# cherise215/Cooperative_Training_and_Latent_Space_Data_Augmentation

Hardware: AMD Instinct MI355X
Metric: cooperative-training slices/sec (256x256, bs16 per GPU) (higher is better)
Workload: dtype f32 (bf16x3 split)

## Files before the change

cooperative_training_and_latent_space_data_augmentation_amd/_ffi.py:

```python
from __future__ import annotations

import ctypes as C
import os

import numpy as np

_HERE = os.path.dirname(os.path.abspath(__file__))
LIB_PATH = os.path.join(_HERE, "csrc", "libctl_hip.so")
ABI_VERSION = 11
RED_BLOCKS = 512

IN_PLAIN, IN_UP2, IN_ZINS2, IN_C4 = 0, 1, 2, 3
ACT_NONE, ACT_LEAKY, ACT_SIGMOID = 0, 1, 2
EPI_BIAS, EPI_ACCUM, EPI_RES, EPI_STATS, EPI_BNBWD, EPI_TAILBWD = 1, 2, 4, 8, 16, 32
(OP_CONV, OP_WGRAD, OP_WGRAD_REDUCE, OP_PACK, OP_BN_FINALIZE, OP_BN_EVAL, OP_BN_ACT, OP_BWD_REDUCE, OP_BN_BWD_FINALIZE,
 OP_BWD_APPLY, OP_CHAN_SUM_FINALIZE, OP_SUMPOOL2, OP_SIGMOID_BWD, OP_ZERO, OP_COPY, OP_PACK_BATCH, OP_WGRAD_REDUCE_BATCH, OP_DROPOUT2D, OP_BN_REPLAY,
 OP_WGRAD_GROUP) = range(1, 21)
WGRAD_GROUP_MAX = 8
OP_MAX_T = 14

CONV_DTYPE = np.dtype([
    ("n", "<i4"), ("hin", "<i4"), ("win", "<i4"), ("cin", "<i4"), ("hout", "<i4"), ("wout", "<i4"), ("cout", "<i4"),
    ("ks", "<i4"), ("stride", "<i4"), ("pad", "<i4"), ("in_mode", "<i4"), ("pro_affine", "<i4"), ("pro_slope", "<f4"),
    ("epi_flags", "<i4"), ("epi_act", "<i4"), ("epi_slope", "<f4"), ("out_h", "<i4"), ("out_w", "<i4"),
    ("out_sy", "<i4"), ("out_sx", "<i4"), ("nsub", "<i4"), ("out_sub", "<i4"), ("groups", "<i4"), ("dt", "<i4")])
DT_BF16, DT_X16, DT_Y16, DT_RES16, DT_X3 = 1, 2, 4, 8, 16
PACK_X3 = 16
OP_DTYPE = np.dtype([("kind", "<i4"), ("i", "<i4", (27,)), ("f", "<f4", (4,)), ("slot", "<i4", (OP_MAX_T,)),
                     ("off", "<i8", (OP_MAX_T,)), ("l", "<i8", (4,))], align=True)


class CtlError(RuntimeError):
    pass


class _Lib:
    def __init__(self):
        self._lib = None

    def load(self):
        if self._lib is not None:
            return self._lib
        if not os.path.exists(LIB_PATH):
            raise CtlError(f"HIP extension not built: {LIB_PATH} is missing. Run `python -c 'import __graft_entry__ as g; "
                           "g.build()'` (or `make -C <package>/csrc`). There is no fallback path.")
        import torch
        lib = C.CDLL(LIB_PATH)
        lib.ctl_last_error.restype = C.c_char_p
        lib.ctl_version.restype = C.c_int
        lib.ctl_launch_count.restype = C.c_ulonglong
        for name in ("ctl_conv_wpack_floats", "ctl_conv_stats_floats", "ctl_wgrad_partial_floats",
                     "ctl_wgrad_bias_partial_floats", "ctl_latent_score_ws_floats", "ctl_latent_mask_apply_ws_floats",
                     "ctl_rescale_intensity_ws_floats", "ctl_sizeof_op", "ctl_sizeof_conv", "ctl_latent_mask_fused_ws_floats", "ctl_conv_wpack_floats_x3",
                     "ctl_surface_stats_ws_bytes", "ctl_surface_map_ws_bytes", "ctl_cc_ws_bytes", "ctl_aug_ws_bytes", "ctl_aug_warp_ws_bytes",
                     "ctl_aug_spline_ws_bytes", "ctl_aug_warp_cubic_ws_bytes", "ctl_aug_bias_ws_bytes"):
            getattr(lib, name).restype = C.c_size_t
        p, i32, i64, f32, u64 = C.c_void_p, C.c_int32, C.c_int64, C.c_float, C.c_uint64
        sig = {
            "ctl_conv_wpack_floats": [i32, i32, i32],
            "ctl_conv_stats_floats": [p], "ctl_conv_stats_blocks": [p],
            "ctl_wgrad_splits": [p], "ctl_wgrad_partial_floats": [p], "ctl_wgrad_bias_partial_floats": [p],
            "ctl_pack_weights": [p, p, i32, i32, i32, i64, i64, i64, i64, i32, p],
            "ctl_conv_forward": [p] * 12, "ctl_conv_forward_ex": [p] * 16, "ctl_conv_pool_ok": [p],
            "ctl_conv_wgrad": [p] * 8, "ctl_conv_wgrad_ex": [p] * 10,
            "ctl_wgrad_group_class": [p, i32], "ctl_wgrad_group_plan": [p, i32, p], "ctl_conv_wgrad_group": [i32] + [p] * 11,
            "ctl_wgrad_reduce": [p, p, p, p, i64, i64, i64, i64, p, i32, p],
            "ctl_confusion_hist": [p, p, i64, i32, p, p],
            "ctl_rescale_intensity": [p, p, p, i32, i64, f32, f32, f32, p],
            "ctl_noise_clamp": [p, p, u64, f32, f32, f32, p, i64, p],
            "ctl_rescale_intensity_ws_floats": [i32],
            "ctl_crop_or_pad": [p, p, i32, i32, i32, i32, i32, i32, p],
            "ctl_bn_finalize": [p, i32, i32, i64, p, p, f32, f32, i32, p, p, p, p, p, p, p, i32, p],
            "ctl_bn_finalize_ex": [p, i32, i32, i64, p, p, f32, f32, i32, p, p, p, p, p, p, p, p, i32, p],
            "ctl_bn_replay_running": [p, p, p, p, i32, f32, p],
            "ctl_bn_eval_coeffs": [i32, p, p, p, p, f32, p, p, i32, p],
            "ctl_bn_act": [p, p, p, f32, p, i64, i32, i32, p],
            "ctl_bwd_reduce": [i32, p, p, p, p, p, f32, i64, i32, p, i32, p], "ctl_red_blocks": [],
            "ctl_bn_bwd_finalize": [p, i32, i64, p, p, p, p, p, p, i32, i32, i32, p],
            "ctl_bn_bwd_finalize_ex": [p, i32, i64, p, p, p, p, p, p, i32, i32, i32, C.c_uint32, p],
            "ctl_bwd_apply": [i32, p, p, p, p, p, f32, p, i64, i32, p, p, i32, p],
            "ctl_chan_sum_finalize": [p, i32, p, i32, p],
            "ctl_sumpool2": [p, p, i32, i32, i32, i32, i32, p],
            "ctl_sigmoid_bwd": [p, p, p, i64, p],
            "ctl_softmax_t_fwd": [p, f32, p, i64, i32, p],
            "ctl_softmax_t_bwd": [p, p, f32, p, i64, i32, p],
            "ctl_onehot": [p, p, i64, i32, p],
            "ctl_ce2d_fwd": [p, p, i64, i32, p, p, p],
            "ctl_ce2d_bwd": [p, p, p, i64, i32, p, p],
            "ctl_mse_fwd": [p, p, i64, f32, p, p, p],
            "ctl_mse_bwd": [p, p, p, i64, f32, p, p],
            "ctl_argmax_c": [p, p, i64, i32, p],
            "ctl_latent_score_ws_floats": [i32, i32, i32, i32],
            "ctl_latent_score": [i32, p, p, p, i32, i32, i32, p],
            "ctl_latent_mask_apply": [i32, p, p, p, i32, p, p, p, p, i32, i32, i32, p],
            "ctl_latent_mask_apply_ws_floats": [i32, i32, i32, i32],
            "ctl_latent_mask_fused_ws_floats": [i32, i32, i32, i32],
            "ctl_latent_mask_fused": [i32, p, p, p, i32, p, p, p, p, p, i32, i32, i32, p],
            "ctl_dropout2d": [p, p, u64, f32, p, p, i32, i32, i32, p],
            "ctl_uniform": [p, i64, u64, p],
            "ctl_step_tick": [p, p],
            "ctl_spin": [i32, p],
            "ctl_dropout2d_ex": [p, p, u64, p, f32, p, p, p, i32, i32, i32, p],
            "ctl_dropout2d_dt": [p, p, u64, p, f32, p, p, i32, i32, i32, C.c_uint32, p],
            "ctl_uniform_dev": [p, i64, u64, p, p],
            "ctl_adam_dev": [p, p, p, p, i64, f32, f32, f32, f32, p, f32, p],
            "ctl_adam": [p, p, p, p, i64, f32, f32, f32, f32, i32, f32, p],
            "ctl_accumulate": [p, p, i32, i64, p],
            "ctl_plan_run": [p, i32, p, i32, p],
            "ctl_prof_start": [C.c_char_p], "ctl_prof_start_sampled": [C.c_char_p, i32], "ctl_prof_stop": [p, C.c_size_t],
            "ctl_pack_weights_batched": [p, p, p, i32, i64, p], "ctl_wgrad_reduce_batched": [p, p, p, i32, i64, p],
            "ctl_pack_weights_bf16_batched": [p, p, p, i32, i64, p],
            "ctl_pack_weights_x3_batched": [p, p, p, i32, i64, p], "ctl_conv_wpack_floats_x3": [i32, i32, i32],
            "ctl_bwd_reduce_rows": [i32, i64, i32],
            "ctl_bn_act_dt": [p, p, p, f32, p, i64, i32, i32, C.c_uint32, p],
            "ctl_bwd_reduce_dt": [i32, p, p, p, p, p, f32, i64, i32, p, i32, C.c_uint32, p, p],
            "ctl_bwd_apply_dt": [i32, p, p, p, p, p, f32, p, i64, i32, p, p, i32, C.c_uint32, p],
            "ctl_sumpool2_dt": [p, p, i32, i32, i32, i32, i32, C.c_uint32, p],
            "ctl_surface_stats_rows": [i32, i32, i32, i32], "ctl_surface_stats_ws_bytes": [i32] * 6,
            "ctl_surface_stats": [p, p, i32, i32, i32, i32, i32, i32, i32, p, p, p, C.c_size_t, p],
            "ctl_surface_map_ws_bytes": [i32] * 4,
            "ctl_surface_map": [p, i32, i32, i32, i32, i32, p, p, p, p, C.c_size_t, p],
            "ctl_cc_ws_bytes": [i32] * 5, "ctl_cc_label": [p, i32, i32, i32, i32, i32, i32, p, p],
            "ctl_cc_keep_largest": [p, i32, i32, i32, i32, i32, i32, p, p, p, C.c_size_t, p],
            "ctl_aug_ws_bytes": [i32] * 3, "ctl_aug_warp_ws_bytes": [i32] * 5, "ctl_aug_field": [p, p, p, p, i32, i32, i32, p, p, C.c_size_t, p],
            "ctl_aug_warp": [p, p, p, p, p, i32, i32, i32, i32, i32, p, p, p, C.c_size_t, p],
            "ctl_aug_spline_ws_bytes": [i32] * 4, "ctl_aug_warp_cubic_ws_bytes": [i32] * 6,
            "ctl_aug_spline_coeffs": [p, p, p, i32, i32, i32, i32, p, p, C.c_size_t, p],
            "ctl_aug_warp_cubic": [p, p, p, p, p, i32, i32, i32, i32, i32, i32, p, p, p, C.c_size_t, p],
            "ctl_aug_bias_ws_bytes": [i32] * 3, "ctl_aug_bias": [p, p, p, p, i32, i32, i32, p, p, C.c_size_t, p],
            "ctl_aug_coarse_field": [p, i32, i32, i32, p, p],
        }
        for name, args in sig.items():
            getattr(lib, name).argtypes = args
        if lib.ctl_version() != ABI_VERSION or lib.ctl_sizeof_op() != OP_DTYPE.itemsize or lib.ctl_sizeof_conv() != CONV_DTYPE.itemsize:
            raise CtlError(f"ABI mismatch: library version {lib.ctl_version()} vs binding {ABI_VERSION}, sizeof(ctl_op)={lib.ctl_sizeof_op()} "
                           f"vs {OP_DTYPE.itemsize}, sizeof(ctl_conv)={lib.ctl_sizeof_conv()} vs {CONV_DTYPE.itemsize}")
        if lib.ctl_red_blocks() != RED_BLOCKS:
            raise CtlError(f"ABI mismatch: the library was built with CTL_RED_BLOCKS={lib.ctl_red_blocks()}, this binding sizes scratch for {RED_BLOCKS}")
        self._lib = lib
        return lib

    def __getattr__(self, name):
        return getattr(self.load(), name)


lib = _Lib()

EXPORTED = ["ctl_version", "ctl_last_error", "ctl_conv_wpack_floats", "ctl_conv_stats_floats", "ctl_conv_stats_blocks",
            "ctl_pack_weights", "ctl_conv_forward", "ctl_conv_forward_ex", "ctl_conv_pool_ok", "ctl_wgrad_splits", "ctl_wgrad_partial_floats",
            "ctl_wgrad_bias_partial_floats", "ctl_conv_wgrad", "ctl_conv_wgrad_ex", "ctl_wgrad_reduce", "ctl_bn_finalize", "ctl_bn_finalize_ex", "ctl_bn_replay_running", "ctl_bn_eval_coeffs",
            "ctl_bn_act", "ctl_bwd_reduce", "ctl_bn_bwd_finalize", "ctl_bn_bwd_finalize_ex", "ctl_bwd_apply", "ctl_chan_sum_finalize", "ctl_sumpool2",
            "ctl_sigmoid_bwd", "ctl_softmax_t_fwd", "ctl_softmax_t_bwd", "ctl_onehot", "ctl_ce2d_fwd", "ctl_ce2d_bwd",
            "ctl_mse_fwd", "ctl_mse_bwd", "ctl_argmax_c", "ctl_latent_score_ws_floats", "ctl_latent_score",
            "ctl_latent_mask_apply", "ctl_latent_mask_apply_ws_floats", "ctl_dropout2d", "ctl_uniform", "ctl_adam", "ctl_plan_run", "ctl_sizeof_op",
            "ctl_sizeof_conv", "ctl_prof_start", "ctl_prof_start_sampled", "ctl_prof_stop", "ctl_pack_weights_batched",
            "ctl_wgrad_reduce_batched", "ctl_confusion_hist", "ctl_rescale_intensity_ws_floats", "ctl_rescale_intensity",
            "ctl_noise_clamp", "ctl_crop_or_pad", "ctl_step_tick", "ctl_spin", "ctl_dropout2d_ex", "ctl_dropout2d_dt", "ctl_uniform_dev", "ctl_adam_dev",
            "ctl_latent_mask_fused_ws_floats", "ctl_latent_mask_fused", "ctl_accumulate", "ctl_pack_weights_bf16_batched",
            "ctl_bn_act_dt", "ctl_bwd_reduce_dt", "ctl_bwd_apply_dt", "ctl_sumpool2_dt", "ctl_bwd_reduce_rows", "ctl_red_blocks",
            "ctl_launch_count", "ctl_conv_wpack_floats_x3", "ctl_pack_weights_x3_batched", "ctl_wgrad_group_class", "ctl_wgrad_group_plan",
            "ctl_conv_wgrad_group", "ctl_surface_stats_rows", "ctl_surface_stats_ws_bytes", "ctl_surface_stats", "ctl_surface_map_ws_bytes",
            "ctl_surface_map", "ctl_cc_ws_bytes", "ctl_cc_label", "ctl_cc_keep_largest", "ctl_aug_ws_bytes", "ctl_aug_warp_ws_bytes", "ctl_aug_field",
            "ctl_aug_warp", "ctl_aug_spline_ws_bytes", "ctl_aug_warp_cubic_ws_bytes", "ctl_aug_spline_coeffs", "ctl_aug_warp_cubic",
            "ctl_aug_bias_ws_bytes", "ctl_aug_bias", "ctl_aug_coarse_field"]


def prof_start(kernel_filter: str = "", every: int = 1) -> None:
    check(lib.ctl_prof_start_sampled(kernel_filter.encode(), int(every)), "ctl_prof_start_sampled")


def prof_stop() -> dict:
    buf = C.create_string_buffer(1 << 18)
    check(lib.ctl_prof_stop(buf, len(buf)), "ctl_prof_stop")
    out = {}
    for line in buf.value.decode().splitlines():
        parts = line.split()
        out[parts[0]] = {k: float(v) for k, v in (kv.split("=") for kv in parts[1:])}
    return out


def check(rc: int, what: str = "") -> None:
    if rc != 0:
        msg = lib.ctl_last_error()
        raise CtlError(f"{what} failed (rc={rc}): {msg.decode() if msg else ''}")


def conv_desc(**kw) -> np.ndarray:
    d = np.zeros((), dtype=CONV_DTYPE)
    d["pad"] = 1 if kw.get("ks", 3) in (3, 4) else 0
    d["stride"] = 1
    d["nsub"] = 1
    d["groups"] = 1
    d["out_sy"] = d["out_sx"] = 1
    for k, v in kw.items():
        d[k] = v
    if "out_h" not in kw:
        d["out_h"] = d["hout"]
    if "out_w" not in kw:
        d["out_w"] = d["wout"]
    return d


def desc_ptr(d: np.ndarray) -> int:
    return d.ctypes.data
```

cooperative_training_and_latent_space_data_augmentation_amd/csrc/ctl_common.h:

```cpp
#pragma once
#include <hip/hip_runtime.h>
#include <stdint.h>
#include <stdio.h>
#include "ctl_hip.h"

void ctl_set_error(const char* fmt, ...);

#define CTL_FAIL(code, ...)            \
    do {                               \
        ctl_set_error(__VA_ARGS__);    \
        return (code);                 \
    } while (0)

#define CTL_REQUIRE(cond, ...)                        \
    do {                                              \
        if (!(cond)) CTL_FAIL(CTL_EINVAL, __VA_ARGS__); \
    } while (0)

void ctl_count_launches(int n);
#define CTL_LAUNCH_CHECK(name)                                                         \
    do {                                                                               \
        ctl_count_launches(1);                                                         \
        hipError_t e__ = hipGetLastError();                                            \
        if (e__ != hipSuccess) CTL_FAIL(CTL_ELAUNCH, "%s: %s", name, hipGetErrorString(e__)); \
    } while (0)

__host__ __device__ static inline int ctl_cdiv(int a, int b) { return (a + b - 1) / b; }
__host__ __device__ static inline int64_t ctl_cdiv64(int64_t a, int64_t b) { return (a + b - 1) / b; }

typedef float f32x4 __attribute__((ext_vector_type(4)));

__device__ __forceinline__ float ctl_leaky(float v, float slope) { return v > 0.f ? v : v * slope; }
__device__ __forceinline__ float ctl_leaky_grad(float out, float slope) { return out > 0.f ? 1.f : slope; }

__device__ __forceinline__ void ctl_barrier_lds_reads_done() { asm volatile("s_barrier" ::: "memory"); }
__device__ __forceinline__ void ctl_barrier_lds_writes_done() { asm volatile("s_waitcnt lgkmcnt(0)\n\ts_barrier" ::: "memory"); }

#ifdef CTL_TUNING
#include <stdlib.h>
static inline int ctl_tune_int(const char* name, int dflt) { const char* e = getenv(name); return e ? atoi(e) : dflt; }
static inline const char* ctl_tune_str(const char* name) { return getenv(name); }
#else
static inline constexpr int ctl_tune_int(const char*, int dflt) { return dflt; }
static inline constexpr const char* ctl_tune_str(const char*) { return nullptr; }
#endif

typedef unsigned int u32x2e __attribute__((ext_vector_type(2)));
typedef __bf16 bf16x2e __attribute__((ext_vector_type(2)));
typedef float f32x2e __attribute__((ext_vector_type(2)));
__device__ __forceinline__ f32x4 ldq(const void* __restrict__ p, int64_t i, bool b16) {
    if (b16) {
        const u32x2e u = reinterpret_cast<const u32x2e*>(p)[i];
        return f32x4{__builtin_bit_cast(float, u.x << 16), __builtin_bit_cast(float, u.x & 0xffff0000u),
                     __builtin_bit_cast(float, u.y << 16), __builtin_bit_cast(float, u.y & 0xffff0000u)};
    }
    return reinterpret_cast<const f32x4*>(p)[i];
}
#ifndef CTL_ELEM_NT
#define CTL_ELEM_NT 0
#endif
__device__ __forceinline__ void stq(void* __restrict__ p, int64_t i, f32x4 v, bool b16) {
    if (b16) {
        const u32x2e pk = u32x2e{__builtin_bit_cast(unsigned, __builtin_convertvector(f32x2e{v.x, v.y}, bf16x2e)),
                                 __builtin_bit_cast(unsigned, __builtin_convertvector(f32x2e{v.z, v.w}, bf16x2e))};
        if (CTL_ELEM_NT) __builtin_nontemporal_store(pk, reinterpret_cast<u32x2e*>(p) + i); else reinterpret_cast<u32x2e*>(p)[i] = pk;
    } else {
        if (CTL_ELEM_NT) __builtin_nontemporal_store(v, reinterpret_cast<f32x4*>(p) + i); else reinterpret_cast<f32x4*>(p)[i] = v;
    }
}

__device__ __forceinline__ double wave_sum_double(double v) {
    for (int o = 32; o > 0; o >>= 1) v += __shfl_xor(v, o);
    return v;
}

struct ctl_bn_chan { float gamma, beta, rm, rv; };
__device__ __forceinline__ ctl_bn_chan ctl_bn_chan_load(int ch, const float* __restrict__ gamma, const float* __restrict__ beta,
                                                        int update_running, const float* __restrict__ running_mean,
                                                        const float* __restrict__ running_var) {
    ctl_bn_chan p;
    p.gamma = gamma[ch]; p.beta = beta[ch];
    p.rm = update_running ? running_mean[ch] : 0.f;
    p.rv = update_running ? running_var[ch] : 0.f;
    return p;
}
__device__ __forceinline__ void ctl_bn_coefs(double s1, double s2, double count, int c, int g, int ch, ctl_bn_chan& p, float eps,
                                             float momentum, int update_running, float* __restrict__ running_mean,
                                             float* __restrict__ running_var, float* __restrict__ scale, float* __restrict__ shift,
                                             float* __restrict__ save_mean, float* __restrict__ save_invstd,
                                             float* __restrict__ save_uvar = nullptr) {
    const double mean = s1 / count;
    double var = s2 / count - mean * mean;
    if (var < 0.0) var = 0.0;
    const float invstd = (float)(1.0 / sqrt(var + (double)eps));
    const float sc = p.gamma * invstd;
    scale[g * c + ch] = sc;
    shift[g * c + ch] = p.beta - (float)mean * sc;
    if (save_mean) save_mean[g * c + ch] = (float)mean;
    if (save_invstd) save_invstd[g * c + ch] = invstd;
    if (update_running) {
        const double unbiased = count > 1.0 ? var * count / (count - 1.0) : var;
        if (save_uvar) save_uvar[g * c + ch] = (float)unbiased;
        p.rm = (1.f - momentum) * p.rm + momentum * (float)mean;
        p.rv = (1.f - momentum) * p.rv + momentum * (float)unbiased;
        running_mean[ch] = p.rm;
        running_var[ch] = p.rv;
    }
}
struct ctl_conv_cfg {
    int mt, tw, nt;
    int th;
    int tiles_h, tiles_w;
    int g;
    int cot;
    int pc;
};
int ctl_conv_pick_cfg(const ctl_conv* d, ctl_conv_cfg* c, int for_wgrad);
int ctl_conv_grid_x(int ntiles, int other, int occ);
static inline int ctl_num_cus() { static const int n = ctl_tune_int("CTL_NUM_CUS", 256); return n; }

int ctl_conv_forward_bf16(const ctl_conv* d, const void* x, const void* x2, const void* wpack, const float* bias, const float* pro_scale,
                          const float* pro_shift, const void* res, const float* res_scale, const float* res_shift, const void* res2, void* y,
                          float* stats_partial, void* pool, void* xout, ctl_stream stream);
int ctl_conv_bf16_stats_blocks(const ctl_conv* d);
int ctl_wgrad_bf16_splits(const ctl_conv* d);
int ctl_conv_wgrad_bf16(const ctl_conv* d, const void* x, const float* pro_scale, const float* pro_shift, const void* dy, const void* dy2,
                        const float* dy_coef, float* w_partial, float* b_partial, ctl_stream stream);

int ctl_wgrad_bf16_group_class(const ctl_conv* d, int has_dy2);
int ctl_wgrad_bf16_group_plan(const ctl_conv* descs, int n, int32_t* splits);
int ctl_conv_wgrad_bf16_group(int n, const ctl_conv* descs, const int32_t* splits, const void* const* x, const float* const* pro_scale,
                              const float* const* pro_shift, const void* const* dy, const void* const* dy2, const float* const* dy_coef,
                              float* const* w_partial, float* const* b_partial, ctl_stream stream);

int ctl_conv_x3_ok(const ctl_conv* d);
int ctl_conv_x3_stats_blocks(const ctl_conv* d);
int ctl_conv_forward_x3(const ctl_conv* d, const float* x, const float* wpack, const float* bias, const float* pro_scale, const float* pro_shift,
                        const float* res, const float* res_scale, const float* res_shift, const float* res2, const float* x2, float* y,
                        float* stats_partial, float* pool, float* xout, ctl_stream stream);

int ctl_wgrad_x3_ok(const ctl_conv* d);
int ctl_wgrad_x3_splits(const ctl_conv* d);
int ctl_conv_wgrad_x3(const ctl_conv* d, const float* x, const float* pro_scale, const float* pro_shift, const float* dy, const float* dy2,
                      const float* dy_coef, float* w_partial, float* b_partial, ctl_stream stream);

int ctl_prof_begin(const char* kind, const ctl_conv* d, const ctl_conv_cfg* c, int nt, hipStream_t stream, bool dy2 = false);
void ctl_prof_end(int token, hipStream_t stream);
int ctl_prof_begin_raw(const char* id, double flops, double bytes, hipStream_t stream);
```

cooperative_training_and_latent_space_data_augmentation_amd/csrc/ctl_conv.hip:

```cpp
#include <stdlib.h>

#include <type_traits>

#include "ctl_common.h"

#include "ctl_conv_common.h"

#ifdef CTL_TIMING
#define CTL_TM_WAVES 65536
__device__ unsigned long long ctl_tm[CTL_TM_WAVES][10];
#define TM_DECL unsigned long long tm_prev = __builtin_amdgcn_s_memtime(), tm_acc[10] = {0, 0, 0, 0, 0, 0, 0, 0, 0, 0}; \
                const unsigned long long tm_t0 = tm_prev, tm_r0 = __builtin_amdgcn_s_memrealtime();
#define TM(i) { const unsigned long long tm_now = __builtin_amdgcn_s_memtime(); tm_acc[i] += tm_now - tm_prev; tm_prev = tm_now; }
#define TM_COUNT(i) { tm_acc[i] += 1; }
#define TM_FLUSH { const unsigned w_ = ((blockIdx.x + gridDim.x * (blockIdx.y + gridDim.y * blockIdx.z)) * 4 + (threadIdx.x >> 6)) % CTL_TM_WAVES; \
                   tm_acc[8] = __builtin_amdgcn_s_memtime() - tm_t0; tm_acc[9] = __builtin_amdgcn_s_memrealtime() - tm_r0; \
                   if ((threadIdx.x & 63) == 0) { _Pragma("unroll") for (int i_ = 0; i_ < 10; ++i_) ctl_tm[w_][i_] += tm_acc[i_]; } }
extern "C" int ctl_debug_timing(unsigned long long* out8) {
    static unsigned long long host[CTL_TM_WAVES][10];
    if (hipMemcpyFromSymbol(host, HIP_SYMBOL(ctl_tm), sizeof(host)) != hipSuccess) return -1;
    for (int i = 0; i < 12; ++i) out8[i] = 0;
    for (int w = 0; w < CTL_TM_WAVES; ++w) {
        for (int i = 0; i < 10; ++i) out8[i] += host[w][i];
        if (host[w][8] > out8[10]) out8[10] = host[w][8];
// ... 466 lines not shown
    constexpr int TPR = (LDS_FLOATS / TAP_FLOATS) < NACC ? (LDS_FLOATS / TAP_FLOATS) : NACC;
    const int64_t split_base = (int64_t)blockIdx.x * TAPS * cin_p * cout_p;
#pragma unroll
    for (int tap0 = 0; tap0 < NACC; tap0 += TPR) {
        if (tap0 > 0) ctl_barrier_lds_reads_done();
#pragma unroll
        for (int tp = 0; tp < TPR; ++tp) {
            const int tap = tap0 + tp;
            if (tap < NACC) {
#pragma unroll
                for (int t = 0; t < NTW; ++t) {
                    float* r0 = red + tp * TAP_FLOATS + ((wave * NTW + t) * 4) * 64 + lane;
                    r0[0] = acc[tap][t].x; r0[64] = acc[tap][t].y; r0[128] = acc[tap][t].z; r0[192] = acc[tap][t].w;
                }
            }
        }
        ctl_barrier_lds_writes_done();
#pragma unroll
        for (int tp = 0; tp < TPR; ++tp) {
            const int tap = tap0 + tp;
            if (tap < NACC) {
#pragma unroll
                for (int e0 = 0; e0 < NTW * 256; e0 += 256) {
                    const int e = e0 + tid;
                    const int t = e >> 8, r = (e >> 6) & 3, l = e & 63;
                    float v = 0.f;
#pragma unroll
                    for (int w = 0; w < 4; ++w) v += red[tp * TAP_FLOATS + ((w * NTW + t) * 4 + r) * 64 + l];
                    const int co = (cot0 + t) * 16 + (l & 15);
                    if (C4) {
                        const int wtap = 4 * tap + (l >> 4);
                        if (wtap < TAPS && co < cout_p) w_partial[split_base + ((int64_t)wtap * cin_p + r) * cout_p + co] = v;
                    } else {
                        const int ci = g * 16 + (l >> 4) * 4 + r;
                        if (co < cout_p) w_partial[split_base + ((int64_t)tap * cin_p + ci) * cout_p + co] = v;
                    }
                }
            }
        }
    }
    if (g == 0 && b_partial != nullptr) {
        ctl_barrier_lds_reads_done();
#pragma unroll
        for (int t = 0; t < NTW; ++t) {
            float v = bsum[t];
            v += __shfl_xor(v, 16);
            v += __shfl_xor(v, 32);
            if (q == 0) red[(wave * NTW + t) * 16 + p] = v;
        }
        ctl_barrier_lds_writes_done();
        if (tid < NTW * 16) {
            float v = 0.f;
#pragma unroll
            for (int w = 0; w < 4; ++w) v += red[w * NTW * 16 + tid];
            const int co = cot0 * 16 + tid;
            if (co < cout_p) b_partial[(int64_t)blockIdx.x * cout_p + co] = v;
        }
    }
#ifdef CTL_TIMING_WGRAD
    tm_acc[5] += __builtin_amdgcn_s_memtime() - tm_loop_end;
    TM_FLUSH
#endif
}

__global__ __launch_bounds__(256) void wgrad_reduce_kernel(const float* __restrict__ w_partial,
                                                            const float* __restrict__ b_partial, int splits, int taps,
                                                            int ks, int cin, int cout, int cin_p, int cout_p,
                                                            float* __restrict__ dw, int64_t s_co, int64_t s_ci,
                                                            int64_t s_kh, int64_t s_kw, float* __restrict__ dbias,
                                                            int accumulate) {
    __shared__ float sm[8][32];
    const int e = threadIdx.x & 31, sl = threadIdx.x >> 5;
    const int64_t total = (int64_t)taps * cin * cout;
    const int64_t idx = (int64_t)blockIdx.x * 32 + e;
    const bool is_w = idx < total;
    const bool is_b = !is_w && dbias != nullptr && idx < total + cout;
    float v = 0.f;
    int co = 0, ci = 0, tap = 0;
    if (is_w) {
        co = idx % cout;
        ci = (idx / cout) % cin;
        tap = idx / ((int64_t)cout * cin);
        const int64_t stride = (int64_t)taps * cin_p * cout_p;
        const float* src = w_partial + ((int64_t)tap * cin_p + ci) * cout_p + co;
        for (int s = sl; s < splits; s += 8) v += src[s * stride];
    } else if (is_b) {
        co = idx - total;
        for (int s = sl; s < splits; s += 8) v += b_partial[(int64_t)s * cout_p + co];
    }
    sm[sl][e] = v;
    __syncthreads();
    if (sl == 0 && (is_w || is_b)) {
        float t = 0.f;
#pragma unroll
        for (int k = 0; k < 8; ++k) t += sm[k][e];
        float* dst = is_w ? dw + co * s_co + ci * s_ci + (tap / ks) * s_kh + (tap % ks) * s_kw : dbias + co;
        *dst = accumulate ? (*dst + t) : t;
    }
}

__global__ void pack_weights_kernel(const float* __restrict__ src, float* __restrict__ dst, int cout, int cin, int ks,
                                    int g_chunks, int64_t total, int64_t s_co, int64_t s_ci, int64_t s_kh,
                                    int64_t s_kw, int flip) {
    const int64_t idx = (int64_t)blockIdx.x * blockDim.x + threadIdx.x;
    if (idx >= total) return;
    const int j = idx & 3, lane = (idx >> 2) & 63;
    int64_t rest = idx >> 8;
    const int g = rest % g_chunks;
    rest /= g_chunks;
    const int taps = ks * ks;
    const int tap = rest % taps;
    const int cot = rest / taps;
    const int co = cot * 16 + (lane & 15);
    const int ci = g * 16 + (lane >> 4) * 4 + j;
    int kh = tap / ks, kw = tap % ks;
    if (flip) { kh = ks - 1 - kh; kw = ks - 1 - kw; }
    float v = 0.f;
    if (co < cout && ci < cin) v = src[co * s_co + ci * s_ci + kh * s_kh + kw * s_kw];
    dst[idx] = v;
}

__global__ void pack_weights_batched_kernel(const float* __restrict__ params, float* __restrict__ wpack,
                                            const int64_t* __restrict__ table) {
    const int64_t* r = table + (int64_t)blockIdx.y * 12;
    const int64_t total = r[10];
    const int64_t idx = (int64_t)blockIdx.x * blockDim.x + threadIdx.x;
    if (idx >= total || (r[11] & CTL_PACK_X3)) return;
    const float* src = params + r[0];
    float* dst = wpack + r[1];
    const int cout = (int)r[2], cin = (int)r[3], ks = (int)r[4], flip = (int)r[5];
    const int g_chunks = (cin + 15) / 16;
    const int j = idx & 3, lane = (idx >> 2) & 63;
    int64_t rest = idx >> 8;
    const int g = rest % g_chunks;
    rest /= g_chunks;
    const int taps = ks * ks;
    const int tap = rest % taps;
    const int cot = rest / taps;
    const int co = cot * 16 + (lane & 15);
    const int ci = g * 16 + (lane >> 4) * 4 + j;
    int kh = tap / ks, kw = tap % ks;
    float v = 0.f;
    if (r[11] == 4) {
        const int c = j, quad = (int)((idx >> 8) % 3), cot4 = (int)((idx >> 8) / 3);
        const int co4 = cot4 * 16 + (lane & 15), tp = 4 * quad + (lane >> 4);
        if (co4 < cout && c < cin && tp < 9) v = src[co4 * r[6] + c * r[7] + (tp / 3) * r[8] + (tp % 3) * r[9]];
        dst[idx] = v;
        return;
    }
    if (r[11] == 1) {
        if (co < cout && ci < cin) {
            for (int a = 0; a < 2; ++a) {
                const int sh = a + 2 - kh;
                if (sh < 0 || sh > 2) continue;
                for (int b = 0; b < 2; ++b) {
                    const int sw = b + 2 - kw;
                    if (sw < 0 || sw > 2) continue;
                    v += src[co * r[6] + ci * r[7] + sh * r[8] + sw * r[9]];
                }
            }
        }
    } else if (r[11] == 2) {
        if (co < cout && ci < cin) {
            const int a = flip >> 1, b = flip & 1;
            const int h0 = (kh == 0) ? 0 : (a ? 2 : 1), h1 = (kh == 0) ? (a ? 1 : 0) : 2;
            const int w0 = (kw == 0) ? 0 : (b ? 2 : 1), w1 = (kw == 0) ? (b ? 1 : 0) : 2;
            for (int sh = h0; sh <= h1; ++sh)
                for (int sw = w0; sw <= w1; ++sw) v += src[co * r[6] + ci * r[7] + sh * r[8] + sw * r[9]];
        }
    } else if (r[11] == 3) {
        if (co < cout && ci < cin) {
            const int a = flip >> 1, b = flip & 1;
            const int sh = a ? (kh == 0 ? 2 : 0) : (kh == 0 ? 1 : -1);
            const int sw = b ? (kw == 0 ? 2 : 0) : (kw == 0 ? 1 : -1);
            if (sh >= 0 && sw >= 0) v = src[co * r[6] + ci * r[7] + sh * r[8] + sw * r[9]];
        }
    } else {
        if (flip) { kh = ks - 1 - kh; kw = ks - 1 - kw; }
        if (co < cout && ci < cin) v = src[co * r[6] + ci * r[7] + kh * r[8] + kw * r[9]];
    }
    dst[idx] = v;
}

__global__ __launch_bounds__(256) void wgrad_reduce_batched_kernel(const float* __restrict__ scratch, float* __restrict__ grad,
                                                                    const int64_t* __restrict__ table) {
    __shared__ float sm[32][65];
    const int64_t* r = table + (int64_t)blockIdx.y * 16;
    const int splits = (int)r[4], taps = (int)(r[5] & 0xff), ks = (int)(r[5] >> 8), cin = (int)r[6], cout = (int)r[7];
    const int cin_p = (int)r[8], cout_p = (int)r[9];
    const int64_t total = (int64_t)taps * cin * cout;
    const bool has_b = r[1] >= 0 && r[3] >= 0;
    const bool wide = splits <= 64;
    const int EW = wide ? 64 : 8, SLN = wide ? 4 : 32;
    if ((int64_t)blockIdx.x * EW >= total + (has_b ? cout : 0)) return;
    const int e = wide ? (threadIdx.x & 63) : (threadIdx.x & 7), sl = wide ? (threadIdx.x >> 6) : (threadIdx.x >> 3);
    const int64_t idx = (int64_t)blockIdx.x * EW + e;
    const bool is_w = idx < total, is_b = !is_w && has_b && idx < total + cout;
    float v = 0.f;
    int co = 0, ci = 0, tap = 0;
    if (is_w) {
        co = idx % cout;
        ci = (idx / cout) % cin;
        tap = idx / ((int64_t)cout * cin);
        const int64_t stride = (int64_t)taps * cin_p * cout_p;
        const float* src = scratch + r[0] + ((int64_t)tap * cin_p + ci) * cout_p + co;
        for (int s0 = sl; s0 < splits; s0 += 8 * SLN) {
            float t8[8];
#pragma unroll
            for (int u = 0; u < 8; ++u) { const int s = s0 + u * SLN; t8[u] = s < splits ? src[s * stride] : 0.f; }
#pragma unroll
            for (int u = 0; u < 8; ++u) v += t8[u];
        }
    } else if (is_b) {
        co = idx - total;
        const float* src = scratch + r[1] + co;
        for (int s = sl; s < splits; s += SLN) v += src[(int64_t)s * cout_p];
    }
    sm[sl][e] = v;
    __syncthreads();
    if (sl == 0 && (is_w || is_b)) {
        float t = 0.f;
        for (int k = 0; k < SLN; ++k) t += sm[k][e];
        float* dst = is_w ? grad + r[2] + co * r[10] + ci * r[11] + (tap / ks) * r[12] + (tap % ks) * r[13] : grad + r[3] + co;
        *dst = r[14] ? (*dst + t) : t;
    }
}

extern "C" int ctl_pack_weights_batched(const float* params, float* wpack, const int64_t* table, int32_t n_rec,
                                        int64_t max_total, ctl_stream stream) {
    CTL_REQUIRE(params && wpack && table && n_rec > 0 && max_total > 0, "pack_weights_batched: bad arguments");
    pack_weights_batched_kernel<<<dim3((unsigned)ctl_cdiv64(max_total, 256), (unsigned)n_rec), dim3(256), 0, (hipStream_t)stream>>>(
        params, wpack, table);
    CTL_LAUNCH_CHECK("pack_weights_batched");
    return CTL_OK;
}
extern "C" int ctl_wgrad_reduce_batched(const float* scratch, float* grad, const int64_t* table, int32_t n_rec,
                                        int64_t max_elems, ctl_stream stream) {
    CTL_REQUIRE(scratch && grad && table && n_rec > 0 && max_elems > 0, "wgrad_reduce_batched: bad arguments");
    wgrad_reduce_batched_kernel<<<dim3((unsigned)max_elems, (unsigned)n_rec), dim3(256), 0, (hipStream_t)stream>>>(
        scratch, grad, table);
    CTL_LAUNCH_CHECK("wgrad_reduce_batched");
    return CTL_OK;
}

extern "C" size_t ctl_conv_wpack_floats(int32_t cin, int32_t cout, int32_t ks) {
    return (size_t)ctl_cdiv(cout, 16) * ks * ks * ctl_cdiv(cin, 16) * 256;
}

static bool conv_combo_ok(const ctl_conv* d) {
    const int k = d->ks, s = d->stride, m = d->in_mode, pd = d->pad;
    if (k == 3 && s == 1 && pd == 1 && m != CTL_IN_C4) return true;
    if (k == 3 && s == 1 && pd == 1 && m == CTL_IN_C4 && d->cin <= 4 && d->nsub == 1) return true;
    if (k == 3 && s == 2 && pd == 1 && m == CTL_IN_PLAIN) return true;
    if (k == 1 && s == 1 && pd == 0 && m != CTL_IN_ZINS2) return true;
    if (k == 2 && s == 2 && pd == 0 && m == CTL_IN_PLAIN) return true;
    if (k == 4 && s == 2 && pd == 1 && m == CTL_IN_PLAIN) return true;
    if (k == 2 && s == 1 && (pd == 0 || pd == 2) && m == CTL_IN_PLAIN && d->nsub == 4) return true;
    return false;
}

int ctl_conv_pick_cfg(const ctl_conv* d, ctl_conv_cfg* c, int for_wgrad) {
    CTL_REQUIRE(conv_combo_ok(d), "conv: unsupported ks/stride/pad/in_mode %d/%d/%d/%d", d->ks, d->stride, d->pad,
                d->in_mode);
    CTL_REQUIRE(d->cin == 1 || d->cin % 4 == 0, "conv: cin must be 1 or a multiple of 4 (got %d)", d->cin);
    CTL_REQUIRE(d->cout == 1 || d->cout % 4 == 0, "conv: cout must be 1 or a multiple of 4 (got %d)", d->cout);
    CTL_REQUIRE(d->cin < 16 ? (d->cin == 1 || d->cin == 4 || d->cin == 8 || d->cin == 12) : d->cin % 16 == 0,
                "conv: cin >= 16 must be a multiple of 16 (got %d)", d->cin);
    CTL_REQUIRE(d->nsub == 1 || d->nsub == 4, "conv: nsub must be 1 or 4");
    c->cot = ctl_cdiv(d->cout, 16);
    c->g = ctl_cdiv(d->cin, 16);
    c->nt = (c->cot % 2 == 0) ? 2 : 1;
    auto blocks = [&](int mt, int tw) {
        const int th = 4 * mt * 16 / tw;
        return (int64_t)d->n * ctl_cdiv(d->hout, th) * ctl_cdiv(d->wout, tw) * (c->cot / c->nt) * d->nsub;
    };
    int mt, tw;
    if (for_wgrad) {
        if (d->hout >= 8) { mt = 2; tw = 16; }
        else { mt = 1; tw = 16; }
    } else if (d->stride == 2) {
        if (blocks(2, 16) >= 384) { mt = 2; tw = 16; } else { mt = 1; tw = 16; }
        if (d->ks == 4 && c->nt == 2) { mt = 1; tw = 16; }
    } else if (d->wout >= 32 && blocks(4, 32) >= 512 && !(c->nt == 2 && blocks(4, 32) > 768)) {
        mt = 4; tw = 32;
    } else if (blocks(2, 16) >= 384) {
        mt = 2; tw = 16;
    } else {
        mt = 1; tw = 16;
    }
    {
        static int fm = 0, ft = 0, fn = 0;
        static const bool forced = [] {
            const char* f = ctl_tune_str("CTL_FORCE_CFG");
            return f && sscanf(f, "%d,%d,%d", &fm, &ft, &fn) == 3;
        }();
        if (forced) {
            const bool tile_ok = (fm == 4 && ft == 32 && d->stride == 1 && !for_wgrad) || (fm == 2 && ft == 16) || (fm == 1 && ft == 16);
            if (tile_ok) { mt = fm; tw = ft; }
            if ((fn == 1 || fn == 2) && c->cot % fn == 0) c->nt = fn;
            if (d->ks == 4 && c->nt == 2) { mt = 1; tw = 16; }
        }
    }
    c->pc = 0;
    c->mt = mt; c->tw = tw; c->th = 4 * mt * 16 / tw;
    c->tiles_h = ctl_cdiv(d->hout, c->th);
    c->tiles_w = ctl_cdiv(d->wout, c->tw);
    return CTL_OK;
}

int ctl_conv_grid_x(int ntiles, int other, int occ) {
    static int per_cu = -1;
    if (per_cu < 0) {
        per_cu = ctl_tune_int("CTL_PERSIST", 4);
        if (per_cu < 1) per_cu = 1;
    }
    const int resident = occ < per_cu ? occ : per_cu;
    int cap = (ctl_num_cus() * resident) / other;
    if (other > 1 && cap >= 8) cap -= cap % 8;
    if (cap < 1) cap = 1;
    return ntiles < cap ? ntiles : cap;
}

extern "C" int ctl_pack_weights(const float* src, float* dst, int32_t cout, int32_t cin, int32_t ks, int64_t s_co,
                                int64_t s_ci, int64_t s_kh, int64_t s_kw, int32_t flip, ctl_stream stream) {
    CTL_REQUIRE(src && dst && cout > 0 && cin > 0 && ks >= 1 && ks <= 4, "pack_weights: bad arguments");
    const int64_t total = (int64_t)ctl_conv_wpack_floats(cin, cout, ks);
    pack_weights_kernel<<<dim3((unsigned)ctl_cdiv64(total, 256)), dim3(256), 0, (hipStream_t)stream>>>(
        src, dst, cout, cin, ks, ctl_cdiv(cin, 16), total, s_co, s_ci, s_kh, s_kw, flip);
    CTL_LAUNCH_CHECK("pack_weights");
    return CTL_OK;
}

struct conv_call {
    const ctl_conv* d; ctl_conv_cfg c;
    const float *x, *wpack, *bias, *pro_scale, *pro_shift, *res, *res_scale, *res_shift, *res2, *x2;
    float *y, *stats_partial, *pool, *xout;
    hipStream_t stream;
    bool query;
    int grid_x;
};

template <int KS, int S, int MODE, int MT, int TW, int NT, int EPI, bool X2 = false>
static void conv_go(conv_call& a) {
    if constexpr (!X2 && ((KS == 3 && S == 1 && MODE == CTL_IN_PLAIN) || (KS == 4 && S == 2)) && EPI != 2) {
        if (a.d->pro_affine == 2) { conv_go<KS, S, MODE, MT, TW, NT, EPI, true>(a); return; }
    }
    static int occ = 0;
    if (!occ) {
        int n = 0;
        if (hipOccupancyMaxActiveBlocksPerMultiprocessor(&n, conv_igemm_kernel<KS, S, MODE, MT, TW, NT, EPI, X2>, 256, 0) != hipSuccess || n < 1) {
            (void)hipGetLastError();
            n = 2;
        }
        occ = n;
    }
    const ctl_conv* d = a.d;
    const int ntiles = d->n * a.c.tiles_h * a.c.tiles_w;
    a.grid_x = ctl_conv_grid_x(ntiles, (a.c.cot / NT) * d->nsub, occ);
    if (a.query) return;
    const dim3 grid((unsigned)a.grid_x, (unsigned)(a.c.cot / NT), (unsigned)d->nsub);
    conv_igemm_kernel<KS, S, MODE, MT, TW, NT, EPI, X2><<<grid, dim3(256), 0, a.stream>>>(
        *d, a.x, a.wpack, a.bias, a.pro_scale, a.pro_shift, a.res, a.res_scale, a.res_shift, a.y, a.stats_partial, a.c.tiles_h,
        a.c.tiles_w, a.c.g, (int64_t)ctl_conv_wpack_floats(d->cin, d->cout, d->ks), ntiles, a.res2, a.x2, a.pool, a.xout);
}
template <int KS, int S, int MODE>
constexpr bool conv_tail_ok() { return (KS == 1 && MODE == CTL_IN_PLAIN) || KS == 2 || (KS == 3 && S == 1 && MODE == CTL_IN_ZINS2); }
template <int KS, int S, int MODE, int MT, int TW>
static void conv_go_nt(conv_call& a) {
    const bool epi = (a.d->epi_flags & (CTL_EPI_RES | CTL_EPI_ACCUM | CTL_EPI_BNBWD)) != 0;
    if constexpr (conv_tail_ok<KS, S, MODE>()) {
        if (a.d->epi_flags & CTL_EPI_TAILBWD) {
            if (a.c.nt == 2) conv_go<KS, S, MODE, MT, TW, 2, 2>(a); else conv_go<KS, S, MODE, MT, TW, 1, 2>(a);
            return;
        }
    }
    if constexpr (KS == 3 && S == 1 && MODE == CTL_IN_PLAIN) {
        if ((a.d->epi_flags & (CTL_EPI_RES | CTL_EPI_ACCUM | CTL_EPI_BNBWD)) == CTL_EPI_BNBWD && a.d->cout % 16 == 0 && a.d->epi_act == CTL_ACT_NONE) {
            if (a.c.nt == 2) conv_go<KS, S, MODE, MT, TW, 2, 3>(a); else conv_go<KS, S, MODE, MT, TW, 1, 3>(a);
            return;
        }
    }
    if (a.c.nt == 2) { if (epi) conv_go<KS, S, MODE, MT, TW, 2, 1>(a); else conv_go<KS, S, MODE, MT, TW, 2, 0>(a); }
    else { if (epi) conv_go<KS, S, MODE, MT, TW, 1, 1>(a); else conv_go<KS, S, MODE, MT, TW, 1, 0>(a); }
}
template <int KS, int S, int MODE>
static void conv_go_tile(conv_call& a) {
    if (S == 1 && a.c.mt == 4 && a.c.tw == 32) conv_go_nt<KS, S, MODE, (S == 1 ? 4 : 2), (S == 1 ? 32 : 16)>(a);
    else if (a.c.mt == 2) conv_go_nt<KS, S, MODE, 2, 16>(a);
    else conv_go_nt<KS, S, MODE, 1, 16>(a);
}
static int conv_dispatch(conv_call& a) {
    const int k = a.d->ks, s = a.d->stride, m = a.d->in_mode;
    if (k == 3 && s == 1 && m == CTL_IN_PLAIN) conv_go_tile<3, 1, CTL_IN_PLAIN>(a);
    else if (k == 3 && s == 1 && m == CTL_IN_UP2) conv_go_tile<3, 1, CTL_IN_UP2>(a);
    else if (k == 3 && s == 1 && m == CTL_IN_ZINS2) conv_go_tile<3, 1, CTL_IN_ZINS2>(a);
    else if (k == 3 && s == 1 && m == CTL_IN_C4) conv_go_tile<3, 1, CTL_IN_C4>(a);
    else if (k == 3 && s == 2) conv_go_tile<3, 2, CTL_IN_PLAIN>(a);
    else if (k == 1 && m == CTL_IN_PLAIN) conv_go_tile<1, 1, CTL_IN_PLAIN>(a);
    else if (k == 1 && m == CTL_IN_UP2) conv_go_tile<1, 1, CTL_IN_UP2>(a);
    else if (k == 2 && s == 2) conv_go_tile<2, 2, CTL_IN_PLAIN>(a);
    else if (k == 2 && s == 1) conv_go_tile<2, 1, CTL_IN_PLAIN>(a);
    else if (k == 4 && s == 2) {
        const bool epi = (a.d->epi_flags & (CTL_EPI_RES | CTL_EPI_ACCUM | CTL_EPI_BNBWD)) != 0;
        if (a.c.mt == 2 && a.c.nt == 1) { if (epi) conv_go<4, 2, CTL_IN_PLAIN, 2, 16, 1, 1>(a); else conv_go<4, 2, CTL_IN_PLAIN, 2, 16, 1, 0>(a); }
        else if (a.c.nt == 2) { if (epi) conv_go<4, 2, CTL_IN_PLAIN, 1, 16, 2, 1>(a); else conv_go<4, 2, CTL_IN_PLAIN, 1, 16, 2, 0>(a); }
        else { if (epi) conv_go<4, 2, CTL_IN_PLAIN, 1, 16, 1, 1>(a); else conv_go<4, 2, CTL_IN_PLAIN, 1, 16, 1, 0>(a); }
    }
    else CTL_FAIL(CTL_EUNSUPPORTED, "conv_forward: no kernel for this combination");
    return CTL_OK;
}

extern "C" int ctl_conv_stats_blocks(const ctl_conv* d) {
    if (d->dt & CTL_DT_BF16) return ctl_conv_bf16_stats_blocks(d);
    if (d->dt & CTL_DT_X3) return ctl_conv_x3_stats_blocks(d);
    conv_call a = {};
    a.d = d;
    if (ctl_conv_pick_cfg(d, &a.c, 0) != CTL_OK) return -1;
    a.query = true;
    if (conv_dispatch(a) != CTL_OK) return -1;
    return a.grid_x * d->nsub;
}
extern "C" size_t ctl_conv_stats_floats(const ctl_conv* d) {
    const int b = ctl_conv_stats_blocks(d);
    return b < 0 ? 0 : (size_t)(d->groups > 1 ? d->groups : 1) * b * 2 * d->cout;
}

extern "C" int ctl_conv_forward(const ctl_conv* d, const float* x, const float* wpack, const float* bias,
                                const float* pro_scale, const float* pro_shift, const float* res,
                                const float* res_scale, const float* res_shift, float* y, float* stats_partial,
                                ctl_stream stream) {
    return ctl_conv_forward_ex(d, x, wpack, bias, pro_scale, pro_shift, res, res_scale, res_shift, nullptr, nullptr, y, stats_partial, nullptr, nullptr, stream);
}
extern "C" int ctl_conv_pool_ok(const ctl_conv* d) {
    ctl_conv_cfg c;
    if (!d) return 0;
    if (!(d->epi_flags & CTL_EPI_TAILBWD) || d->ks != 1 || d->stride != 1 || d->in_mode != CTL_IN_PLAIN || d->nsub != 1 || (d->out_h & 1) || (d->out_w & 1) ||
        d->out_h != d->hout || d->out_w != d->wout || d->cout % 16 != 0)
        return 0;
    if (ctl_conv_pick_cfg(d, &c, 0) != CTL_OK) return 0;
    return (c.mt == 4 && c.tw == 32) || (c.mt == 2 && c.tw == 16);
}
extern "C" int ctl_conv_forward_ex(const ctl_conv* d, const float* x, const float* wpack, const float* bias,
                                   const float* pro_scale, const float* pro_shift, const float* res,
                                   const float* res_scale, const float* res_shift, const float* res2, const float* x2, float* y,
                                   float* stats_partial, float* pool, float* xout, ctl_stream stream) {
    CTL_REQUIRE(d && x && wpack && y, "conv_forward: null argument");
    CTL_REQUIRE(!xout || d->pro_affine == 2, "conv_forward: `xout` (the virtual input written out) goes with the BatchNorm-backward prologue (pro_affine 2)");
    CTL_REQUIRE(!pool || ctl_conv_pool_ok(d), "conv_forward: `pool` needs a CTL_EPI_TAILBWD 1x1 conv with even output sizes whose tile configuration gives every wave a row pair (ctl_conv_pool_ok)");
    CTL_REQUIRE((d->dt & CTL_DT_BF16) || !(d->dt & (CTL_DT_X16 | CTL_DT_Y16 | CTL_DT_RES16)), "conv_forward: bf16-stored tensors need CTL_DT_BF16");
    conv_call a = {};
    a.d = d;
    int rc = ctl_conv_pick_cfg(d, &a.c, 0);
    if (rc != CTL_OK) return rc;
    CTL_REQUIRE(!(d->epi_flags & CTL_EPI_BIAS) || bias, "conv_forward: CTL_EPI_BIAS without bias");
    CTL_REQUIRE(!(d->epi_flags & CTL_EPI_RES) || (res && res_scale && res_shift), "conv_forward: CTL_EPI_RES without res");
    CTL_REQUIRE(!(d->epi_flags & CTL_EPI_STATS) || stats_partial, "conv_forward: CTL_EPI_STATS without a partial buffer");
    CTL_REQUIRE(!(d->epi_flags & CTL_EPI_BNBWD) || ((d->epi_flags & CTL_EPI_STATS) && res && res_scale && res_shift &&
                                                    !(d->epi_flags & (CTL_EPI_RES | CTL_EPI_ACCUM | CTL_EPI_BIAS)) && d->epi_act == CTL_ACT_NONE),
                "conv_forward: CTL_EPI_BNBWD needs CTL_EPI_STATS + res (= u) + res_scale/res_shift (BatchNorm coefficients) and nothing else");
    if (d->epi_flags & CTL_EPI_TAILBWD) {
        const int k = d->ks, s = d->stride, m = d->in_mode;
        CTL_REQUIRE((d->epi_flags & CTL_EPI_STATS) && res && res2 && !(d->epi_flags & (CTL_EPI_RES | CTL_EPI_BNBWD | CTL_EPI_BIAS)) &&
                    d->epi_act == CTL_ACT_NONE && d->cout % 16 == 0,
                    "conv_forward: CTL_EPI_TAILBWD needs CTL_EPI_STATS + res (= the block output) + res2 (= the BatchNorm input), cout %% 16 == 0, nothing else but CTL_EPI_ACCUM");
        CTL_REQUIRE((k == 1 && m == CTL_IN_PLAIN) || k == 2 || (k == 3 && s == 1 && m == CTL_IN_ZINS2),
                    "conv_forward: CTL_EPI_TAILBWD is built for the launches that write a block's output gradient (1x1, 2x2, zero-insert 3x3)");
        CTL_REQUIRE(d->epi_slope >= 0.f && d->epi_slope <= 1.f, "conv_forward: LeakyReLU slope must be in [0, 1]");
    }
    CTL_REQUIRE(d->pro_affine >= 0 && d->pro_affine <= 2, "conv_forward: pro_affine must be 0, 1 or 2");
    CTL_REQUIRE(d->pro_affine != 1 || (pro_scale && pro_shift), "conv_forward: prologue without scale/shift");
    CTL_REQUIRE(d->pro_affine != 2 || (x2 && pro_scale && d->cin % 16 == 0 && d->in_mode == CTL_IN_PLAIN &&
                                       ((d->ks == 3 && d->stride == 1) || (d->ks == 4 && d->stride == 2)) && !(d->epi_flags & CTL_EPI_TAILBWD)),
                "conv_forward: the BatchNorm-backward prologue (pro_affine 2) needs x2 + coefficients, cin %% 16 == 0 and a plain 3x3 stride-1 or 4x4 stride-2 conv");
    CTL_REQUIRE(!d->pro_affine || (d->groups > 1 ? d->groups : 1) * d->cin <= CTL_PRO_MAX, "conv_forward: groups * cin = %d prologue coefficients exceed %d", (d->groups > 1 ? d->groups : 1) * d->cin, CTL_PRO_MAX);
    CTL_REQUIRE(d->pro_affine != 1 || (d->pro_slope >= 0.f && d->pro_slope <= 1.f), "conv_forward: prologue slope must be in [0, 1]");
    CTL_REQUIRE(d->epi_act != CTL_ACT_LEAKY || (d->epi_slope >= 0.f && d->epi_slope <= 1.f), "conv_forward: LeakyReLU slope must be in [0, 1]");
    CTL_REQUIRE(d->n > 0 && d->hout > 0 && d->wout > 0, "conv_forward: empty problem");
    CTL_REQUIRE(d->groups >= 0 && (d->groups <= 1 || d->n % d->groups == 0), "conv_forward: n=%d is not divisible into %d groups", d->n, d->groups);
    CTL_REQUIRE((int64_t)d->n * d->hin * d->win * d->cin * 4 < (1ll << 31) &&
                (int64_t)d->n * d->out_h * d->out_w * d->cout * 4 < (1ll << 31),
                "conv_forward: tensors must stay below 2 GiB (32-bit buffer offsets)");
    if (d->dt & CTL_DT_X3)
        return ctl_conv_forward_x3(d, x, wpack, bias, pro_scale, pro_shift, res, res_scale, res_shift, res2, x2, y, stats_partial, pool, xout, stream);
    if (d->dt & CTL_DT_BF16) {
        const int ptok16 = ctl_prof_begin("conv_igemm_bf16", d, &a.c, a.c.nt, (hipStream_t)stream);
        rc = ctl_conv_forward_bf16(d, x, x2, wpack, bias, pro_scale, pro_shift, res, res_scale, res_shift, res2, y, stats_partial, pool, xout, stream);
        ctl_prof_end(ptok16, (hipStream_t)stream);
        return rc;
    }
    a.x = x; a.wpack = wpack; a.bias = bias; a.pro_scale = pro_scale; a.pro_shift = pro_shift; a.res = res;
    a.res_scale = res_scale; a.res_shift = res_shift; a.res2 = res2; a.x2 = x2; a.y = y; a.stats_partial = stats_partial; a.pool = pool; a.xout = xout;
    a.stream = (hipStream_t)stream;
    const int ptok = ctl_prof_begin("conv_igemm", d, &a.c, a.c.nt, a.stream);
    rc = conv_dispatch(a);
    if (rc != CTL_OK) return rc;
    ctl_prof_end(ptok, a.stream);
    CTL_LAUNCH_CHECK("conv_forward");
    return CTL_OK;
}

#ifndef CTL_WGRAD_PIPE
#define CTL_WGRAD_PIPE 1
#endif
struct wgrad_cfg { ctl_conv_cfg c; int ntw, splits, ntiles, cin_p, cout_p; };

struct wgrad_call {
    const ctl_conv* d; wgrad_cfg* w;
    const float *x, *pro_scale, *pro_shift, *dy, *dy2, *dy_coef;
    float *w_partial, *b_partial;
    hipStream_t stream;
    bool query;
};

template <int KS, int S, int MODE, int MT, int TW, int NTW>
static void wgrad_go(wgrad_call& a) {
    static int occ = 0;
    if (!occ) {
        int n = 0;
        if (hipOccupancyMaxActiveBlocksPerMultiprocessor(&n, conv_wgrad_kernel<KS, S, MODE, MT, TW, NTW>, 256, 0) != hipSuccess || n < 1) {
            (void)hipGetLastError();
            n = 2;
        }
        occ = n;
    }
    wgrad_cfg& w = *a.w;
    static int per_cu = -1;
    if (per_cu < 0) {
        per_cu = ctl_tune_int("CTL_WGRAD_PERSIST", 1);
        if (per_cu < 1) per_cu = 1;
    }
    const int par = w.c.g * (w.c.cot / NTW);
    static const int slots = ctl_tune_int("CTL_WGRAD_SLOTS", 0);
    static const int narrow_cu = ctl_tune_int("CTL_WGRAD_NARROW_PERSIST", 2);
    const int cu_blocks = (KS == 1 || MODE == CTL_IN_C4) ? narrow_cu : per_cu;
    int splits = (slots > 0 ? slots : ctl_num_cus() * (occ < cu_blocks ? occ : cu_blocks)) / par;
    if (splits > 512) splits = 512;
    if (splits > w.ntiles) splits = w.ntiles;
    if (splits < 1) splits = 1;
    w.splits = splits;
    if (a.query) return;
    const dim3 grid((unsigned)splits, (unsigned)w.c.g, (unsigned)(w.c.cot / NTW));
    if constexpr (KS == 3 && S == 1 && MODE != CTL_IN_C4) {
        static const int pipe = ctl_tune_int("CTL_WGRAD_PIPE", CTL_WGRAD_PIPE);
        const bool pipe_on = pipe >= 2 || (pipe == 1 && a.dy2 && w.ntiles >= 8 * splits);
        if (pipe_on && a.d->cin % 4 == 0 && a.d->cout % 4 == 0 && a.d->cin <= CTL_PRO_MAX) {
            if (a.dy2)
                conv_wgrad_kernel<KS, S, MODE, MT, TW, NTW, true, true><<<grid, dim3(256), 0, a.stream>>>(
                    *a.d, a.x, a.pro_scale, a.pro_shift, a.dy, a.w_partial, a.b_partial, w.c.tiles_h, w.c.tiles_w, w.ntiles, w.cin_p, w.cout_p, a.dy2, a.dy_coef);
            else
                conv_wgrad_kernel<KS, S, MODE, MT, TW, NTW, false, true><<<grid, dim3(256), 0, a.stream>>>(
                    *a.d, a.x, a.pro_scale, a.pro_shift, a.dy, a.w_partial, a.b_partial, w.c.tiles_h, w.c.tiles_w, w.ntiles, w.cin_p, w.cout_p, nullptr, nullptr);
            return;
        }
    }
    if constexpr (KS == 3 && S == 1) {
        if (a.dy2) {
            conv_wgrad_kernel<KS, S, MODE, MT, TW, NTW, true><<<grid, dim3(256), 0, a.stream>>>(
                *a.d, a.x, a.pro_scale, a.pro_shift, a.dy, a.w_partial, a.b_partial, w.c.tiles_h, w.c.tiles_w, w.ntiles, w.cin_p, w.cout_p, a.dy2, a.dy_coef);
            return;
        }
    }
    conv_wgrad_kernel<KS, S, MODE, MT, TW, NTW><<<grid, dim3(256), 0, a.stream>>>(
        *a.d, a.x, a.pro_scale, a.pro_shift, a.dy, a.w_partial, a.b_partial, w.c.tiles_h, w.c.tiles_w, w.ntiles, w.cin_p, w.cout_p, nullptr, nullptr);
}
template <int KS, int S, int MODE>
static void wgrad_go_tile(wgrad_call& a) {
    const wgrad_cfg& w = *a.w;
    if (w.c.mt == 2) { if (w.ntw == 2) wgrad_go<KS, S, MODE, 2, 16, 2>(a); else wgrad_go<KS, S, MODE, 2, 16, 1>(a); }
    else { if (w.ntw == 2) wgrad_go<KS, S, MODE, 1, 16, 2>(a); else wgrad_go<KS, S, MODE, 1, 16, 1>(a); }
}
static int wgrad_dispatch(wgrad_call& a) {
    const int k = a.d->ks, s = a.d->stride, m = a.d->in_mode;
    if (k == 3 && s == 1 && m == CTL_IN_PLAIN) wgrad_go_tile<3, 1, CTL_IN_PLAIN>(a);
    else if (k == 3 && s == 1 && m == CTL_IN_UP2) wgrad_go_tile<3, 1, CTL_IN_UP2>(a);
    else if (k == 3 && s == 1 && m == CTL_IN_C4) wgrad_go_tile<3, 1, CTL_IN_C4>(a);
    else if (k == 3 && s == 2) wgrad_go_tile<3, 2, CTL_IN_PLAIN>(a);
    else if (k == 1 && m == CTL_IN_PLAIN) wgrad_go_tile<1, 1, CTL_IN_PLAIN>(a);
    else if (k == 1 && m == CTL_IN_UP2) wgrad_go_tile<1, 1, CTL_IN_UP2>(a);
    else if (k == 2 && s == 2) wgrad_go_tile<2, 2, CTL_IN_PLAIN>(a);
    else CTL_FAIL(CTL_EUNSUPPORTED, "conv_wgrad: no kernel for this combination");
    return CTL_OK;
}

static int wgrad_pick(const ctl_conv* d, wgrad_cfg* w) {
    CTL_REQUIRE(d->nsub == 1, "wgrad: nsub must be 1");
    CTL_REQUIRE(d->in_mode != CTL_IN_ZINS2, "wgrad: zero-insert input is not a forward mode");
    int rc = ctl_conv_pick_cfg(d, &w->c, 1);
    if (rc != CTL_OK) return rc;
    w->ntw = (w->c.cot >= 2 && w->c.cot % 2 == 0) ? 2 : 1;
    w->ntiles = d->n * w->c.tiles_h * w->c.tiles_w;
    w->cin_p = w->c.g * 16;
    w->cout_p = w->c.cot * 16;
    if (d->dt & CTL_DT_BF16) {
        w->splits = ctl_wgrad_bf16_splits(d);
        return w->splits > 0 ? CTL_OK : CTL_EUNSUPPORTED;
    }
    if (d->dt & CTL_DT_X3) {
        w->splits = ctl_wgrad_x3_splits(d);
        return w->splits > 0 ? CTL_OK : CTL_EUNSUPPORTED;
    }
    wgrad_call a = {};
    a.d = d; a.w = w; a.query = true;
    return wgrad_dispatch(a);
}

extern "C" int ctl_wgrad_splits(const ctl_conv* d) {
// ... 70 lines not shown
```

cooperative_training_and_latent_space_data_augmentation_amd/csrc/ctl_conv_igemm.h:

```cpp
#pragma once
#include <stdlib.h>

#include <type_traits>

#include "ctl_common.h"

#include "ctl_conv_common.h"
#include "ctl_conv_x3_stage.h"

#ifndef TM_DECL
#define TM_DECL
#define TM(i)
#define TM_COUNT(i)
#define TM_FLUSH
#endif

#define CTL_MODE_IS_PLAIN(M) ((M) == CTL_IN_PLAIN || (M) == CTL_IN_C4)

template <int KS, int S, int MODE, int MT, int TW, bool X2 = false>
struct XStage {
    using G = Geom<KS, S, MT, TW>;
    static constexpr bool C4M = (MODE == CTL_IN_C4);
    static constexpr int UNITS = G::IH * G::IW * (C4M ? 1 : 4);
    static constexpr int NU = (UNITS + 255) / 256;
    static constexpr int PADH = (G::PAD + 1) >> 1;
    int rel[NU];
    int rc[NU];
    int lds[NU];
    f32x4 v[NU];
    f32x4 v2[X2 ? NU : 1];
    unsigned vmask;
    int pad_h, pad_w;
    bool all_in;
    int tb_last;

    __device__ __forceinline__ void init(const ctl_conv& d) {
        const int tid = threadIdx.x, cq = C4M ? 0 : (tid & 3);
#pragma unroll
        for (int i = 0; i < NU; ++i) {
            const int u = tid + i * 256;
            const int pix = C4M ? u : (u >> 2);
            const int r = pix / G::IW;
            const int c = pix - r * G::IW;
            const bool in = u < UNITS;
            const int rr = CTL_MODE_IS_PLAIN(MODE) ? r : (((r - G::PAD) >> 1) + PADH);
            const int cc = CTL_MODE_IS_PLAIN(MODE) ? c : (((c - G::PAD) >> 1) + PADH);
            rel[i] = in ? ((rr * d.win + cc) * d.cin + cq * 4) * 4 : CTL_OOB;
            rc[i] = in ? (r | (c << 16)) : 0x7fff7fff;
            lds[i] = in ? (C4M ? (r * G::IWP + c) * 4 : ((r * G::IWP + G::ldscol(c)) * 16 + cq * 4)) : G::XT_IMAGE;
        }
        vmask = 0;
        all_in = false;
        pad_h = pad_w = G::PAD;
    }

    __device__ __forceinline__ void load(__amdgpu_buffer_rsrc_t rx, const ctl_conv& d, int n, int ho0, int wo0, int g) { load(rx, rx, d, n, ho0, wo0, g); }
    __device__ __forceinline__ void load(__amdgpu_buffer_rsrc_t rx, __amdgpu_buffer_rsrc_t rx2, const ctl_conv& d, int n, int ho0, int wo0, int g) {
        const int vh0 = ho0 * S - pad_h, vw0 = wo0 * S - pad_w;
        const unsigned hv = CTL_MODE_IS_PLAIN(MODE) ? d.hin : 2 * d.hin;
        const unsigned wv = CTL_MODE_IS_PLAIN(MODE) ? d.win : 2 * d.win;
        const int oh = CTL_MODE_IS_PLAIN(MODE) ? vh0 : ((ho0 >> 1) - PADH);
        const int ow = CTL_MODE_IS_PLAIN(MODE) ? vw0 : ((wo0 >> 1) - PADH);
        const int tb = (((n * d.hin + oh) * d.win + ow) * d.cin + g * 16) * 4;
        tb_last = tb;
#ifdef CTL_NO_INTERIOR
        all_in = false;
#else
        all_in = MODE != CTL_IN_ZINS2 && vh0 >= 0 && vw0 >= 0 && vh0 + G::IH <= (int)hv && vw0 + G::IW <= (int)wv &&
                 g * 16 + 16 <= d.cin;
#endif
        if (all_in) {
#pragma unroll
            for (int i = 0; i < NU; ++i) v[i] = ctl_bload4s(rx, rel[i], tb);
            if constexpr (X2) {
#pragma unroll
                for (int i = 0; i < NU; ++i) v2[i] = ctl_bload4s(rx2, rel[i], tb);
            }
            return;
        }
        const bool chan_ok = C4M || g * 16 + (threadIdx.x & 3) * 4 < d.cin;
        unsigned m = 0;
        int vo[NU];
#pragma unroll
        for (int i = 0; i < NU; ++i) {
            const int vh = vh0 + (rc[i] & 0xffff), vw = vw0 + (rc[i] >> 16);
            bool ok = chan_ok && (unsigned)vh < hv && (unsigned)vw < wv;
            if (MODE == CTL_IN_ZINS2) ok = ok && (((vh | vw) & 1) == 0);
            vo[i] = ok ? (tb + rel[i]) : CTL_OOB;
            m |= ok ? (1u << i) : 0u;
        }
        vmask = m;
        if constexpr (X2) {
#pragma unroll
            for (int i = 0; i < NU; ++i) { v[i] = ctl_bload4(rx, vo[i]); v2[i] = ctl_bload4(rx2, vo[i]); }
        } else if (d.cin >= 4) {
#pragma unroll
            for (int i = 0; i < NU; ++i) v[i] = ctl_bload4(rx, vo[i]);
        } else {
#pragma unroll
            for (int i = 0; i < NU; ++i) v[i] = f32x4{ctl_bload1(rx, vo[i]), 0.f, 0.f, 0.f};
        }
    }

    __device__ __forceinline__ void store(float* __restrict__ xt, const ctl_conv& d, int g,
                                          const float* pro_scale, const float* pro_shift, int goff, const float* pro_c = nullptr) {
        store(xt, d, g, pro_scale, pro_shift, goff, pro_c, ctl_rsrc((const void*)nullptr, 0), false);
    }
    __device__ __forceinline__ void store(float* __restrict__ xt, const ctl_conv& d, int g,
                                          const float* pro_scale, const float* pro_shift, int goff, const float* pro_c,
                                          __amdgpu_buffer_rsrc_t rxout, bool xout_on) {
        if constexpr (X2) {
            const int cb = g * 16 + (threadIdx.x & 3) * 4;
            const f32x4 ca = *reinterpret_cast<const f32x4*>(pro_scale + goff + cb), cbb = *reinterpret_cast<const f32x4*>(pro_shift + goff + cb);
            const f32x4 cc = *reinterpret_cast<const f32x4*>(pro_c + goff + cb);
            const f32x4 zero = {0.f, 0.f, 0.f, 0.f};
#pragma unroll
            for (int i = 0; i < NU; ++i) {
                const bool in = all_in || ((vmask >> i) & 1u);
                const f32x4 r = in ? (ca * v[i] + cbb * v2[i] + cc) : zero;
                *reinterpret_cast<f32x4*>(xt + lds[i]) = r;
                if (xout_on) {
                    const unsigned tr = (unsigned)((rc[i] & 0xffff) - pad_h), tc = (unsigned)((rc[i] >> 16) - pad_w);
                    const bool own = in && tr < (unsigned)(G::TH * S) && tc < (unsigned)(TW * S);
                    ctl_bstore4(rxout, own ? (tb_last + rel[i]) : CTL_OOB, r);
                }
            }
            return;
        }
        if (!d.pro_affine) {
#pragma unroll
            for (int i = 0; i < NU; ++i) *reinterpret_cast<f32x4*>(xt + lds[i]) = v[i];
            return;
        }
        const int cb = C4M ? 0 : g * 16 + (threadIdx.x & 3) * 4;
        f32x4 sc = {1.f, 1.f, 1.f, 1.f}, sh = {0.f, 0.f, 0.f, 0.f};
        if (cb < d.cin) {
            if (d.cin >= 4) {
                sc = *reinterpret_cast<const f32x4*>(pro_scale + goff + cb);
                sh = *reinterpret_cast<const f32x4*>(pro_shift + goff + cb);
            } else {
                sc.x = pro_scale[goff];
                sh.x = pro_shift[goff];
            }
        }
        const float slope = d.pro_slope;
        if (all_in) {
#pragma unroll
            for (int i = 0; i < NU; ++i) *reinterpret_cast<f32x4*>(xt + lds[i]) = ctl_leaky01(v[i] * sc + sh, slope);
            return;
        }
        const f32x4 zero = {0.f, 0.f, 0.f, 0.f};
#pragma unroll
        for (int i = 0; i < NU; ++i) {
            const f32x4 t = ctl_leaky01(v[i] * sc + sh, slope);
            *reinterpret_cast<f32x4*>(xt + lds[i]) = ((vmask >> i) & 1u) ? t : zero;
        }
    }
};


#ifndef CTL_LB_MID
#define CTL_LB_MID 3
#endif
#ifndef CTL_LB_SMALL
#define CTL_LB_SMALL 3
#endif
#ifndef CTL_PC_SETS
#define CTL_PC_SETS 3
#endif
#ifndef CTL_PC_SETS_X2
#define CTL_PC_SETS_X2 2
#endif
template <int KS, int S, int MODE, int MT, int TW, int NT, int EPI, bool X2 = false, bool X3 = false, bool PC = false>
#ifndef CTL_LB_X2EPI
#define CTL_LB_X2EPI 2
#endif
#ifndef CTL_LB_X2
#define CTL_LB_X2 2
#endif
#ifndef CTL_LB_SMALL_X2EPI
#define CTL_LB_SMALL_X2EPI CTL_LB_SMALL
#endif
#ifndef CTL_LB_X3
#define CTL_LB_X3(MT, NT, X2) (((NT) == 1 && (MT) >= 2 && !(X2)) ? 3 : 2)
#endif
__global__ __launch_bounds__(PC ? 512 : 256, PC ? 2 : X3 ? CTL_LB_X3(MT, NT, X2) : (MT * NT >= 8 || KS == 4) ? 2 : ((MT * NT >= 4) ? (X2 ? (EPI ? CTL_LB_X2EPI : CTL_LB_X2) : CTL_LB_MID)
                                                                                    : ((X2 && EPI) ? CTL_LB_SMALL_X2EPI : CTL_LB_SMALL))) void conv_igemm_kernel(const ctl_conv d, const float* __restrict__ x,
                                                          const float* __restrict__ wpack,
                                                          const float* __restrict__ bias,
                                                          const float* __restrict__ pro_scale,
                                                          const float* __restrict__ pro_shift,
                                                          const float* __restrict__ res,
                                                          const float* __restrict__ res_scale,
                                                          const float* __restrict__ res_shift, float* __restrict__ y,
                                                          float* __restrict__ stats_partial, int tiles_h, int tiles_w,
                                                          int G_chunks, int64_t wpack_sub_stride, int ntiles,
                                                          const float* __restrict__ res2, const float* __restrict__ x2,
                                                          float* __restrict__ pool, float* __restrict__ xout) {
    using G = Geom<KS, S, MT, TW>;
    constexpr int TAPS = KS * KS;
    constexpr bool C4 = (MODE == CTL_IN_C4);
    static_assert(!C4 || (KS == 3 && S == 1), "K-packed taps: 3x3 stride-1 only");
    static_assert(!X3 || !C4, "X3: whole 16-channel chunks");
    static_assert(!PC || X3, "the producer / consumer form exists for the X3 launches");
    constexpr int NIMG = PC ? 2 : 1;
    using XS3 = XStage3<KS, S, C4 ? CTL_IN_PLAIN : MODE, MT, TW, X2>;
    constexpr int NFRAG = X3 ? (TAPS + 1) / 2 : (C4 ? 3 : TAPS);
    constexpr int WSPL = X3 ? 3 : 1;
    constexpr int RED_FLOATS = 4 * NT * 16 * 2;
    constexpr int WT_FLOATS = NFRAG * NT * WSPL * 256;
    constexpr int XT_ALLOC = X3 ? XS3::XT_BYTES / 4 : G::XT_FLOATS;
    static_assert((NIMG * (XT_ALLOC + WT_FLOATS) + RED_FLOATS + (X2 ? 3 : 2) * CTL_PRO_MAX) * 4 <= 160 * 1024, "LDS budget of one CU");
    __shared__ __attribute__((aligned(16))) float xt[NIMG * (XT_ALLOC + WT_FLOATS) + RED_FLOATS + (X2 ? 3 : 2) * CTL_PRO_MAX];
    float* wt = xt + NIMG * XT_ALLOC;
    float* sred = wt + NIMG * WT_FLOATS;
    float* cf_scale = sred + RED_FLOATS;
    float* cf_shift = cf_scale + CTL_PRO_MAX;
    float* cf_c = cf_shift + (X2 ? CTL_PRO_MAX : 0);
    constexpr int WU = NFRAG * NT * WSPL * 64, NW = (WU + 255) / 256;

    const int tid = threadIdx.x;
    const int lane = tid & 63;
    const int wave_all = __builtin_amdgcn_readfirstlane(tid >> 6);
    const int wave = PC ? (wave_all & 3) : wave_all;
    const bool consumer = PC && wave_all >= 4;
    const int p = lane & 15, q = lane >> 4;
    const int P = gridDim.x < 8 ? (int)gridDim.x : 8;
    const int xcd = blockIdx.x % P, jblk = blockIdx.x / P;
    const int nb = ((int)gridDim.x - xcd + P - 1) / P;
    const int t_lo = (int)(((int64_t)ntiles * xcd) / P), t_hi = (int)(((int64_t)ntiles * (xcd + 1)) / P);
    const int bid0 = t_lo + jblk;
    const int z = blockIdx.z;
    const int cot0 = blockIdx.y * NT;
    const float* wp = wpack + (int64_t)z * wpack_sub_stride;
    const int my_tiles = (bid0 < t_hi) ? (t_hi - bid0 + nb - 1) / nb : 0;
    const int total_it = my_tiles * G_chunks;
    const int flags = d.epi_flags;
    const int ngroups = d.groups > 1 ? d.groups : 1;
    const int group_n = d.n / ngroups;
    const int oy0 = (z >> 1) * d.out_sub, ox0 = (z & 1) * d.out_sub;
    const __amdgpu_buffer_rsrc_t rx = ctl_rsrc(x, (int64_t)d.n * d.hin * d.win * d.cin * 4);
    const __amdgpu_buffer_rsrc_t rx2 = X2 ? ctl_rsrc(x2, (int64_t)d.n * d.hin * d.win * d.cin * 4) : rx;
    const bool xout_on = X2 && xout != nullptr && blockIdx.y == 0 && blockIdx.z == 0;
    const __amdgpu_buffer_rsrc_t rxout = xout_on ? ctl_rsrc(xout, (int64_t)d.n * d.hin * d.win * d.cin * 4) : rx;
    const int64_t ybytes = (int64_t)d.n * d.out_h * d.out_w * d.cout * 4;
    const __amdgpu_buffer_rsrc_t ry = ctl_rsrc(y, ybytes);
    const __amdgpu_buffer_rsrc_t rres = ctl_rsrc(EPI ? (const void*)res : (const void*)y, ybytes);
    constexpr bool TAIL = (EPI == 2);
    const __amdgpu_buffer_rsrc_t rres2 = ctl_rsrc(TAIL ? (const void*)res2 : (const void*)y, ybytes);
    constexpr bool CAN_POOL = TAIL && KS == 1 && S == 1 && MODE == CTL_IN_PLAIN && (MT / (TW / 16)) == 2;
    const __amdgpu_buffer_rsrc_t rpool = ctl_rsrc(CAN_POOL && pool ? (const void*)pool : (const void*)y, CAN_POOL && pool ? ybytes / 4 : ybytes);

    f32x4 ssum[NT], ssq[NT];
#pragma unroll
    for (int t = 0; t < NT; ++t) ssum[t] = ssq[t] = f32x4{0.f, 0.f, 0.f, 0.f};

    constexpr int TWT = TW / 16;
    static_assert(MT % TWT == 0, "a wave's M-tiles must cover whole tile rows");
    const int wrow = wave * (MT / TWT);
    int yrel[MT];
#pragma unroll
    for (int m = 0; m < MT; ++m)
        yrel[m] = (((wrow + m / TWT) * d.out_sy * d.out_w + ((m % TWT) * 16 + p) * d.out_sx) * d.cout + q * 4) * 4;
    const float* xrd = xt + ((wrow * S) * G::IWP + p) * 16 + q * 4;
    const float* wrd = wt + lane * 4;
    const float* xrd4[3];
#pragma unroll
    for (int j = 0; j < 3; ++j) {
        const int tp = (4 * j + q < 9) ? 4 * j + q : 8;
        xrd4[j] = xt + ((wrow + tp / 3) * G::IWP + p + tp % 3) * 4;
    }
    int xoff3[X3 ? NFRAG : 1];
    if constexpr (X3) {
#pragma unroll
        for (int f = 0; f < NFRAG; ++f) {
            int tap = 2 * f + (q >> 1);
            tap = tap < TAPS ? tap : TAPS - 1;
            const int kh = tap / KS, kw = tap % KS;
            const int kcol = (S == 2) ? ((kw & 1) * G::IWH + (kw >> 1)) : kw;
            xoff3[f] = (((wrow * S + kh) * G::IWP + p + kcol) * 16) + (q & 1) * XS3::PLANE;
        }
    }
    const unsigned char* xt8 = reinterpret_cast<const unsigned char*>(xt);
    const unsigned char* wrd8 = reinterpret_cast<const unsigned char*>(wt) + lane * 16;

    std::conditional_t<X3, XS3, XStage<KS, S, MODE, MT, TW, X2>> xs;
    xs.init(d);
    if (KS == 2 && S == 1) {
        xs.pad_h = d.pad == 2 ? 1 - (z >> 1) : 0;
        xs.pad_w = d.pad == 2 ? 1 - (z & 1) : 0;
    }
    const __amdgpu_buffer_rsrc_t rw = ctl_rsrc(wp, (int64_t)ctl_cdiv(d.cout, 16) * NFRAG * G_chunks * WSPL * 1024);
    f32x4 wv[NW];
    int wrel[NW];
#pragma unroll
    for (int i = 0; i < NW; ++i) {
        const int u = tid + i * 256;
        const int tt = u >> 6, l = u & 63;
        const int sp = X3 ? tt % WSPL : 0, tq = tt / WSPL;
        const int tap = tq / NT, t = tq - tap * NT;
        wrel[i] = (u < WU) ? (((((cot0 + t) * NFRAG + tap) * G_chunks) * WSPL + sp) * 64 + l) * 16 : CTL_OOB;
    }
    auto wload = [&](int g) {
#pragma unroll
        for (int i = 0; i < NW; ++i) wv[i] = ctl_bload4s(rw, wrel[i], g * WSPL * 1024);
    };
    auto wstore = [&](int img = 0) {
#pragma unroll
        for (int i = 0; i < NW; ++i) {
            const int u = tid + i * 256;
            if (u < WU) *reinterpret_cast<f32x4*>(wt + img * WT_FLOATS + u * 4) = wv[i];
        }
    };

    TileWalk cur, nxt;
    cur.init(bid0, nb, tiles_h, tiles_w);
    nxt = cur;
    TM_DECL
    if (!PC && total_it > 0) {
        xs.load(rx, rx2, d, cur.n, cur.th * G::TH, cur.tw * TW, 0);
        wload(0);
    }
    f32x4 bias4[NT];
    float bv[NT][4];
    {
        const bool has_bias = (flags & CTL_EPI_BIAS) != 0;
        const float* bp = has_bias ? bias : wpack;
#pragma unroll
        for (int t = 0; t < NT; ++t) {
            const int co0 = (cot0 + t) * 16 + q * 4;
#pragma unroll
            for (int k = 0; k < 4; ++k) bv[t][k] = bp[has_bias ? (co0 + k < d.cout ? co0 + k : d.cout - 1) : k];
        }
    }
    {
        const int ncf = ngroups * d.cin;
        const bool pro_on = X2 || d.pro_affine != 0;
        const bool con = pro_on && tid < ncf;
        const int ci = con ? tid : 0;
        float c0, c1, c2 = 0.f;
        if constexpr (X2) {
            const int gi = ci / d.cin, ch = ci - gi * d.cin;
            c0 = pro_scale[(gi * 3 + 0) * d.cin + ch]; c1 = pro_scale[(gi * 3 + 1) * d.cin + ch]; c2 = pro_scale[(gi * 3 + 2) * d.cin + ch];
        } else {
            const float* ps = pro_on ? pro_scale : wpack;
            const float* ph = pro_on ? pro_shift : wpack;
            c0 = ps[ci]; c1 = ph[ci];
        }
        static_assert(NT == 1 || NT == 2, "bias hand-over written for one or two cout tiles per block");
        if constexpr (NT == 1)
            asm volatile("" : "+v"(c0), "+v"(c1), "+v"(c2), "+v"(bv[0][0]), "+v"(bv[0][1]), "+v"(bv[0][2]), "+v"(bv[0][3]));
        else
            asm volatile("" : "+v"(c0), "+v"(c1), "+v"(c2), "+v"(bv[0][0]), "+v"(bv[0][1]), "+v"(bv[0][2]), "+v"(bv[0][3]),
                              "+v"(bv[NT - 1][0]), "+v"(bv[NT - 1][1]), "+v"(bv[NT - 1][2]), "+v"(bv[NT - 1][3]));
        const bool hb = (flags & CTL_EPI_BIAS) != 0;
#pragma unroll
        for (int t = 0; t < NT; ++t) {
            const int co0 = (cot0 + t) * 16 + q * 4;
            bias4[t] = f32x4{(hb && co0 + 0 < d.cout) ? bv[t][0] : 0.f, (hb && co0 + 1 < d.cout) ? bv[t][1] : 0.f,
                             (hb && co0 + 2 < d.cout) ? bv[t][2] : 0.f, (hb && co0 + 3 < d.cout) ? bv[t][3] : 0.f};
            asm volatile("" ::"v"(bias4[t]));
        }
        if (pro_on) {
            if (con) {
                cf_scale[tid] = c0; cf_shift[tid] = c1;
                if constexpr (X2) cf_c[tid] = c2;
            }
            __syncthreads();
        }
    }
    if constexpr (!PC) {
        if (total_it > 0) {
            xs.store(xt, d, 0, cf_scale, cf_shift, (cur.n / group_n) * d.cin, cf_c, rxout, xout_on);
            wstore();
        }
        __syncthreads();
    }

    constexpr bool WREG3 = X3 && !PC && MT == 1 && (NFRAG * NT * 3 <= 15);
    const bool wreg_on = WREG3 && G_chunks == 1;
    x3_bf16x8 wreg[WREG3 ? NFRAG : 1][WREG3 ? 3 : 1][WREG3 ? NT : 1];
    if constexpr (WREG3) {
        if (wreg_on) {
#pragma unroll
            for (int f = 0; f < NFRAG; ++f)
#pragma unroll
                for (int sp = 0; sp < 3; ++sp)
#pragma unroll
                    for (int t = 0; t < NT; ++t) wreg[f][sp][t] = *reinterpret_cast<const x3_bf16x8*>(wrd8 + ((f * NT + t) * 3 + sp) * 1024);
        }
    }

    const int srows = gridDim.x * gridDim.z * (PC ? 4 : 1), srow = (z * gridDim.x + blockIdx.x) * (PC ? 4 : 1) + (PC ? wave : 0);
    auto flush_stats = [&](int grp) {
#pragma unroll
        for (int t = 0; t < NT; ++t) {
            float a[8] = {ssum[t].x, ssum[t].y, ssum[t].z, ssum[t].w, ssq[t].x, ssq[t].y, ssq[t].z, ssq[t].w};
#pragma unroll
            for (int i = 0; i < 8; ++i) {
                float v = a[i];
                v += __shfl_xor(v, 1); v += __shfl_xor(v, 2); v += __shfl_xor(v, 4); v += __shfl_xor(v, 8);
                a[i] = v;
            }
            if constexpr (PC) {
                if (p == 0) {
#pragma unroll
                    for (int r = 0; r < 4; ++r) {
                        const int co = (cot0 + t) * 16 + q * 4 + r;
                        if (co < d.cout) {
                            stats_partial[(((int64_t)grp * srows + srow) * 2 + 0) * d.cout + co] = a[r];
                            stats_partial[(((int64_t)grp * srows + srow) * 2 + 1) * d.cout + co] = a[4 + r];
                        }
                    }
                }
                ssum[t] = ssq[t] = f32x4{0.f, 0.f, 0.f, 0.f};
                continue;
            }
            if (p == 0) {
#pragma unroll
                for (int r = 0; r < 4; ++r) {
                    sred[((wave * NT + t) * 16 + q * 4 + r) * 2 + 0] = a[r];
                    sred[((wave * NT + t) * 16 + q * 4 + r) * 2 + 1] = a[4 + r];
                }
            }
            ssum[t] = ssq[t] = f32x4{0.f, 0.f, 0.f, 0.f};
        }
        if constexpr (PC) return;
        __syncthreads();
        if (tid < NT * 16 * 2) {
            const int stat = tid / (NT * 16), cl = tid % (NT * 16);
            float v = 0.f;
#pragma unroll
            for (int w = 0; w < 4; ++w) v += sred[((w * NT * 16) + cl) * 2 + stat];
            const int co = cot0 * 16 + cl;
            if (co < d.cout) stats_partial[(((int64_t)grp * srows + srow) * 2 + stat) * d.cout + co] = v;
        }
        __syncthreads();
    };
    int cur_grp = (my_tiles > 0) ? cur.n / group_n : 0;
    if constexpr (PC) {
        if ((flags & CTL_EPI_STATS) && ngroups > 1 && consumer && p == 0) {
            for (int gi = 0; gi < ngroups; ++gi)
#pragma unroll
                for (int t = 0; t < NT; ++t)
#pragma unroll
                    for (int r = 0; r < 4; ++r) {
                        const int co = (cot0 + t) * 16 + q * 4 + r;
                        if (co < d.cout) {
                            stats_partial[(((int64_t)gi * srows + srow) * 2 + 0) * d.cout + co] = 0.f;
                            stats_partial[(((int64_t)gi * srows + srow) * 2 + 1) * d.cout + co] = 0.f;
                        }
                    }
        }
    } else if ((flags & CTL_EPI_STATS) && ngroups > 1 && tid < NT * 16 * 2) {
        const int stat = tid / (NT * 16), co = cot0 * 16 + tid % (NT * 16);
        if (co < d.cout)
            for (int gi = 0; gi < ngroups; ++gi) stats_partial[(((int64_t)gi * srows + srow) * 2 + stat) * d.cout + co] = 0.f;
    }

    TM(7)
    f32x4 acc[MT][NT];
#ifndef CTL_X3_ABLATE
#define CTL_X3_ABLATE 0
#endif

    auto mfma_phase3 = [&](auto wreg_tag, const unsigned char* xb, const unsigned char* wb) {
        constexpr bool WR = decltype(wreg_tag)::value;
#ifndef CTL_X3_MS
#define CTL_X3_MS(MT, NT, X2) ((CTL_LB_X3(MT, NT, X2) == 3 || (MT) < 2) ? 1 : 2)
#endif
        constexpr int MS = PC ? (MT >= 2 ? 2 : 1) : CTL_X3_MS(MT, NT, X2);
        constexpr int NSTEP = NFRAG * (MT / MS);
        x3_bf16x8 xf[2][MS][3], wf[2][WR ? 1 : 3][WR ? 1 : NT];
        auto xread = [&](int st, int b) {
            const int f = st / (MT / MS), m0 = (st % (MT / MS)) * MS;
#pragma unroll
            for (int mi = 0; mi < MS; ++mi)
#pragma unroll
                for (int sp = 0; sp < 3; ++sp)
                    xf[b][mi][sp] = *reinterpret_cast<const x3_bf16x8*>(xb + xoff3[f] + ((((m0 + mi) / TWT) * S) * G::IWP + ((m0 + mi) % TWT) * 16) * 16 + 2 * sp * XS3::PLANE);
        };
        auto wread = [&](int f, int b) {
            if constexpr (!WR) {
#pragma unroll
                for (int sp = 0; sp < 3; ++sp)
#pragma unroll
                    for (int t = 0; t < NT; ++t) wf[b][sp][t] = *reinterpret_cast<const x3_bf16x8*>(wb + ((f * NT + t) * 3 + sp) * 1024);
            }
        };
        xread(0, 0);
        wread(0, 0);
#pragma unroll
        for (int st = 0; st < NSTEP; ++st) {
            const int f = st / (MT / MS), m0 = (st % (MT / MS)) * MS, b = st & 1;
            if (st + 1 < NSTEP) {
                xread(st + 1, b ^ 1);
                if ((st + 1) % (MT / MS) == 0) wread(f + 1, (f + 1) & 1);
            }
#pragma unroll
            for (int mi = 0; mi < MS; ++mi) asm volatile("" : "+v"(xf[b][mi][0]), "+v"(xf[b][mi][1]), "+v"(xf[b][mi][2]) : : "memory");
#pragma unroll
            for (int t = 0; t < NT; ++t) {
                x3_bf16x8 ah, am, al;
                if constexpr (WR) { ah = wreg[WREG3 ? f : 0][0][WREG3 ? t : 0]; am = wreg[WREG3 ? f : 0][WREG3 ? 1 : 0][WREG3 ? t : 0]; al = wreg[WREG3 ? f : 0][WREG3 ? 2 : 0][WREG3 ? t : 0]; }
                else { ah = wf[f & 1][0][t]; am = wf[f & 1][WR ? 0 : 1][t]; al = wf[f & 1][WR ? 0 : 2][t]; }
#define CTL_X3_MFMA(A, SP) _Pragma("unroll") for (int mi = 0; mi < MS; ++mi) \
                    acc[m0 + mi][t] = __builtin_amdgcn_mfma_f32_16x16x32_bf16(A, xf[b][mi][SP], acc[m0 + mi][t], 0, 0, 0);
                CTL_X3_MFMA(al, 0)
                CTL_X3_MFMA(ah, 2)
                CTL_X3_MFMA(am, 1)
                CTL_X3_MFMA(am, 0)
                CTL_X3_MFMA(ah, 1)
                CTL_X3_MFMA(ah, 0)
#undef CTL_X3_MFMA
            }
        }
    };

    constexpr bool BNB = (EPI == 3), HAS_OV = (EPI == 1 || EPI == 2);
    f32x4 rv[EPI ? MT : 1][EPI ? NT : 1], ov[HAS_OV ? MT : 1][HAS_OV ? NT : 1], r2[TAIL ? MT : 1][TAIL ? NT : 1];
    f32x4 e_rs[EPI ? NT : 1] = {}, e_rh[EPI ? NT : 1] = {};
    auto tile_full = [&](int ho0, int wo0) {
#ifdef CTL_NO_FULL_EPI
        return false;
#else
        return ho0 + G::TH <= d.hout && wo0 + TW <= d.wout && (cot0 + NT) * 16 <= d.cout;
#endif
    };
    auto tile_ybase = [&](int n, int ho0, int wo0) {
        return (((n * d.out_h + ho0 * d.out_sy + oy0) * d.out_w + wo0 * d.out_sx + ox0) * d.cout + cot0 * 16) * 4;
    };
    auto epi_load = [&](auto full_tag, int n, int ho0, int wo0) {
        constexpr bool FULL = decltype(full_tag)::value;
        if constexpr (EPI != 0) {
            const int grp = n / group_n;
            const int ybase = tile_ybase(n, ho0, wo0);
#pragma unroll
            for (int t = 0; t < NT; ++t) {
                const bool cok = FULL || (cot0 + t) * 16 + q * 4 < d.cout;
#pragma unroll
                for (int m = 0; m < MT; ++m) {
                    const bool pvm = FULL || ((ho0 + wrow + m / TWT < d.hout) && (wo0 + (m % TWT) * 16 + p < d.wout));
                    const int vo = FULL ? (yrel[m] + t * 64) : ((pvm && cok) ? (ybase + yrel[m] + t * 64) : CTL_OOB);
                    const int so = FULL ? ybase : 0;
                    rv[m][t] = f32x4{0.f, 0.f, 0.f, 0.f};
                    if constexpr (HAS_OV) ov[m][t] = f32x4{0.f, 0.f, 0.f, 0.f};
                    if constexpr (BNB) {
                        rv[m][t] = ctl_bload4s(rres, vo, so);
                    } else if constexpr (TAIL) {
                        rv[m][t] = ctl_bload4s(rres, vo, so);
                        r2[m][t] = ctl_bload4s(rres2, vo, so);
                        if (flags & CTL_EPI_ACCUM) ov[m][t] = ctl_bload4s(ry, vo, so);
                    } else if (d.cout >= 4) {
                        if (flags & (CTL_EPI_RES | CTL_EPI_BNBWD)) rv[m][t] = ctl_bload4s(rres, vo, so);
                        if (flags & CTL_EPI_ACCUM) ov[m][t] = ctl_bload4s(ry, vo, so);
                    } else {
                        if (flags & (CTL_EPI_RES | CTL_EPI_BNBWD)) rv[m][t].x = ctl_bload1(rres, vo);
                        if (flags & CTL_EPI_ACCUM) ov[m][t].x = ctl_bload1(ry, vo);
                    }
                }
                const int co0 = (cot0 + t) * 16 + q * 4;
                const int cc = cok ? co0 : 0;
                f32x4 rs = {0.f, 0.f, 0.f, 0.f}, rh = {0.f, 0.f, 0.f, 0.f};
                if (!TAIL && (BNB || (flags & (CTL_EPI_RES | CTL_EPI_BNBWD)))) {
                    if (d.cout >= 4) {
                        rs = *reinterpret_cast<const f32x4*>(res_scale + grp * d.cout + cc);
                        rh = *reinterpret_cast<const f32x4*>(res_shift + grp * d.cout + cc);
                    } else { rs.x = res_scale[grp]; rh.x = res_shift[grp]; }
                }
                e_rs[t] = rs; e_rh[t] = rh;
            }
        }
    };
    auto epi_finish = [&](auto full_tag, int n, int ho0, int wo0) {
        constexpr bool FULL = decltype(full_tag)::value;
        const int ybase = tile_ybase(n, ho0, wo0);
#ifndef CTL_NO_FAST_EPI
        if constexpr (!EPI && FULL) {
            if (d.epi_act == CTL_ACT_NONE) {
                if (flags & CTL_EPI_STATS) {
                    asm volatile("" ::: "memory");
#pragma unroll
                    for (int t = 0; t < NT; ++t)
#pragma unroll
                        for (int m = 0; m < MT; ++m) { ssum[t] += acc[m][t]; ssq[t] += acc[m][t] * acc[m][t]; }
                }
#pragma unroll
                for (int t = 0; t < NT; ++t)
#pragma unroll
                    for (int m = 0; m < MT; ++m) ctl_bstore4(ry, ybase + yrel[m] + t * 64, acc[m][t]);
                return;
            }
        }
#endif
        bool pv[MT];
#pragma unroll
        for (int m = 0; m < MT; ++m)
            pv[m] = FULL || ((ho0 + wrow + m / TWT < d.hout) && (wo0 + (m % TWT) * 16 + p < d.wout));
#pragma unroll
        for (int t = 0; t < NT; ++t) {
            const int co0 = (cot0 + t) * 16 + q * 4;
            const bool cok = FULL || co0 < d.cout;
            const f32x4 rs = e_rs[EPI ? t : 0], rh = e_rh[EPI ? t : 0];
#pragma unroll
            for (int m = 0; m < MT; ++m) {
                f32x4 v = acc[m][t];
                if constexpr (TAIL) {
                    v += ov[m][t];
                    const f32x4 o = rv[m][t];
                    const float sl = d.epi_slope;
                    v.x *= o.x > 0.f ? 1.f : sl; v.y *= o.y > 0.f ? 1.f : sl;
                    v.z *= o.z > 0.f ? 1.f : sl; v.w *= o.w > 0.f ? 1.f : sl;
                    if (FULL || pv[m]) { ssum[t] += v; ssq[t] += v * r2[m][t]; }
                    if (FULL) ctl_bstore4(ry, ybase + yrel[m] + t * 64, v);
                    else ctl_bstore4(ry, (pv[m] && cok) ? (ybase + yrel[m] + t * 64) : CTL_OOB, v);
                    if constexpr (CAN_POOL) {
                        if (pool) {
                            f32x4 hs;
                            hs.x = v.x + __shfl_xor(v.x, 1); hs.y = v.y + __shfl_xor(v.y, 1);
                            hs.z = v.z + __shfl_xor(v.z, 1); hs.w = v.w + __shfl_xor(v.w, 1);
                            if (m < TWT) ov[m][t] = hs;
                            else {
                                const f32x4 top = ov[m - TWT][t];
                                const f32x4 pl = {top.x + hs.x, top.y + hs.y, top.z + hs.z, top.w + hs.w};
                                const int lo = ((((n * (d.out_h >> 1) + ((ho0 + wrow) >> 1)) * (d.out_w >> 1) + ((wo0 + (m % TWT) * 16 + p) >> 1)) * d.cout) + co0) * 4;
                                ctl_bstore4(rpool, ((p & 1) == 0 && (FULL || (pv[m] && cok))) ? lo : CTL_OOB, pl);
                            }
                        }
                    }
                    continue;
                }
                if (BNB || (EPI == 1 && (flags & CTL_EPI_BNBWD))) {
                    const f32x4 u = rv[m][t], sa = u * rs + rh;
                    const float sl = d.epi_slope;
                    v.x *= sa.x > 0.f ? 1.f : sl; v.y *= sa.y > 0.f ? 1.f : sl;
                    v.z *= sa.z > 0.f ? 1.f : sl; v.w *= sa.w > 0.f ? 1.f : sl;
                    if (FULL || pv[m]) { ssum[t] += v; ssq[t] += v * u; }
                } else {
                    if (EPI) v += rv[m][t] * rs + rh;
                    if (flags & CTL_EPI_STATS) {
                        if (FULL) { ssum[t] += v; ssq[t] += v * v; }
                        else if (pv[m]) { ssum[t] += v; ssq[t] += v * v; }
                    }
                }
                if (d.epi_act == CTL_ACT_LEAKY) {
                    v = ctl_leaky01(v, d.epi_slope);
                } else if (d.epi_act == CTL_ACT_SIGMOID) {
                    v.x = 1.f / (1.f + expf(-v.x)); v.y = 1.f / (1.f + expf(-v.y));
                    v.z = 1.f / (1.f + expf(-v.z)); v.w = 1.f / (1.f + expf(-v.w));
                }
                if constexpr (HAS_OV) v += ov[m][t];
                if (FULL) {
                    ctl_bstore4(ry, ybase + yrel[m] + t * 64, v);
                } else {
                    const int vo = (pv[m] && cok) ? (ybase + yrel[m] + t * 64) : CTL_OOB;
                    if (d.cout >= 4) ctl_bstore4(ry, vo, v);
                    else ctl_bstore1(ry, vo, v.x);
                }
            }
        }
    };

    if constexpr (PC) {
        const bool wdouble = G_chunks > 1;
        if (!consumer) {
            constexpr int R = X2 ? CTL_PC_SETS_X2 : CTL_PC_SETS;
            typename XS3::Pay P[R];
            int s_n[R], s_g[R];
            TileWalk lw = cur;
            int lg = 0, lit = 0;
            auto load_step = [&](typename XS3::Pay& pay, int& sn, int& sg) {
                xs.template load<true>(pay, rx, rx2, d, lw.n, lw.th * G::TH, lw.tw * TW, lg, lit < total_it);
                sn = lw.n; sg = lg;
                ++lit;
                if (++lg == G_chunks) { lg = 0; lw.next(); }
            };
#pragma unroll
            for (int r = 0; r < R - 1; ++r) load_step(P[r], s_n[r], s_g[r]);
            wload(0);
            load_step(P[R - 1], s_n[R - 1], s_g[R - 1]);
            auto run = [&](auto wd_tag) {
                constexpr bool WD = decltype(wd_tag)::value;
                int wg = 0;
                auto step = [&](int it, typename XS3::Pay& pay, int& sn, int& sg, bool more) {
                    const int img = it & 1;
#ifdef CTL_TIMING_X3_VMCNT
                    asm volatile("s_waitcnt vmcnt(%0)" :: "n"((R - 1) * XS3::NU * (X2 ? 4 : 2)) : "memory");
                    TM(9)
#endif
                    xs.template store<true>(pay, xt + img * XT_ALLOC, d, sg, cf_scale, cf_shift, (sn / group_n) * d.cin, cf_c, rxout, xout_on);
                    if constexpr (WD) wstore(img);
                    else if (it == 0) wstore(0);
                    TM(3)
                    if (more) {
                        if constexpr (WD) { wg = (wg + 1 == G_chunks) ? 0 : wg + 1; wload(wg); }
                        load_step(pay, sn, sg);
                    }
                    TM(0)
                    ctl_barrier_lds_writes_done();
                    TM(4)
                };
                const int full = (total_it / R) * R;
                for (int it0 = 0; it0 < full; it0 += R) {
#pragma unroll
                    for (int r = 0; r < R; ++r) step(it0 + r, P[r], s_n[r], s_g[r], true);
                }
#pragma unroll
                for (int r = 0; r < R - 1; ++r)
                    if (full + r < total_it) {
                        step(full + r, P[r], s_n[r], s_g[r], false);
                        if constexpr (WD) { if (full + r + 1 < total_it) { wg = (wg + 1 == G_chunks) ? 0 : wg + 1; wload(wg); } }
                    }
            };
            if (wdouble) run(std::true_type{}); else run(std::false_type{});
            TM_FLUSH
            return;
        }
#ifndef CTL_PC_PRIO
#define CTL_PC_PRIO 2
#endif
        __builtin_amdgcn_s_setprio(CTL_PC_PRIO);
        TileWalk cw = cur;
        int g = 0;
        for (int it = 0; it < total_it; ++it) {
            const int n = cw.n, ho0 = cw.th * G::TH, wo0 = cw.tw * TW;
            const bool last = (g == G_chunks - 1);
            const bool full = tile_full(ho0, wo0);
            if (last) {
                const int grp = n / group_n;
                if ((flags & CTL_EPI_STATS) && grp != cur_grp) { flush_stats(cur_grp); cur_grp = grp; }
                if (full) epi_load(std::true_type{}, n, ho0, wo0); else epi_load(std::false_type{}, n, ho0, wo0);
            }
            TM(7)
            ctl_barrier_lds_reads_done();
            TM(2)
            TM_COUNT(6)
            if (g == 0) {
#pragma unroll
                for (int m = 0; m < MT; ++m)
#pragma unroll
                    for (int t = 0; t < NT; ++t) acc[m][t] = bias4[t];
            }
            const int img = it & 1;
            mfma_phase3(std::false_type{}, xt8 + img * (XT_ALLOC * 4), wrd8 + (wdouble ? img : 0) * (WT_FLOATS * 4));
            TM(1)
            if (last) {
                if (full) epi_finish(std::true_type{}, n, ho0, wo0); else epi_finish(std::false_type{}, n, ho0, wo0);
            }
            TM(5)
            if (++g == G_chunks) { g = 0; cw.next(); }
        }
        if (flags & CTL_EPI_STATS) flush_stats(cur_grp);
        TM_FLUSH
        return;
    } else {
    for (int it = 0, g = 0; it < total_it; ++it) {
        TM_COUNT(6)
        const int n = cur.n, ho0 = cur.th * G::TH, wo0 = cur.tw * TW;
        const bool has_next = it + 1 < total_it;
        const int g2 = (g + 1 == G_chunks) ? 0 : g + 1;
        const bool new_w = has_next && G_chunks > 1;
        if (g2 == 0) nxt.next();
        if (has_next && !(X3 && (CTL_X3_ABLATE & 2))) {
            xs.load(rx, rx2, d, nxt.n, nxt.th * G::TH, nxt.tw * TW, g2);
            if (new_w) wload(g2);
        }
        TM(0)
        if (g == 0) {
#pragma unroll
            for (int m = 0; m < MT; ++m)
#pragma unroll
                for (int t = 0; t < NT; ++t) acc[m][t] = bias4[t];
        }
        if constexpr (X3 && (CTL_X3_ABLATE & 4)) {
        } else if constexpr (X3) {
            if constexpr (WREG3) {
                if (wreg_on) mfma_phase3(std::true_type{}, xt8, wrd8);
                else mfma_phase3(std::false_type{}, xt8, wrd8);
            } else {
                mfma_phase3(std::false_type{}, xt8, wrd8);
            }
        } else
        {
            f32x4 wf[2][NT], xf[2][MT];
            auto lds_operands = [&](int tap, int b) {
                const int kh = tap / KS, kw = tap % KS;
                const int kcol = (S == 2) ? ((kw & 1) * G::IWH + (kw >> 1)) : kw;
#pragma unroll
                for (int t = 0; t < NT; ++t) wf[b][t] = *reinterpret_cast<const f32x4*>(wrd + (tap * NT + t) * 256);
#pragma unroll
                for (int m = 0; m < MT; ++m) {
                    if (C4) xf[b][m] = *reinterpret_cast<const f32x4*>(xrd4[tap] + ((m / TWT) * G::IWP + (m % TWT) * 16) * 4);
                    else xf[b][m] = *reinterpret_cast<const f32x4*>(xrd + (((m / TWT) * S + kh) * G::IWP + (m % TWT) * 16 + kcol) * 16);
                }
            };
            lds_operands(0, 0);
#pragma unroll
            for (int tap = 0; tap < NFRAG; ++tap) {
                const int b = tap & 1;
                if (tap + 1 < NFRAG) lds_operands(tap + 1, b ^ 1);
#ifdef CTL_PIN_READ_AHEAD
                __builtin_amdgcn_sched_barrier(0);
#endif
#pragma unroll
                for (int m = 0; m < MT; ++m) {
#pragma unroll
                    for (int t = 0; t < NT; ++t) {
                        acc[m][t] = __builtin_amdgcn_mfma_f32_16x16x4f32(wf[b][t].x, xf[b][m].x, acc[m][t], 0, 0, 0);
                        acc[m][t] = __builtin_amdgcn_mfma_f32_16x16x4f32(wf[b][t].y, xf[b][m].y, acc[m][t], 0, 0, 0);
                        acc[m][t] = __builtin_amdgcn_mfma_f32_16x16x4f32(wf[b][t].z, xf[b][m].z, acc[m][t], 0, 0, 0);
                        acc[m][t] = __builtin_amdgcn_mfma_f32_16x16x4f32(wf[b][t].w, xf[b][m].w, acc[m][t], 0, 0, 0);
                    }
                }
#ifdef CTL_PIN_READ_AHEAD
                __builtin_amdgcn_sched_barrier(0);
#endif
            }
        }

        TM(1)
        ctl_barrier_lds_reads_done();
        TM(2)
#ifdef CTL_TIMING_X3_VMCNT
        asm volatile("s_waitcnt vmcnt(0)" ::: "memory");
        TM(9)
#endif
        if (has_next) {
            xs.store(xt, d, g2, cf_scale, cf_shift, (nxt.n / group_n) * d.cin, cf_c, rxout, xout_on);
            if (new_w) wstore();
        }
        TM(3)
        ctl_barrier_lds_writes_done();
        TM(4)

        if (g == G_chunks - 1 && !(X3 && (CTL_X3_ABLATE & 8))) {
            const int grp = n / group_n;
            if ((flags & CTL_EPI_STATS) && grp != cur_grp) {
                flush_stats(cur_grp);
                cur_grp = grp;
            }
            if (tile_full(ho0, wo0)) { epi_load(std::true_type{}, n, ho0, wo0); epi_finish(std::true_type{}, n, ho0, wo0); }
            else { epi_load(std::false_type{}, n, ho0, wo0); epi_finish(std::false_type{}, n, ho0, wo0); }
        }
        TM(5)
        if (g2 == 0) cur = nxt;
        g = g2;
    }
    }
#ifndef CTL_TIMING_WGRAD
#ifdef CTL_TIMING_DOMINANT_ONLY
    if (KS == 3 && S == 1 && MODE == 0 && MT == 4 && TW == 32 && NT == 1 && EPI == 0)
#endif
    TM_FLUSH
#endif

    if (flags & CTL_EPI_STATS) flush_stats(cur_grp);
}
```

cooperative_training_and_latent_space_data_augmentation_amd/csrc/ctl_conv_x3.hip:

```cpp
#include "ctl_common.h"
#ifdef CTL_TIMING_X3
#define CTL_TM_WAVES 65536
__device__ unsigned long long ctl_tm3[CTL_TM_WAVES][10];
#define TM_DECL unsigned long long tm_prev = __builtin_amdgcn_s_memtime(), tm_acc[10] = {0, 0, 0, 0, 0, 0, 0, 0, 0, 0}; \
                const unsigned long long tm_t0 = tm_prev, tm_r0 = __builtin_amdgcn_s_memrealtime();
#define TM(i) { const unsigned long long tm_now = __builtin_amdgcn_s_memtime(); tm_acc[i] += tm_now - tm_prev; tm_prev = tm_now; }
#define TM_COUNT(i) { tm_acc[i] += 1; }
#ifdef CTL_TIMING_X3_VMCNT
#define CTL_TM3_REAL
#else
#define CTL_TM3_REAL tm_acc[9] = __builtin_amdgcn_s_memrealtime() - tm_r0;
#endif
#define TM_FLUSH { const unsigned w_ = ((blockIdx.x + gridDim.x * (blockIdx.y + gridDim.y * blockIdx.z)) * 8 + (threadIdx.x >> 6)) % CTL_TM_WAVES; \
                   tm_acc[8] = __builtin_amdgcn_s_memtime() - tm_t0; CTL_TM3_REAL \
                   if ((threadIdx.x & 63) == 0) { _Pragma("unroll") for (int i_ = 0; i_ < 10; ++i_) ctl_tm3[w_][i_] += tm_acc[i_]; } }
extern "C" int ctl_debug_timing_x3(unsigned long long* out12) {
    static unsigned long long host[CTL_TM_WAVES][10];
    if (hipMemcpyFromSymbol(host, HIP_SYMBOL(ctl_tm3), sizeof(host)) != hipSuccess) return -1;
    for (int i = 0; i < 12; ++i) out12[i] = 0;
    for (int w = 0; w < CTL_TM_WAVES; ++w) {
        for (int i = 0; i < 10; ++i) out12[i] += host[w][i];
        if (host[w][8] > out12[10]) out12[10] = host[w][8];
        if (host[w][8]) out12[11] += 1;
    }
    for (int w = 0; w < CTL_TM_WAVES; ++w) for (int i = 0; i < 10; ++i) host[w][i] = 0;
    return hipMemcpyToSymbol(HIP_SYMBOL(ctl_tm3), host, sizeof(host)) == hipSuccess ? 0 : -1;
}
#endif
#include "ctl_conv_igemm.h"

__device__ static float x3_pack_value(const float* __restrict__ src, const int64_t* __restrict__ r, int mode, int co, int ci, int kh, int kw) {
    const int cout = (int)r[2], cin = (int)r[3], ks = (int)r[4], flip = (int)r[5];
    if (co >= cout || ci >= cin) return 0.f;
    float v = 0.f;
    if (mode == 1) {
        for (int a = 0; a < 2; ++a) {
            const int sh = a + 2 - kh;
            if (sh < 0 || sh > 2) continue;
            for (int b = 0; b < 2; ++b) {
                const int sw = b + 2 - kw;
                if (sw < 0 || sw > 2) continue;
                v += src[co * r[6] + ci * r[7] + sh * r[8] + sw * r[9]];
            }
        }
    } else if (mode == 2) {
        const int a = flip >> 1, b = flip & 1;
        const int h0 = (kh == 0) ? 0 : (a ? 2 : 1), h1 = (kh == 0) ? (a ? 1 : 0) : 2;
        const int w0 = (kw == 0) ? 0 : (b ? 2 : 1), w1 = (kw == 0) ? (b ? 1 : 0) : 2;
        for (int sh = h0; sh <= h1; ++sh)
            for (int sw = w0; sw <= w1; ++sw) v += src[co * r[6] + ci * r[7] + sh * r[8] + sw * r[9]];
    } else if (mode == 3) {
        const int a = flip >> 1, b = flip & 1;
        const int sh = a ? (kh == 0 ? 2 : 0) : (kh == 0 ? 1 : -1);
        const int sw = b ? (kw == 0 ? 2 : 0) : (kw == 0 ? 1 : -1);
        if (sh >= 0 && sw >= 0) v = src[co * r[6] + ci * r[7] + sh * r[8] + sw * r[9]];
    } else {
        if (flip) { kh = ks - 1 - kh; kw = ks - 1 - kw; }
        v = src[co * r[6] + ci * r[7] + kh * r[8] + kw * r[9]];
    }
    return v;
}
__global__ void pack_weights_x3_batched_kernel(const float* __restrict__ params, float* __restrict__ wpack, const int64_t* __restrict__ table) {
    const int64_t* r = table + (int64_t)blockIdx.y * 12;
    if (!(r[11] & CTL_PACK_X3)) return;
    const int mode = (int)(r[11] & ~(int64_t)CTL_PACK_X3);
    const int cout = (int)r[2], cin = (int)r[3], ks = (int)r[4];
    const int g_chunks = (cin + 15) / 16, taps = ks * ks, nfrag = (taps + 1) / 2;
    const int64_t total = (int64_t)((cout + 15) / 16) * nfrag * g_chunks * 64 * 4;
    const int64_t idx = (int64_t)blockIdx.x * blockDim.x + threadIdx.x;
    if (idx >= total) return;
    const float* src = params + r[0];
    unsigned* dst = reinterpret_cast<unsigned*>(wpack + r[1]);
    const int jp = idx & 3, lane = (idx >> 2) & 63;
    int64_t rest = idx >> 8;
    const int g = rest % g_chunks;
    rest /= g_chunks;
    const int f = rest % nfrag;
    const int cot = rest / nfrag;
    const int co = cot * 16 + (lane & 15), q = lane >> 4;
    const int tap = 2 * f + (q >> 1);
    float a = 0.f, b = 0.f;
    if (tap < taps) {
        const int ci = g * 16 + (q & 1) * 8 + jp * 2;
        a = x3_pack_value(src, r, mode, co, ci, tap / ks, tap % ks);
        b = x3_pack_value(src, r, mode, co, ci + 1, tap / ks, tap % ks);
    }
    const int64_t base = ((((int64_t)cot * nfrag + f) * g_chunks + g) * 3) * 256 + lane * 4 + jp;
#pragma unroll
    for (int sp = 0; sp < 3; ++sp) dst[base + sp * 256] = x3_pack2(x3_part(a, sp), x3_part(b, sp));
}
extern "C" size_t ctl_conv_wpack_floats_x3(int32_t cin, int32_t cout, int32_t ks) {
    return (size_t)ctl_cdiv(cout, 16) * ((ks * ks + 1) / 2) * ctl_cdiv(cin, 16) * 3 * 256;
}
extern "C" int ctl_pack_weights_x3_batched(const float* params, float* wpack, const int64_t* table, int32_t n_rec, int64_t max_total, ctl_stream stream) {
    CTL_REQUIRE(params && wpack && table && n_rec > 0 && max_total > 0, "pack_weights_x3_batched: bad arguments");
    pack_weights_x3_batched_kernel<<<dim3((unsigned)ctl_cdiv64(max_total, 3 * 256) + 1, (unsigned)n_rec), dim3(256), 0, (hipStream_t)stream>>>(params, wpack, table);
    CTL_LAUNCH_CHECK("pack_weights_x3_batched");
    return CTL_OK;
}

struct conv3_call {
    const ctl_conv* d; ctl_conv_cfg c;
    const float *x, *wpack, *bias, *pro_scale, *pro_shift, *res, *res_scale, *res_shift, *res2, *x2;
    float *y, *stats_partial, *pool, *xout;
    hipStream_t stream;
    bool query;
    int grid_x;
    int stat_rows_per_block;
};

#ifndef CTL_X3_PC_DEFAULT
#define CTL_X3_PC_DEFAULT 1
#endif
#ifndef CTL_X3_PC_MIN_STEPS
#define CTL_X3_PC_MIN_STEPS 4
#endif
static bool conv3_pc_shape_ok(const ctl_conv* d) {
    const int f = d->epi_flags & (CTL_EPI_RES | CTL_EPI_ACCUM | CTL_EPI_BNBWD | CTL_EPI_TAILBWD);
    const bool epi_ok = f == 0 || (f == CTL_EPI_BNBWD && d->cout % 16 == 0 && d->epi_act == CTL_ACT_NONE);
    return d->ks == 3 && d->stride == 1 && d->in_mode == CTL_IN_PLAIN && d->nsub == 1 && epi_ok;
}
template <int KS, int S, int MODE, int MT, int TW, int NT, int EPI, bool X2>
constexpr bool conv3_pc_ok() { return S == 1 && KS == 3 && MODE == CTL_IN_PLAIN && (EPI == 0 || EPI == 3); }
template <int KS, int S, int MODE, int MT, int TW, int NT, int EPI, bool X2>
static bool conv3_go_pc(conv3_call& a) {
    if constexpr (conv3_pc_ok<KS, S, MODE, MT, TW, NT, EPI, X2>()) {
        if (!a.c.pc) return false;
        const ctl_conv* d = a.d;
        const int ntiles = d->n * a.c.tiles_h * a.c.tiles_w;
        const int grid_x = ctl_conv_grid_x(ntiles, (a.c.cot / NT) * d->nsub, 1);
        a.grid_x = grid_x;
        a.stat_rows_per_block = 4;
        if (a.query) return true;
        const dim3 grid((unsigned)grid_x, (unsigned)(a.c.cot / NT), (unsigned)d->nsub);
        conv_igemm_kernel<KS, S, MODE, MT, TW, NT, EPI, X2, true, true><<<grid, dim3(512), 0, a.stream>>>(
            *d, a.x, a.wpack, a.bias, a.pro_scale, a.pro_shift, a.res, a.res_scale, a.res_shift, a.y, a.stats_partial, a.c.tiles_h,
            a.c.tiles_w, a.c.g, (int64_t)ctl_conv_wpack_floats_x3(d->cin, d->cout, d->ks), ntiles, a.res2, a.x2, a.pool, a.xout);
        return true;
    }
    return false;
}
template <int KS, int S, int MODE, int MT, int TW, int NT, int EPI, bool X2 = false>
static void conv3_go(conv3_call& a) {
    if constexpr (!X2 && ((KS == 3 && S == 1 && MODE == CTL_IN_PLAIN) || (KS == 4 && S == 2)) && EPI != 2) {
        if (a.d->pro_affine == 2) { conv3_go<KS, S, MODE, MT, TW, NT, EPI, true>(a); return; }
    }
    a.stat_rows_per_block = 1;
    if (conv3_go_pc<KS, S, MODE, MT, TW, NT, EPI, X2>(a)) return;
    static int occ = 0;
    if (!occ) {
        int n = 0;
        if (hipOccupancyMaxActiveBlocksPerMultiprocessor(&n, conv_igemm_kernel<KS, S, MODE, MT, TW, NT, EPI, X2, true>, 256, 0) != hipSuccess || n < 1) {
            (void)hipGetLastError();
            n = 2;
        }
        occ = n;
    }
    const ctl_conv* d = a.d;
    const int ntiles = d->n * a.c.tiles_h * a.c.tiles_w;
    a.grid_x = ctl_conv_grid_x(ntiles, (a.c.cot / NT) * d->nsub, occ);
    if (a.query) return;
    const dim3 grid((unsigned)a.grid_x, (unsigned)(a.c.cot / NT), (unsigned)d->nsub);
    conv_igemm_kernel<KS, S, MODE, MT, TW, NT, EPI, X2, true><<<grid, dim3(256), 0, a.stream>>>(
        *d, a.x, a.wpack, a.bias, a.pro_scale, a.pro_shift, a.res, a.res_scale, a.res_shift, a.y, a.stats_partial, a.c.tiles_h,
        a.c.tiles_w, a.c.g, (int64_t)ctl_conv_wpack_floats_x3(d->cin, d->cout, d->ks), ntiles, a.res2, a.x2, a.pool, a.xout);
}
template <int KS, int S, int MODE>
constexpr bool conv3_tail_ok() { return KS == 2 || (KS == 3 && S == 1 && MODE == CTL_IN_ZINS2); }
template <int KS, int S, int MODE, int MT, int TW>
static void conv3_go_nt(conv3_call& a) {
    constexpr bool NT2 = !(S == 2 && KS >= 3);
    const bool epi = (a.d->epi_flags & (CTL_EPI_RES | CTL_EPI_ACCUM | CTL_EPI_BNBWD)) != 0;
    const bool two = NT2 && a.c.nt == 2;
    auto go = [&](auto E) {
        constexpr int EPI = decltype(E)::value;
        if constexpr (NT2) { if (two) { conv3_go<KS, S, MODE, MT, TW, 2, EPI>(a); return; } }
        conv3_go<KS, S, MODE, MT, TW, 1, EPI>(a);
    };
    if constexpr (conv3_tail_ok<KS, S, MODE>()) {
        if (a.d->epi_flags & CTL_EPI_TAILBWD) { go(std::integral_constant<int, 2>{}); return; }
    }
    if constexpr (KS == 3 && S == 1 && MODE == CTL_IN_PLAIN) {
        if ((a.d->epi_flags & (CTL_EPI_RES | CTL_EPI_ACCUM | CTL_EPI_BNBWD)) == CTL_EPI_BNBWD && a.d->cout % 16 == 0 && a.d->epi_act == CTL_ACT_NONE) {
            go(std::integral_constant<int, 3>{});
            return;
        }
    }
    if (epi) go(std::integral_constant<int, 1>{}); else go(std::integral_constant<int, 0>{});
}
template <int KS, int S, int MODE>
static void conv3_go_tile(conv3_call& a) {
    if (S == 1 && a.c.mt == 4 && a.c.tw == 32) conv3_go_nt<KS, S, MODE, (S == 1 ? 4 : 2), (S == 1 ? 32 : 16)>(a);
    else if (a.c.mt == 2) conv3_go_nt<KS, S, MODE, 2, 16>(a);
    else conv3_go_nt<KS, S, MODE, 1, 16>(a);
}
static int conv3_dispatch(conv3_call& a) {
    const int k = a.d->ks, s = a.d->stride, m = a.d->in_mode;
    if (k == 3 && s == 1 && m == CTL_IN_PLAIN) conv3_go_tile<3, 1, CTL_IN_PLAIN>(a);
    else if (k == 3 && s == 1 && m == CTL_IN_UP2) conv3_go_tile<3, 1, CTL_IN_UP2>(a);
    else if (k == 3 && s == 1 && m == CTL_IN_ZINS2) conv3_go_tile<3, 1, CTL_IN_ZINS2>(a);
    else if (k == 3 && s == 2) conv3_go_tile<3, 2, CTL_IN_PLAIN>(a);
    else if (k == 2 && s == 2) conv3_go_tile<2, 2, CTL_IN_PLAIN>(a);
    else if (k == 2 && s == 1) conv3_go_tile<2, 1, CTL_IN_PLAIN>(a);
    else if (k == 4 && s == 2) conv3_go_nt<4, 2, CTL_IN_PLAIN, 1, 16>(a);
    else CTL_FAIL(CTL_EUNSUPPORTED, "conv_forward(x3): no kernel for ks/stride/in_mode %d/%d/%d", k, s, m);
    return CTL_OK;
}

static int conv3_pick_cfg(const ctl_conv* d, ctl_conv_cfg* c) {
    const int rc = ctl_conv_pick_cfg(d, c, 0);
    if (rc != CTL_OK) return rc;
    static const int pc_on = ctl_tune_int("CTL_X3_PC", CTL_X3_PC_DEFAULT), min_steps = ctl_tune_int("CTL_X3_PC_MIN_STEPS", CTL_X3_PC_MIN_STEPS);
    static const int pc_min_g = ctl_tune_int("CTL_X3_PC_MIN_G", 4);
    if (pc_on && conv3_pc_shape_ok(d) && c->g >= pc_min_g && c->nt == 2) {
        static const int tiles[3][2] = {{4, 32}, {2, 16}, {1, 16}};
        const int other = (c->cot / c->nt) * d->nsub;
        for (int i = 0; i < 3; ++i) {
            const int mt = tiles[i][0], tw = tiles[i][1], th = 4 * mt * 16 / tw;
            if (tw == 32 && d->wout < 32) continue;
            const int64_t ntiles = (int64_t)d->n * ctl_cdiv(d->hout, th) * ctl_cdiv(d->wout, tw);
            if (ntiles * other < ctl_num_cus() && i < 2) continue;
            const int grid_x = ctl_conv_grid_x((int)ntiles, other, 1);
            static const int gate = ctl_tune_int("CTL_X3_PC_GATE", 1);
            const bool shares_ok = !gate || ntiles <= grid_x || ntiles % grid_x == 0;
            if (shares_ok && ntiles * c->g >= (int64_t)min_steps * grid_x) {
                c->pc = 1; c->mt = mt; c->tw = tw; c->th = th;
                c->tiles_h = ctl_cdiv(d->hout, th); c->tiles_w = ctl_cdiv(d->wout, tw);
            }
            break;
        }
    }
    if (d->stride == 2 && d->ks >= 3) {
        c->nt = 1;
        if (d->ks == 4 && c->mt != 1) {
            c->mt = 1; c->tw = 16; c->th = 4;
            c->tiles_h = ctl_cdiv(d->hout, c->th);
            c->tiles_w = ctl_cdiv(d->wout, c->tw);
        }
    }
    return CTL_OK;
}

int ctl_conv_x3_ok(const ctl_conv* d) {
    return d->cin % 16 == 0 && (d->cout % 16 == 0 || (d->cout < 16 && d->cout % 4 == 0)) && d->ks >= 2 && d->in_mode != CTL_IN_C4 && !(d->dt & (CTL_DT_BF16 | CTL_DT_X16 | CTL_DT_Y16 | CTL_DT_RES16));
}
int ctl_conv_x3_stats_blocks(const ctl_conv* d) {
    conv3_call a = {};
    a.d = d;
    if (!ctl_conv_x3_ok(d) || conv3_pick_cfg(d, &a.c) != CTL_OK) return -1;
    a.query = true;
    if (conv3_dispatch(a) != CTL_OK) return -1;
    return a.grid_x * d->nsub * a.stat_rows_per_block;
}
int ctl_conv_forward_x3(const ctl_conv* d, const float* x, const float* wpack, const float* bias, const float* pro_scale, const float* pro_shift,
                        const float* res, const float* res_scale, const float* res_shift, const float* res2, const float* x2, float* y,
                        float* stats_partial, float* pool, float* xout, ctl_stream stream) {
    CTL_REQUIRE(ctl_conv_x3_ok(d), "conv_forward(x3): CTL_DT_X3 needs fp32-stored tensors, cin %% 16 == 0, cout %% 16 == 0 (or 4 / 8 / 12) and a 2x2 / 3x3 / 4x4 kernel "
                                   "(got cin %d, cout %d, ks %d, in_mode %d, dt %d)", d->cin, d->cout, d->ks, d->in_mode, d->dt);
    CTL_REQUIRE(!pool, "conv_forward(x3): `pool` belongs to the 1x1 hosts, which stay on the fp32 pipe");
    conv3_call a = {};
    a.d = d;
    int rc = conv3_pick_cfg(d, &a.c);
    if (rc != CTL_OK) return rc;
    a.x = x; a.wpack = wpack; a.bias = bias; a.pro_scale = pro_scale; a.pro_shift = pro_shift; a.res = res; a.res_scale = res_scale;
    a.res_shift = res_shift; a.res2 = res2; a.x2 = x2; a.y = y; a.stats_partial = stats_partial; a.pool = pool; a.xout = xout;
    a.stream = (hipStream_t)stream;
    a.query = true;
    rc = conv3_dispatch(a);
    if (rc != CTL_OK) return rc;
    a.query = false;
    const int ptok = ctl_prof_begin(a.stat_rows_per_block == 4 ? "conv_igemm_x3pc" : "conv_igemm_x3", d, &a.c, a.c.nt, a.stream);
    rc = conv3_dispatch(a);
    if (ptok >= 0) ctl_prof_end(ptok, a.stream);
    if (rc != CTL_OK) return rc;
    CTL_LAUNCH_CHECK("conv_forward(x3)");
    return CTL_OK;
}
```

cooperative_training_and_latent_space_data_augmentation_amd/csrc/ctl_plan.cpp:

```cpp
#include <stdarg.h>
#include <stdlib.h>
#include <string.h>

#include "ctl_common.h"

static thread_local char g_err[512] = "";

void ctl_set_error(const char* fmt, ...) {
    va_list ap;
    va_start(ap, fmt);
    vsnprintf(g_err, sizeof(g_err), fmt, ap);
    va_end(ap);
}

#include <atomic>
#include <map>
#include <string>
#include <vector>
namespace {
struct ProfRec { std::string id; hipEvent_t a, b; double flops, bytes; void* stream; };
bool g_prof_on = false;
std::string g_prof_filter;
std::vector<ProfRec> g_prof;
std::vector<hipEvent_t> g_prof_pool;
int g_prof_every = 1;
long g_prof_seen = 0;
hipEvent_t prof_event() {
    if (!g_prof_pool.empty()) { hipEvent_t e = g_prof_pool.back(); g_prof_pool.pop_back(); return e; }
    hipEvent_t e = nullptr;
    return hipEventCreate(&e) == hipSuccess ? e : nullptr;
}
}

int ctl_prof_begin(const char* kind, const ctl_conv* d, const ctl_conv_cfg* c, int nt, hipStream_t stream, bool dy2) {
    if (!g_prof_on) return -1;
    char id[160], sfx[40];
    const int f = d->epi_flags;
    const bool bnb_only = (f & (CTL_EPI_RES | CTL_EPI_ACCUM | CTL_EPI_BNBWD)) == CTL_EPI_BNBWD && d->ks == 3 && d->stride == 1 && d->in_mode == CTL_IN_PLAIN && d->cout % 16 == 0;
    const int e32 = (f & CTL_EPI_TAILBWD) ? 2 : (bnb_only ? 3 : ((f & (CTL_EPI_RES | CTL_EPI_ACCUM | CTL_EPI_BNBWD)) ? 1 : 0));
    const int e16 = (f & CTL_EPI_TAILBWD) ? 5 : ((f & CTL_EPI_BNBWD) ? 4 : ((f & CTL_EPI_RES) ? 2 : ((f & CTL_EPI_ACCUM) ? 3 : 0)));
    const int e = (d->dt & CTL_DT_BF16) ? e16 : e32;
    const bool two = d->pro_affine == 2 || dy2;
    char nar[12] = "";
    if (d->cout < 16) snprintf(nar, sizeof(nar), ",co%d", d->cout);
    if (e) snprintf(sfx, sizeof(sfx), ",e%d%s%s", e, two ? ",x2" : "", nar);
    else snprintf(sfx, sizeof(sfx), "%s%s", two ? ",x2" : "", nar);
    static const bool shapes = ctl_tune_str("CTL_PROF_SHAPES") != nullptr;
    if (shapes)
        snprintf(id, sizeof(id), "%s<ks%d,s%d,in%d,mt%d,tw%d,nt%d%s>[n%d,h%d,ci%d,co%d,e%d]", kind, d->ks, d->stride, d->in_mode, c->mt, c->tw, nt, sfx, d->n,
                 d->hout, d->cin, d->cout, d->epi_flags);
    else
        snprintf(id, sizeof(id), "%s<ks%d,s%d,in%d,mt%d,tw%d,nt%d%s>", kind, d->ks, d->stride, d->in_mode, c->mt, c->tw, nt, sfx);
    if (!g_prof_filter.empty() && std::string(id).find(g_prof_filter) == std::string::npos) return -1;
    if (g_prof_every > 1 && (g_prof_seen++ % g_prof_every) != 0) return -1;
    ProfRec r;
    r.id = id;
    r.stream = (void*)stream;
    r.a = prof_event();
    r.b = prof_event();
    if (!r.a || !r.b) return -1;
    const double pix = (double)d->n * d->hout * d->wout * d->nsub;
    r.flops = 2.0 * pix * d->cout * d->cin * d->ks * d->ks;
    const double in_b = ((d->dt & CTL_DT_X16) ? 2.0 : 4.0) * d->n * d->hin * d->win * d->cin, out_b = ((d->dt & CTL_DT_Y16) ? 2.0 : 4.0) * pix * d->cout;
    r.bytes = in_b + out_b;
    if (d->pro_affine == 2) r.bytes += in_b;
    if (dy2) r.bytes += out_b;
    if (d->epi_flags & (CTL_EPI_RES | CTL_EPI_BNBWD)) r.bytes += ((d->dt & CTL_DT_RES16) ? 2.0 : 4.0) * pix * d->cout;
    if (d->epi_flags & CTL_EPI_TAILBWD) r.bytes += 2.0 * 4.0 * pix * d->cout;
    if (d->epi_flags & CTL_EPI_ACCUM) r.bytes += out_b;
    (void)hipEventRecord(r.a, stream);
    g_prof.push_back(r);
    return (int)g_prof.size() - 1;
}
int ctl_prof_begin_raw(const char* id, double flops, double bytes, hipStream_t stream) {
    if (!g_prof_on) return -1;
    if (!g_prof_filter.empty() && std::string(id).find(g_prof_filter) == std::string::npos) return -1;
    if (g_prof_every > 1 && (g_prof_seen++ % g_prof_every) != 0) return -1;
    ProfRec r;
    r.id = id;
    r.stream = (void*)stream;
    r.a = prof_event();
    r.b = prof_event();
    if (!r.a || !r.b) return -1;
    r.flops = flops; r.bytes = bytes;
    (void)hipEventRecord(r.a, stream);
    g_prof.push_back(r);
    return (int)g_prof.size() - 1;
}
static int prof_begin_op(const ctl_op& op, hipStream_t stream) {
    if (!g_prof_on) return -1;
    static const bool timeline = ctl_tune_str("CTL_PROF_TIMELINE") != nullptr;
    char id[96];
    double bytes = 0.0;
    const unsigned m = (unsigned)op.i[25];
    auto w = [&](int bit) { return (m >> bit) & 1u ? 2.0 : 4.0; };
    switch (op.kind) {
        case CTL_OP_BWD_REDUCE: {
            const double e = (double)op.l[0] * op.i[1];
            snprintf(id, sizeof(id), "bwd_reduce<%d>", op.i[0]);
            bytes = e * w(0) + (op.i[0] == 0 ? e * w(1) : 0.0) + (op.i[0] != 2 ? e * w(2) : 0.0) + (op.slot[6] >= 0 ? e * w(3) : 0.0);
            break;
        }
        case CTL_OP_BWD_APPLY: {
            const double e = (double)op.l[0] * op.i[1];
            snprintf(id, sizeof(id), "bwd_apply<%d>", op.i[0]);
            bytes = e * w(0) + (op.i[0] == 0 ? e * w(1) : 0.0) + e * w(2) + (op.slot[6] >= 0 ? e * w(3) : 0.0) + e * w(4);
            break;
        }
        case CTL_OP_BN_ACT: {
            const double e = (double)op.l[0] * op.i[0];
            snprintf(id, sizeof(id), "bn_act");
            bytes = e * w(0) + e * w(1);
            break;
        }
        case CTL_OP_SUMPOOL2: {
            const double e = (double)op.i[0] * op.i[1] * op.i[2] * op.i[3];
            snprintf(id, sizeof(id), "sumpool2");
            bytes = 4.0 * e * w(0) + e * w(1) * (op.i[4] ? 2.0 : 1.0);
            break;
        }
        default:
            if (!timeline) return -1;
            snprintf(id, sizeof(id), "op%d", op.kind);
    }
    if (!g_prof_filter.empty() && std::string(id).find(g_prof_filter) == std::string::npos) return -1;
    if (g_prof_every > 1 && (g_prof_seen++ % g_prof_every) != 0) return -1;
    ProfRec r;
    r.id = id;
    r.stream = (void*)stream;
    r.flops = 0.0;
    r.bytes = bytes;
    r.a = prof_event();
    r.b = prof_event();
    if (!r.a || !r.b) return -1;
    (void)hipEventRecord(r.a, stream);
    g_prof.push_back(r);
    return (int)g_prof.size() - 1;
}
void ctl_prof_end(int token, hipStream_t stream) {
    if (token >= 0 && token < (int)g_prof.size()) (void)hipEventRecord(g_prof[token].b, stream);
}
extern "C" int ctl_prof_start_sampled(const char* filter, int32_t every) {
    for (auto& r : g_prof) { g_prof_pool.push_back(r.a); g_prof_pool.push_back(r.b); }
    g_prof.clear();
    g_prof_filter = filter ? filter : "";
    g_prof_every = every > 1 ? every : 1;
    g_prof_seen = 0;
    g_prof_on = true;
    return CTL_OK;
}
extern "C" int ctl_prof_start(const char* filter) { return ctl_prof_start_sampled(filter, 1); }
extern "C" int ctl_prof_stop(char* out, size_t cap) {
    g_prof_on = false;
    struct Agg { long n = 0; double ms = 0, flops = 0, bytes = 0; };
    std::map<std::string, Agg> agg;
    FILE* tl = nullptr;
    if (const char* path = ctl_tune_str("CTL_PROF_TIMELINE")) tl = fopen(path, "w");
    for (auto& r : g_prof) {
        if (tl && !g_prof.empty() && hipEventSynchronize(r.b) == hipSuccess) {
            float t0 = 0.f, t1 = 0.f;
            if (hipEventElapsedTime(&t0, g_prof[0].a, r.a) == hipSuccess && hipEventElapsedTime(&t1, g_prof[0].a, r.b) == hipSuccess)
                fprintf(tl, "%s %p %.6f %.6f\n", r.id.c_str(), r.stream, t0, t1);
        }
        float ms = 0.f;
        if (hipEventSynchronize(r.b) == hipSuccess && hipEventElapsedTime(&ms, r.a, r.b) == hipSuccess) {
            Agg& a = agg[r.id];
            a.n++; a.ms += ms; a.flops += r.flops; a.bytes += r.bytes;
        }
    }
    for (auto& r : g_prof) { g_prof_pool.push_back(r.a); g_prof_pool.push_back(r.b); }
    g_prof.clear();
    if (tl) fclose(tl);
    std::string text;
    for (auto& kv : agg) {
        char line[320];
        snprintf(line, sizeof(line), "%s launches=%ld ms=%.6f flops=%.6e bytes=%.6e\n", kv.first.c_str(), kv.second.n,
                 kv.second.ms, kv.second.flops, kv.second.bytes);
        text += line;
    }
    if (out && cap) {
        CTL_REQUIRE(text.size() + 1 <= cap, "prof_stop: output buffer too small (%zu needed)", text.size() + 1);
        memcpy(out, text.c_str(), text.size() + 1);
    }
    return CTL_OK;
}

static std::atomic<unsigned long long> g_launches{0};
void ctl_count_launches(int n) { g_launches.fetch_add((unsigned long long)n, std::memory_order_relaxed); }
extern "C" unsigned long long ctl_launch_count(void) { return g_launches.load(std::memory_order_relaxed); }
extern "C" int ctl_version(void) { return CTL_ABI_VERSION; }
extern "C" const char* ctl_last_error(void) { return g_err; }
extern "C" size_t ctl_sizeof_op(void) { return sizeof(ctl_op); }
extern "C" size_t ctl_sizeof_conv(void) { return sizeof(ctl_conv); }

static_assert(sizeof(ctl_conv) == 24 * 4, "ctl_conv must be 24 32-bit words (it is embedded in ctl_op.i[0..23]; i[24] and i[25] are taken)");

extern "C" int ctl_plan_run(const ctl_op* ops, int32_t n_ops, void* const* bases, int32_t n_bases, ctl_stream stream_) {
    CTL_REQUIRE(ops && bases && n_ops >= 0, "plan_run: null arguments");
    const ctl_stream stream = stream_;
#ifdef CTL_TUNING
    static const int skip_mask = ctl_tune_int("CTL_SKIP_OPS", 0);
#endif
    for (int32_t k = 0; k < n_ops; ++k) {
        const ctl_op& op = ops[k];
#ifdef CTL_TUNING
        if (((skip_mask & 1) && op.kind == CTL_OP_BN_FINALIZE) || ((skip_mask & 2) && op.kind == CTL_OP_BN_BWD_FINALIZE) ||
            ((skip_mask & 4) && op.kind == CTL_OP_BWD_REDUCE && op.i[0] == 0) || ((skip_mask & 8) && op.kind == CTL_OP_BWD_REDUCE && op.i[0] == 1) ||
            ((skip_mask & 16) && op.kind == CTL_OP_BWD_APPLY))
            continue;
#endif
        void* t[CTL_OP_MAX_T];
        for (int a = 0; a < CTL_OP_MAX_T; ++a) {
            const int s = op.slot[a];
            if (s < 0) { t[a] = nullptr; continue; }
            CTL_REQUIRE(s < n_bases && bases[s], "plan_run: op %d arg %d uses empty slot %d", k, a, s);
            t[a] = (char*)bases[s] + op.off[a];
        }
#define F(a) ((float*)t[a])
#define NG(v) ((v) > 0 ? (v) : 1)
#define CF(a) ((const float*)t[a])
        int rc = CTL_OK;
        ctl_conv d;
        const int ptok = (op.kind == CTL_OP_CONV || op.kind == CTL_OP_WGRAD) ? -1 : prof_begin_op(op, (hipStream_t)stream);
        switch (op.kind) {
            case CTL_OP_CONV:
                memcpy(&d, op.i, sizeof(d));
                rc = ctl_conv_forward_ex(&d, CF(0), CF(1), CF(2), CF(3), CF(4), CF(5), CF(6), CF(7), CF(10), CF(11), F(8), F(9), F(12), F(13), stream);
                break;
            case CTL_OP_WGRAD:
                CTL_REQUIRE(op.i[24] == 0, "plan_run: op %d is a member record of a WGRAD_GROUP (i[24] = %d splits) without its GROUP record", k, op.i[24]);
                memcpy(&d, op.i, sizeof(d));
                rc = ctl_conv_wgrad_ex(&d, CF(0), CF(1), CF(2), CF(3), CF(6), CF(7), F(4), F(5), stream);
                break;
            case CTL_OP_WGRAD_GROUP: {
                const int nm = op.i[0];
                CTL_REQUIRE(nm >= 1 && nm <= 8 && k + nm < n_ops, "plan_run: op %d WGRAD_GROUP with %d members", k, nm);
                ctl_conv ds[8];
                int32_t sp[8];
                const float *mx[8], *mps[8], *mpb[8], *mdy[8], *mdy2[8], *mco[8];
                float *mw[8], *mb[8];
                for (int j = 0; j < nm; ++j) {
                    const ctl_op& mo = ops[k + 1 + j];
                    CTL_REQUIRE(mo.kind == CTL_OP_WGRAD, "plan_run: op %d: member %d of a WGRAD_GROUP is not a WGRAD record", k, j);
                    void* mt[8];
                    for (int a = 0; a < 8; ++a) {
                        const int s = mo.slot[a];
                        if (s < 0) { mt[a] = nullptr; continue; }
                        CTL_REQUIRE(s < n_bases && bases[s], "plan_run: op %d member %d arg %d uses empty slot %d", k, j, a, s);
                        mt[a] = (char*)bases[s] + mo.off[a];
                    }
                    memcpy(&ds[j], mo.i, sizeof(ctl_conv));
                    sp[j] = mo.i[24];
                    mx[j] = (const float*)mt[0]; mps[j] = (const float*)mt[1]; mpb[j] = (const float*)mt[2]; mdy[j] = (const float*)mt[3];
                    mw[j] = (float*)mt[4]; mb[j] = (float*)mt[5]; mdy2[j] = (const float*)mt[6]; mco[j] = (const float*)mt[7];
                }
                rc = ctl_conv_wgrad_group(nm, ds, sp, mx, mps, mpb, mdy, mdy2, mco, mw, mb, stream);
                k += nm;
                break;
            }
            case CTL_OP_WGRAD_REDUCE:
                memcpy(&d, op.i, sizeof(d));
                rc = ctl_wgrad_reduce(&d, CF(0), CF(1), F(2), op.l[0], op.l[1], op.l[2], op.l[3], F(3), op.i[24], stream);
                break;
            case CTL_OP_PACK:
                rc = ctl_pack_weights(CF(0), F(1), op.i[0], op.i[1], op.i[2], op.l[0], op.l[1], op.l[2], op.l[3], op.i[3], stream);
                break;
            case CTL_OP_BN_FINALIZE:
                rc = ctl_bn_finalize_ex(CF(0), op.i[0], op.i[1], op.l[0], CF(1), CF(2), op.f[0], op.f[1], op.i[2], F(3), F(4),
                                        (int64_t*)t[5], F(6), F(7), F(8), F(9), F(10), NG(op.i[3]), stream);
                break;
            case CTL_OP_BN_REPLAY:
                rc = ctl_bn_replay_running(t[0], F(1), (int64_t*)t[2], (const int64_t*)t[3], op.i[0], op.f[0], stream);
                break;
            case CTL_OP_BN_EVAL:
                rc = ctl_bn_eval_coeffs(op.i[0], CF(0), CF(1), CF(2), CF(3), op.f[0], F(4), F(5), NG(op.i[1]), stream);
                break;
            case CTL_OP_BN_ACT:
                rc = ctl_bn_act_dt(CF(0), CF(1), CF(2), op.f[0], F(3), op.l[0], op.i[0], NG(op.i[1]), (uint32_t)op.i[25], stream);
                break;
            case CTL_OP_BWD_REDUCE:
                rc = ctl_bwd_reduce_dt(op.i[0], CF(0), CF(1), CF(2), CF(3), CF(4), op.f[0], op.l[0], op.i[1], F(5), NG(op.i[2]), (uint32_t)op.i[25], F(6), stream);
                break;
            case CTL_OP_BN_BWD_FINALIZE:
                rc = ctl_bn_bwd_finalize_ex(CF(0), op.i[0], op.l[0], CF(1), CF(2), CF(3), F(4), F(5), F(6), op.i[1], NG(op.i[2]), op.i[3], (uint32_t)op.i[4], stream);
                break;
            case CTL_OP_BWD_APPLY:
                rc = ctl_bwd_apply_dt(op.i[0], CF(0), CF(1), CF(2), CF(3), CF(4), op.f[0], CF(5), op.l[0], op.i[1], F(6), F(7), NG(op.i[2]), (uint32_t)op.i[25], stream);
                break;
            case CTL_OP_CHAN_SUM_FINALIZE:
                rc = ctl_chan_sum_finalize(CF(0), op.i[0], F(1), op.i[1], stream);
                break;
            case CTL_OP_SUMPOOL2:
                rc = ctl_sumpool2_dt(CF(0), F(1), op.i[0], op.i[1], op.i[2], op.i[3], op.i[4], (uint32_t)op.i[25], stream);
                break;
            case CTL_OP_SIGMOID_BWD:
                rc = ctl_sigmoid_bwd(CF(0), CF(1), F(2), op.l[0], stream);
                break;
            case CTL_OP_ZERO: {
                CTL_REQUIRE(t[0] && op.l[0] > 0, "plan_run: op %d ZERO needs a pointer and a size", k);
                ctl_count_launches(1);
                hipError_t e = hipMemsetAsync(t[0], 0, (size_t)op.l[0], (hipStream_t)stream);
                if (e != hipSuccess) CTL_FAIL(CTL_ELAUNCH, "plan_run: memset: %s", hipGetErrorString(e));
                break;
            }
            case CTL_OP_PACK_BATCH:
                rc = (op.i[1] & 1) ? ctl_pack_weights_bf16_batched(CF(0), F(1), (const int64_t*)t[2], op.i[0], op.l[0], stream)
                                   : ctl_pack_weights_batched(CF(0), F(1), (const int64_t*)t[2], op.i[0], op.l[0], stream);
                if (rc == CTL_OK && (op.i[1] & 2)) rc = ctl_pack_weights_x3_batched(CF(0), F(1), (const int64_t*)t[2], op.i[0], op.l[0], stream);
                break;
            case CTL_OP_WGRAD_REDUCE_BATCH:
                rc = ctl_wgrad_reduce_batched(CF(0), F(1), (const int64_t*)t[2], op.i[0], op.l[0], stream);
                break;
            case CTL_OP_DROPOUT2D:
                rc = ctl_dropout2d_dt(t[0], CF(1), (uint64_t)op.l[0], (const int64_t*)t[2], op.f[0], t[3], F(4), op.i[0], op.i[1], op.i[2], (uint32_t)op.i[25], stream);
                break;
            case CTL_OP_COPY: {
                CTL_REQUIRE(t[0] && t[1] && op.l[0] > 0, "plan_run: op %d COPY needs two pointers and a size", k);
                ctl_count_launches(1);
                hipError_t e = hipMemcpyAsync(t[1], t[0], (size_t)op.l[0], hipMemcpyDeviceToDevice, (hipStream_t)stream);
                if (e != hipSuccess) CTL_FAIL(CTL_ELAUNCH, "plan_run: memcpy: %s", hipGetErrorString(e));
                break;
            }
            default:
                CTL_FAIL(CTL_EINVAL, "plan_run: op %d has unknown kind %d", k, op.kind);
        }
#undef F
#undef CF
#undef NG
        if (ptok >= 0) ctl_prof_end(ptok, (hipStream_t)stream);
        if (rc != CTL_OK) {
            char msg[400];
            snprintf(msg, sizeof(msg), "%s", g_err);
            ctl_set_error("plan_run: op %d (kind %d) failed: %s", k, op.kind, msg);
            return rc;
        }
    }
    return CTL_OK;
}
```

cooperative_training_and_latent_space_data_augmentation_amd/nets.py:

```python
from __future__ import annotations

import ctypes
from collections import namedtuple
from typing import Dict, List, Optional, Tuple

import numpy as np
import torch
import torch.nn as nn

from . import _ffi, init as _init
from ._ffi import lib, check, OP_DTYPE

(S_X, S_P, S_B, S_NBT, S_WP, S_ACT, S_SCR, S_OUT0, S_OUT1, S_DOUT0, S_DOUT1, S_GRAD, S_DX, S_BSCR, S_TAB, S_STATE, S_KEEP) = range(17)
N_SLOTS = 17
SLOPE = 0.2
EPS = 1e-5
MOMENTUM = 0.1
SMALL_CIN = True
PHASE_CONVS = True
FUSE_BNBWD = True
FUSE_BNAPPLY = True
FUSE_BNBWD16 = True
FUSE_XOUT16 = True
FUSE_XOUT = False
FUSE_POOL = True
FUSE_PAIR = True
FUSE_PAIR16 = True
FUSE_TAIL16 = True
FUSE_BNAPPLY16 = True
X3 = True
X3_WGRAD = True
GROUP_WGRAD = True
GROUP_WGRAD_BF16 = True
FUSE_TAIL = True
CONV_WORDS = _ffi.CONV_DTYPE.itemsize // 4
ALIGN_F = 64

T = namedtuple("T", "ref n h w c b16", defaults=(False,))


def _rup(x: int, a: int) -> int:
    return (x + a - 1) // a * a


class _Holder(nn.Module):
    """Plain container (stands in for nn.Sequential / the block classes; it owns no compute)."""


class _ConvP(nn.Module):
    def __init__(self, cin, cout, ks, transposed=False):
        super().__init__()
        self.cin, self.cout, self.ks, self.transposed = cin, cout, ks, transposed
        shape = (cin, cout, ks, ks) if transposed else (cout, cin, ks, ks)
        self.weight = nn.Parameter(torch.zeros(shape))
        self.bias = nn.Parameter(torch.zeros(cout))


class _BNP(nn.Module):
    def __init__(self, c):
        super().__init__()
        self.c = c
        self.weight = nn.Parameter(torch.ones(c))
        self.bias = nn.Parameter(torch.zeros(c))
        self.register_buffer("running_mean", torch.zeros(c))
        self.register_buffer("running_var", torch.ones(c))
        self.register_buffer("num_batches_tracked", torch.tensor(0, dtype=torch.long))


class ConvInfo:
    __slots__ = ("key", "cin", "cout", "ks", "transposed", "w_off", "b_off", "wp_fwd", "wp_dgrad", "wp_sub", "wp_up", "wp_upf", "wp_s2d", "wp_ph", "wp_c4")


class BNInfo:
    __slots__ = ("key", "c", "g_off", "b_off", "rm_off", "rv_off", "nbt_idx")


class Arena:

    def __init__(self, slot, b16=False, pp=(0, 1)):
        self.slot, self.size, self.b16, self.pp = slot, 0, b16, pp

    def alloc(self, nbytes: int):
        off = self.size
        self.size += _rup(max(int(nbytes), 4), 256)
        return (self.slot, off)

    def tensor(self, n, h, w, c, *_, b16=None) -> T:
        b16 = self.b16 if b16 is None else b16
        p, P = self.pp
        one = (2 if b16 else 4) * n * h * w * c
        slot, off = self.alloc(P * one)
        return T((slot, off + p * one), n, h, w, c, b16)

    def rows(self, floats: int, groups: int):
        p, P = self.pp
        one = 4 * floats * groups
        slot, off = self.alloc(P * one)
        return (slot, off + p * one)


class _ArenaLease:
    __slots__ = ("free", "t")

    def __init__(self, free, t):
        self.free, self.t = free, t

    def __del__(self):
        if self.free is not None:
            self.free.append(self.t)


class ArenaPool:

    def __init__(self):
        self._free: Dict[tuple, list] = {}

    def acquire(self, nbytes: int, device) -> "_ArenaLease":
        nbytes = max(int(nbytes), 256)
        if torch.cuda.is_current_stream_capturing():
            return _ArenaLease(None, torch.empty(nbytes, dtype=torch.uint8, device=device))
        free = self._free.setdefault((torch.cuda.current_stream().cuda_stream, nbytes), [])
        t = free.pop() if free else torch.empty(nbytes, dtype=torch.uint8, device=device)
        return _ArenaLease(free, t)

    def clear(self):
        for lst in self._free.values():
            lst.clear()


class Plan:
    __slots__ = ("ops", "n_ops", "act_bytes", "scr_bytes", "bscr_bytes", "rec", "out_shapes", "table_np", "table_dev", "groups", "bn_log",
                 "replay", "main_ops", "tail_ops")


_TAIL_KINDS = (_ffi.OP_WGRAD, _ffi.OP_WGRAD_GROUP, _ffi.OP_WGRAD_REDUCE, _ffi.OP_WGRAD_REDUCE_BATCH, _ffi.OP_CHAN_SUM_FINALIZE)


def _stack_rec(obj, P: int):
    if isinstance(obj, T):
        return obj._replace(n=obj.n * P)
    if isinstance(obj, dict):
        return {k: _stack_rec(v, P) for k, v in obj.items()}
    if isinstance(obj, (list, tuple)):
        return type(obj)(_stack_rec(v, P) for v in obj)
    return obj


class _StackedForward:
    __slots__ = ("rec", "groups")

    def __init__(self, rec, groups):
        self.rec, self.groups = rec, groups


class PassStack:

    def __init__(self, net: "CtlNet", P: int = 2):
        self.net, self.P = net, P
        self.lease = None
        self.outs = None
        self.shape = None
        self.plans, self.modes, self.xs, self.roots, self.need_dx, self.seqs = [], [], [], [], [], []
        self.douts = []
        self.keep = []
        self.events = []
        self.done = False

    @property
    def filled(self) -> int:
        return len(self.plans)

    def accepts(self, n, h, w, groups) -> bool:
        return (not self.done and self.filled < self.P and self.net.drop_p is None and
                (self.shape is None or self.shape == (n, h, w, groups)))

    def receive(self, p: int, douts):
        cur = self.douts[p]
        for k, d in enumerate(douts):
            if d is None:
                continue
            d = d.float().contiguous(memory_format=torch.channels_last)
            cur[k] = d if cur[k] is None else cur[k] + d
        ev = torch.cuda.Event()
        ev.record()
        self.events[p].append(ev)


class PlanBuilder:
    def __init__(self, net: "CtlNet"):
        self.net = net
        self.groups = int(getattr(net, "_cur_groups", 1))
        self.ops: List[np.ndarray] = []
        self.b16 = bool(getattr(net, "bf16", False))
        self.pp = tuple(getattr(net, "_cur_pp", (0, 1)))
        self.affine_mask = int(getattr(net, "_cur_affine_mask", 0))
        self.split_tail = bool(getattr(net, "_cur_split", False))
        self.act = Arena(S_ACT, self.b16, self.pp)
        self.bscr = Arena(S_BSCR, self.b16)
        self.scr_bytes = 0
        self.reduce_recs: List[list] = []
        self.pending_wgrads: List[dict] = []
        self.table: Optional[np.ndarray] = None
        self.bn_log: List[tuple] = []

    def op(self, kind: int) -> np.ndarray:
        r = np.zeros((), dtype=OP_DTYPE)
        r["kind"] = kind
        r["slot"][:] = -1
        self.ops.append(r)
        return r

    @staticmethod
    def set_t(op, idx, ref):
        if ref is not None:
            op["slot"][idx] = ref[0]
            op["off"][idx] = ref[1]

    def scr(self, *nbytes):
        refs, off = [], 0
        for nb in nbytes:
            refs.append((S_SCR, off))
            off += _rup(int(nb), 256)
        self.scr_bytes = max(self.scr_bytes, off)
        return refs

    @staticmethod
    def P(off_floats):
        return (S_P, 4 * off_floats)

    @staticmethod
    def G(off_floats):
        return (S_GRAD, 4 * off_floats)

    def _conv_desc(self, x: T, cout, ks, stride, in_mode, hout, wout, pro, flags, act, slope, nsub=1, pad=None, dt=0):
        d = _ffi.conv_desc(n=x.n, hin=x.h, win=x.w, cin=x.c, hout=hout, wout=wout, cout=cout, ks=ks, stride=stride,
                           pad=(1 if ks in (3, 4) else 0) if pad is None else pad, in_mode=in_mode, pro_affine=1 if pro else 0,
                           pro_slope=pro[2] if pro else 0.0, epi_flags=flags, epi_act=act, epi_slope=slope, dt=dt)
        if nsub == 4:
            d["out_h"], d["out_w"], d["out_sy"], d["out_sx"], d["nsub"], d["out_sub"] = 2 * hout, 2 * wout, 2, 2, 4, 1
        d["groups"] = self.groups
        return d

    def conv(self, x: T, wp_ref, cout, ks, *, stride=1, in_mode=0, pro=None, bias_ref=None, stats=False, act=0,
             slope=0.0, res=None, accum=False, out: Optional[T] = None, arena: Optional[Arena] = None, nsub=1,
             hout=None, wout=None, bnbwd=None, pad=None, tail=None, x2=None, keep_stats=False, xout: Optional[T] = None):
        res2, want_pool, pool_t = None, False, None
        if tail is not None:
            assert res is None and bnbwd is None and bias_ref is None and act == 0
            stats, res2, slope = True, tail[1], tail[2]
            want_pool = len(tail) > 3 and bool(tail[3])
        if bnbwd is not None:
            assert res is None and not accum and bias_ref is None and act == 0
            stats, res, slope = True, (bnbwd[0], bnbwd[1], bnbwd[2]), bnbwd[3]
        if hout is None:
            if in_mode == _ffi.IN_UP2:
                hout, wout = 2 * x.h, 2 * x.w
            elif stride == 2:
                hout, wout = ((x.h + 1) // 2, (x.w + 1) // 2) if ks == 3 else (x.h // 2, x.w // 2)
            else:
                hout, wout = x.h, x.w
        flags = (_ffi.EPI_BIAS if bias_ref is not None else 0) | (_ffi.EPI_STATS if stats else 0) | \
                ((_ffi.EPI_BNBWD if bnbwd is not None else _ffi.EPI_RES) if res is not None else 0) | (_ffi.EPI_ACCUM if accum else 0) | \
                (_ffi.EPI_TAILBWD if tail is not None else 0)
        oh, ow = (2 * hout, 2 * wout) if nsub == 4 else (hout, wout)
        if out is None:
            out = (arena or self.act).tensor(x.n, oh, ow, cout)
        assert (out.n, out.h, out.w, out.c) == (x.n, oh, ow, cout), (out, x.n, oh, ow, cout)
        dt = _ffi.DT_X3 if (wp_ref[0] == S_WP and wp_ref[1] // 4 in self.net._x3_packs) else 0
        if self.b16:
            assert bnbwd is None or (x.b16 and out.b16 and bnbwd[0].b16), "CTL_EPI_BNBWD (bf16): x, y and u must be bf16-stored"
            assert tail is None or (out.b16 and tail[0].b16 and tail[1].b16), "CTL_EPI_TAILBWD (bf16): y, out and v must be bf16-stored"
            dt = _ffi.DT_BF16 | (_ffi.DT_X16 if x.b16 else 0) | (_ffi.DT_Y16 if out.b16 else 0) | \
                (_ffi.DT_RES16 if (res is not None and res[0].b16) or tail is not None else 0)
        d = self._conv_desc(x, cout, ks, stride, in_mode, hout, wout, pro, flags, act, slope, nsub, pad, dt)
        if x2 is not None:
            assert pro is None and x.b16 == x2[0].b16 == self.b16 and (x2[0].n, x2[0].h, x2[0].w, x2[0].c) == (x.n, x.h, x.w, x.c)
            d["pro_affine"] = 2
            pro = (x2[1], None)
        op = self.op(_ffi.OP_CONV)
        op["i"][:CONV_WORDS] = np.frombuffer(d.tobytes(), dtype="<i4")
        if want_pool and FUSE_POOL and lib.ctl_conv_pool_ok(_ffi.desc_ptr(d)):
            pool_t = self.bscr.tensor(out.n, out.h // 2, out.w // 2, out.c)
        self.last_pool = pool_t
        stats_ref, blocks = None, 0
        if stats:
            blocks = lib.ctl_conv_stats_blocks(_ffi.desc_ptr(d))
            if blocks <= 0:
                raise _ffi.CtlError("conv plan: " + lib.ctl_last_error().decode())
            if tail is not None or keep_stats:
                stats_ref = self.bscr.alloc(4 * self.groups * blocks * 2 * cout)
            else:
                stats_ref, = self.scr(4 * self.groups * blocks * 2 * cout)
        for idx, ref in enumerate([x.ref, wp_ref, bias_ref, pro[0] if pro else None, pro[1] if pro else None,
                                   (tail[0].ref if tail is not None else (res[0].ref if res else None)), res[1] if res else None, res[2] if res else None,
                                   out.ref, stats_ref, res2.ref if res2 is not None else None, x2[0].ref if x2 is not None else None,
                                   pool_t.ref if pool_t is not None else None, xout.ref if xout is not None else None]):
            self.set_t(op, idx, ref)
        assert xout is None or (x2 is not None and (xout.n, xout.h, xout.w, xout.c, xout.b16) == (x.n, x.h, x.w, x.c, x.b16))
        return out, stats_ref, blocks

    def wgrad(self, x: T, dy: T, ks, *, stride=1, in_mode=0, pro=None, dw_ref, strides, dbias_ref=None, accumulate=False, dy2=None):
        assert dy2 is None or (dy.b16 == dy2[0].b16 == self.b16 and ks == 3 and stride == 1)
        dt = (_ffi.DT_BF16 | (_ffi.DT_X16 if x.b16 else 0) | (_ffi.DT_Y16 if dy.b16 else 0)) if self.b16 else 0
        if (X3 and X3_WGRAD and not self.b16 and x.c % 16 == 0 and dy.c % 16 == 0 and
                ((ks == 3 and in_mode in (_ffi.IN_PLAIN, _ffi.IN_UP2) and (stride == 1 or in_mode == _ffi.IN_PLAIN)) or (ks == 2 and stride == 2 and in_mode == _ffi.IN_PLAIN))):
            dt = _ffi.DT_X3
        d = self._conv_desc(x, dy.c, ks, stride, in_mode, dy.h, dy.w, pro, 0, 0, 0.0, dt=dt)
        dp = _ffi.desc_ptr(d)
        assert dw_ref[0] == S_GRAD and (dbias_ref is None or dbias_ref[0] == S_GRAD)
        refs = [x.ref, pro[0] if pro else None, pro[1] if pro else None, dy.ref, None, None, dy2[0].ref if dy2 else None, dy2[1] if dy2 else None]
        if GROUP_WGRAD and (dt == _ffi.DT_X3 or (GROUP_WGRAD_BF16 and self.b16)):
            cls = int(lib.ctl_wgrad_group_class(dp, 1 if dy2 else 0))
            if cls >= 0:
                self.pending_wgrads.append(dict(cls=cls, d=d, refs=refs, dw_ref=dw_ref, dbias_ref=dbias_ref, strides=[int(v) for v in strides],
                                                accumulate=bool(accumulate), cin=x.c, cout=dy.c, ks=ks))
                return
        self._emit_wgrad(d, refs, dw_ref, dbias_ref, strides, accumulate, x.c, dy.c, ks, None)

    def _emit_wgrad(self, d, refs, dw_ref, dbias_ref, strides, accumulate, cin, cout, ks, splits):
        dp = _ffi.desc_ptr(d)
        cin_p, cout_p = _rup(cin, 16), _rup(cout, 16)
        if splits is None:
            wb, bb = 4 * lib.ctl_wgrad_partial_floats(dp), 4 * lib.ctl_wgrad_bias_partial_floats(dp)
        else:
            wb, bb = 4 * splits * ks * ks * cin_p * cout_p, 4 * splits * cout_p
        if wb == 0:
            raise _ffi.CtlError("wgrad plan: " + lib.ctl_last_error().decode())
        wref = self.bscr.alloc(wb)
        bref = self.bscr.alloc(bb) if dbias_ref is not None else None
        words = np.frombuffer(d.tobytes(), dtype="<i4")
        op = self.op(_ffi.OP_WGRAD)
        op["i"][:CONV_WORDS] = words
        refs = list(refs)
        refs[4], refs[5] = wref, bref
        for idx, ref in enumerate(refs):
            self.set_t(op, idx, ref)
        if splits is None:
            splits = lib.ctl_wgrad_splits(dp)
        else:
            op["i"][CONV_WORDS] = splits
        self.reduce_recs.append([wref[1] // 4, bref[1] // 4 if bref else -1, dw_ref[1] // 4, dbias_ref[1] // 4 if dbias_ref else -1,
                                 splits, (ks * ks) | (ks << 8), cin, cout, cin_p, cout_p, *[int(v) for v in strides],
                                 1 if accumulate else 0, 0])

    def flush_wgrad_groups(self):
        pend, self.pending_wgrads = self.pending_wgrads, []
        by_cls: Dict[int, list] = {}
        for w in pend:
            by_cls.setdefault(w["cls"], []).append(w)
        for cls in sorted(by_cls):
            members = by_cls[cls]
            for g0 in range(0, len(members), _ffi.WGRAD_GROUP_MAX):
                grp = members[g0:g0 + _ffi.WGRAD_GROUP_MAX]
                if len(grp) == 1:
                    w = grp[0]
                    self._emit_wgrad(w["d"], w["refs"], w["dw_ref"], w["dbias_ref"], w["strides"], w["accumulate"], w["cin"], w["cout"], w["ks"], None)
                    continue
                descs = np.concatenate([np.atleast_1d(w["d"]) for w in grp])
                splits = np.zeros(len(grp), dtype=np.int32)
                _ffi.check(lib.ctl_wgrad_group_plan(descs.ctypes.data, len(grp), splits.ctypes.data), "ctl_wgrad_group_plan")
                op = self.op(_ffi.OP_WGRAD_GROUP)
                op["i"][0] = len(grp)
                for w, sp in zip(grp, splits):
                    self._emit_wgrad(w["d"], w["refs"], w["dw_ref"], w["dbias_ref"], w["strides"], w["accumulate"], w["cin"], w["cout"], w["ks"], int(sp))

    def flush_wgrad_reductions(self):
        self.flush_wgrad_groups()
        if not self.reduce_recs:
            return
        assert self.table is None
        self.table = np.asarray(self.reduce_recs, dtype=np.int64)
        op = self.op(_ffi.OP_WGRAD_REDUCE_BATCH)
        op["i"][0] = len(self.reduce_recs)
        op["l"][0] = max(-(-((r[5] & 0xff) * r[6] * r[7] + r[7]) // (64 if r[4] <= 64 else 8)) for r in self.reduce_recs)
        self.set_t(op, 0, (S_BSCR, 0))
        self.set_t(op, 1, (S_GRAD, 0))
        self.set_t(op, 2, (S_TAB, 0))
        self.reduce_recs = []

    def bn_forward(self, bn: BNInfo, stats_ref, blocks, count, mode: str):
        c, G = bn.c, self.groups
        assert count % G == 0
        count //= G
        co = {k: self.act.rows(c, G) for k in ("scale", "shift", "mean", "invstd", "uvar")}
        if mode == "C":
            op = self.op(_ffi.OP_BN_EVAL)
            op["i"][0], op["i"][1] = c, G
            op["f"][0] = EPS
            for idx, ref in enumerate([self.P(bn.g_off), self.P(bn.b_off), (S_B, 4 * bn.rm_off), (S_B, 4 * bn.rv_off),
                                       co["scale"], co["shift"]]):
                self.set_t(op, idx, ref)
            return co
        op = self.op(_ffi.OP_BN_FINALIZE)
        op["i"][0], op["i"][1], op["i"][2], op["i"][3] = blocks, c, 1 if mode == "A" else 0, G
        op["l"][0] = count
        op["f"][0], op["f"][1] = EPS, MOMENTUM
        for idx, ref in enumerate([stats_ref, self.P(bn.g_off), self.P(bn.b_off), (S_B, 4 * bn.rm_off),
                                   (S_B, 4 * bn.rv_off), (S_NBT, 8 * bn.nbt_idx), co["scale"], co["shift"], co["mean"],
                                   co["invstd"], co["uvar"]]):
            self.set_t(op, idx, ref)
        self.bn_log.append((bn, co))
        return co

    @staticmethod
    def mask(*ts) -> int:
        return sum(1 << k for k, t in enumerate(ts) if t is not None and t.b16)

    def bn_act(self, x: T, co, slope, out: T):
        op = self.op(_ffi.OP_BN_ACT)
        op["i"][0], op["i"][1] = x.c, self.groups
        op["i"][25] = self.mask(x, out)
        op["l"][0] = x.n * x.h * x.w
        op["f"][0] = slope
        for idx, ref in enumerate([x.ref, co["scale"], co["shift"], out.ref]):
            self.set_t(op, idx, ref)

    def bn_backward(self, mode_kind: int, dy: T, act_src: Optional[T], bn_src: T, bn: BNInfo, co, slope, *, ds: Optional[T],
                    dx: T, affine_grad: bool):
        c, pixels, G = bn_src.c, bn_src.n * bn_src.h * bn_src.w, self.groups
        assert dx is not None or (mode_kind == 0 and ds is not None)
        part, = self.scr(4 * G * _ffi.RED_BLOCKS * 2 * c)
        coef = self.bscr.alloc(4 * 3 * c * G)
        ds_early = mode_kind == 0 and ds is not None and (not self.b16 or dx is None)
        op = self.op(_ffi.OP_BWD_REDUCE)
        op["i"][0], op["i"][1], op["i"][2] = mode_kind, c, G
        op["i"][25] = self.mask(dy, act_src, bn_src, ds if ds_early else None)
        op["l"][0] = pixels
        op["f"][0] = slope
        for idx, ref in enumerate([dy.ref, act_src.ref if act_src else None, bn_src.ref, co["scale"], co["shift"], part,
                                   ds.ref if ds_early else None]):
            self.set_t(op, idx, ref)
        op = self.op(_ffi.OP_BN_BWD_FINALIZE)
        op["i"][0], op["i"][1], op["i"][2], op["i"][4] = c, 0, G, self.affine_mask
        op["l"][0] = pixels // G
        for idx, ref in enumerate([part, self.P(bn.g_off), co["mean"], co["invstd"], coef,
                                   self.G(bn.g_off) if affine_grad else None, self.G(bn.b_off) if affine_grad else None]):
            self.set_t(op, idx, ref)
        if dx is None:
            return coef
        op = self.op(_ffi.OP_BWD_APPLY)
        if ds_early:
            op["i"][0], op["i"][1], op["i"][2] = 2, c, G
            op["i"][25] = self.mask(ds, None, bn_src, None, dx)
            op["l"][0] = pixels
            for idx, ref in enumerate([ds.ref, None, bn_src.ref, None, None, coef, None, dx.ref]):
                self.set_t(op, idx, ref)
            return coef
        op["i"][0], op["i"][1], op["i"][2] = mode_kind, c, G
        op["i"][25] = self.mask(dy, act_src, bn_src, ds, dx)
        op["l"][0] = pixels
        op["f"][0] = slope
        for idx, ref in enumerate([dy.ref, act_src.ref if act_src else None, bn_src.ref, co["scale"], co["shift"], coef,
                                   ds.ref if ds else None, dx.ref]):
            self.set_t(op, idx, ref)
        return coef

    def bn_backward_from_stats(self, g: T, bn_src: T, bn: BNInfo, co, stats_ref, blocks, *, dx: T, affine_grad: bool):
        c, pixels, G = bn_src.c, bn_src.n * bn_src.h * bn_src.w, self.groups
        coef = self.bscr.alloc(4 * 3 * c * G)
        op = self.op(_ffi.OP_BN_BWD_FINALIZE)
        op["i"][0], op["i"][1], op["i"][2], op["i"][3], op["i"][4] = c, 0, G, blocks, self.affine_mask
        op["l"][0] = pixels // G
        for idx, ref in enumerate([stats_ref, self.P(bn.g_off), co["mean"], co["invstd"], coef,
                                   self.G(bn.g_off) if affine_grad else None, self.G(bn.b_off) if affine_grad else None]):
            self.set_t(op, idx, ref)
        if dx is None:
            return coef
        op = self.op(_ffi.OP_BWD_APPLY)
        op["i"][0], op["i"][1], op["i"][2] = 2, c, G
        op["i"][25] = self.mask(g, None, bn_src, None, dx)
        op["l"][0] = pixels
        for idx, ref in enumerate([g.ref, None, bn_src.ref, None, None, coef, None, dx.ref]):
            self.set_t(op, idx, ref)
        return coef

    def chan_sum(self, dy: T, out_ref):
        c = dy.c
        part, = self.scr(4 * _ffi.RED_BLOCKS * 2 * c)
        op = self.op(_ffi.OP_BWD_REDUCE)
        op["i"][0], op["i"][1] = 2, c
        op["i"][25] = self.mask(dy)
        op["l"][0] = dy.n * dy.h * dy.w
        self.set_t(op, 0, dy.ref)
        self.set_t(op, 5, part)
        op = self.op(_ffi.OP_CHAN_SUM_FINALIZE)
        op["i"][0], op["i"][1] = c, 0
        self.set_t(op, 0, part)
        self.set_t(op, 1, out_ref)

    def sumpool2(self, dup: T, dx: T, accumulate=False):
        op = self.op(_ffi.OP_SUMPOOL2)
        op["i"][:5] = [dx.n, dx.h, dx.w, dx.c, 1 if accumulate else 0]
        op["i"][25] = self.mask(dup, dx)
        self.set_t(op, 0, dup.ref)
        self.set_t(op, 1, dx.ref)

    def sigmoid_bwd(self, dy: T, y: T, dx: T):
        assert not (dy.b16 or y.b16 or dx.b16), "sigmoid_bwd works on the fp32 network output"
        op = self.op(_ffi.OP_SIGMOID_BWD)
        op["l"][0] = y.n * y.h * y.w * y.c
        for idx, ref in enumerate([dy.ref, y.ref, dx.ref]):
            self.set_t(op, idx, ref)

    def dropout(self, z: T, out: T, p: float, *, keep_in=None, keep_out=None, salt: int = 0):
        op = self.op(_ffi.OP_DROPOUT2D)
        op["i"][25] = self.mask(z, out)
        op["i"][0], op["i"][1], op["i"][2] = z.n, z.h * z.w, z.c
        op["f"][0] = p
        op["l"][0] = salt
        for idx, ref in enumerate([z.ref, keep_in, None if keep_in is not None else (S_STATE, 0), out.ref, keep_out]):
            self.set_t(op, idx, ref)

    def zero(self, ref, nbytes):
        op = self.op(_ffi.OP_ZERO)
        op["l"][0] = nbytes
        self.set_t(op, 0, ref)

    def copy(self, src_ref, dst_ref, nbytes):
        op = self.op(_ffi.OP_COPY)
        op["l"][0] = nbytes
        self.set_t(op, 0, src_ref)
        self.set_t(op, 1, dst_ref)

    def finish(self, rec=None, out_shapes=None) -> Plan:
        self.flush_wgrad_reductions()
        p = Plan()
        p.replay = None
        p.table_np, p.table_dev = self.table, None
        p.ops = np.stack(self.ops) if self.ops else np.zeros(0, dtype=OP_DTYPE)
        p.ops = np.ascontiguousarray(p.ops)
        p.n_ops = len(self.ops)
        p.main_ops = p.tail_ops = None
        if self.split_tail:
            tail = []
            for k, o in enumerate(self.ops):
                kind = int(o["kind"])
                if kind in _TAIL_KINDS:
                    tail.append(k)
                    if kind == _ffi.OP_CHAN_SUM_FINALIZE:
                        assert int(self.ops[k - 1]["kind"]) == _ffi.OP_BWD_REDUCE and int(self.ops[k - 1]["i"][0]) == 2
                        tail.insert(len(tail) - 1, k - 1)
            ts = set(tail)
            main = [k for k in range(len(self.ops)) if k not in ts]
            p.main_ops = np.ascontiguousarray(p.ops[main])
            p.tail_ops = np.ascontiguousarray(p.ops[tail]) if tail else None
        p.act_bytes, p.scr_bytes, p.bscr_bytes = self.act.size, self.scr_bytes, self.bscr.size
        p.rec, p.out_shapes = rec, out_shapes
        p.groups = self.groups
        p.bn_log = self.bn_log
        return p


class CtlNet(nn.Module):

    def __init__(self, spec, cin: int, device, bf16: bool = False):
        super().__init__()
        self._spec = spec
        self.cin = cin
        self.bf16 = bool(bf16)
        self._bn_track = True
        self._convs: Dict[str, ConvInfo] = {}
        self._bns: Dict[str, BNInfo] = {}
        self._plans: Dict[tuple, Plan] = {}
        self._packed_ok = False
        self._grad_written = True
        self._grad_is_zero = False
        self._defer_grads = False
        self._deferred: list = []
        self._pass_seq = 0
        self._pending_bwd = 0
        self._on_grads_complete = None
# ... 979 lines not shown
```

include/ctl_hip.h:

```cpp
#ifndef CTL_HIP_H
#define CTL_HIP_H

#include <stddef.h>
#include <stdint.h>

#ifdef __cplusplus
extern "C" {
#endif

typedef void* ctl_stream;

enum ctl_status { CTL_OK = 0, CTL_EINVAL = -1, CTL_EUNSUPPORTED = -2, CTL_ELAUNCH = -3 };

#define CTL_ABI_VERSION 11
int         ctl_version(void);
const char* ctl_last_error(void);

enum { CTL_IN_PLAIN = 0, CTL_IN_UP2 = 1, CTL_IN_ZINS2 = 2, CTL_IN_C4 = 3  };
enum { CTL_ACT_NONE = 0, CTL_ACT_LEAKY = 1, CTL_ACT_SIGMOID = 2 };
enum { CTL_EPI_BIAS = 1, CTL_EPI_ACCUM = 2, CTL_EPI_RES = 4, CTL_EPI_STATS = 8, CTL_EPI_BNBWD = 16, CTL_EPI_TAILBWD = 32 };

typedef struct ctl_conv {
    int32_t n, hin, win, cin;
    int32_t hout, wout, cout;
    int32_t ks, stride, pad;
    int32_t in_mode;
    int32_t pro_affine;
    float   pro_slope;
    int32_t epi_flags;
    int32_t epi_act;
    float   epi_slope;
    int32_t out_h, out_w;
    int32_t out_sy, out_sx;
    int32_t nsub, out_sub;
    int32_t groups;
    int32_t dt;
} ctl_conv;
enum { CTL_DT_BF16 = 1, CTL_DT_X16 = 2, CTL_DT_Y16 = 4, CTL_DT_RES16 = 8, CTL_DT_X3 = 16 };
enum { CTL_PACK_X3 = 16 };

size_t ctl_conv_wpack_floats(int32_t cin, int32_t cout, int32_t ks);
size_t ctl_conv_stats_floats(const ctl_conv* d);
int    ctl_conv_stats_blocks(const ctl_conv* d);

int ctl_pack_weights(const float* src, float* dst, int32_t cout, int32_t cin, int32_t ks,
                     int64_t s_co, int64_t s_ci, int64_t s_kh, int64_t s_kw, int32_t flip, ctl_stream stream);

int ctl_conv_forward(const ctl_conv* d, const float* x, const float* wpack, const float* bias,
                     const float* pro_scale, const float* pro_shift,
                     const float* res, const float* res_scale, const float* res_shift,
                     float* y, float* stats_partial, ctl_stream stream);
int ctl_conv_forward_ex(const ctl_conv* d, const float* x, const float* wpack, const float* bias,
                        const float* pro_scale, const float* pro_shift,
                        const float* res, const float* res_scale, const float* res_shift, const float* res2, const float* x2,
                        float* y, float* stats_partial, float* pool, float* xout, ctl_stream stream);
int ctl_conv_pool_ok(const ctl_conv* d);

int    ctl_wgrad_splits(const ctl_conv* d);
size_t ctl_wgrad_partial_floats(const ctl_conv* d);
size_t ctl_wgrad_bias_partial_floats(const ctl_conv* d);
int ctl_conv_wgrad(const ctl_conv* d, const float* x, const float* pro_scale, const float* pro_shift,
                   const float* dy, float* w_partial, float* b_partial, ctl_stream stream);
int ctl_conv_wgrad_ex(const ctl_conv* d, const float* x, const float* pro_scale, const float* pro_shift,
                      const float* dy, const float* dy2, const float* dy_coef, float* w_partial, float* b_partial, ctl_stream stream);

int ctl_wgrad_group_class(const ctl_conv* d, int32_t has_dy2);
int ctl_wgrad_group_plan(const ctl_conv* descs, int32_t n, int32_t* splits);
int ctl_conv_wgrad_group(int32_t n, const ctl_conv* descs, const int32_t* splits, const float* const* x, const float* const* pro_scale,
                         const float* const* pro_shift, const float* const* dy, const float* const* dy2, const float* const* dy_coef,
                         float* const* w_partial, float* const* b_partial, ctl_stream stream);
int ctl_wgrad_reduce(const ctl_conv* d, const float* w_partial, const float* b_partial,
                     float* dw, int64_t s_co, int64_t s_ci, int64_t s_kh, int64_t s_kw,
                     float* dbias, int32_t accumulate, ctl_stream stream);

int ctl_pack_weights_batched(const float* params, float* wpack, const int64_t* table, int32_t n_rec, int64_t max_total,
                             ctl_stream stream);
int ctl_wgrad_reduce_batched(const float* scratch, float* grad, const int64_t* table, int32_t n_rec, int64_t max_blocks,
                             ctl_stream stream);
int ctl_pack_weights_bf16_batched(const float* params, float* wpack, const int64_t* table, int32_t n_rec, int64_t max_total,
                                  ctl_stream stream);
size_t ctl_conv_wpack_floats_x3(int32_t cin, int32_t cout, int32_t ks);
int ctl_pack_weights_x3_batched(const float* params, float* wpack, const int64_t* table, int32_t n_rec, int64_t max_total,
                                ctl_stream stream);

int ctl_bn_finalize(const float* partial, int32_t blocks, int32_t c, int64_t count, const float* gamma,
                    const float* beta, float eps, float momentum, int32_t update_running, float* running_mean,
                    float* running_var, int64_t* num_batches_tracked, float* scale, float* shift, float* save_mean,
                    float* save_invstd, int32_t groups, ctl_stream stream);
int ctl_bn_finalize_ex(const float* partial, int32_t blocks, int32_t c, int64_t count, const float* gamma,
                       const float* beta, float eps, float momentum, int32_t update_running, float* running_mean,
                       float* running_var, int64_t* num_batches_tracked, float* scale, float* shift, float* save_mean,
                       float* save_invstd, float* save_uvar, int32_t groups, ctl_stream stream);
int ctl_bn_replay_running(const void* act, float* buffers, int64_t* num_batches_tracked, const int64_t* table, int32_t n_rec,
                          float momentum, ctl_stream stream);
int ctl_bn_eval_coeffs(int32_t c, const float* gamma, const float* beta, const float* running_mean,
                       const float* running_var, float eps, float* scale, float* shift, int32_t groups, ctl_stream stream);
int ctl_bn_act(const float* x, const float* scale, const float* shift, float slope, float* y, int64_t pixels,
               int32_t c, int32_t groups, ctl_stream stream);

#ifndef CTL_RED_BLOCKS
#define CTL_RED_BLOCKS 512
#endif
int ctl_bwd_reduce(int32_t mode, const float* dy, const float* act_src, const float* bn_src, const float* scale,
                   const float* shift, float slope, int64_t pixels, int32_t c, float* partial, int32_t groups,
                   ctl_stream stream);
int ctl_bwd_reduce_rows(int32_t mode, int64_t pixels_per_group, int32_t c);
int ctl_red_blocks(void);
int ctl_bn_bwd_finalize(const float* partial, int32_t c, int64_t count, const float* gamma, const float* save_mean,
                        const float* save_invstd, float* coef, float* dgamma, float* dbeta, int32_t accumulate,
                        int32_t groups, int32_t blocks, ctl_stream stream);
int ctl_bn_bwd_finalize_ex(const float* partial, int32_t c, int64_t count, const float* gamma, const float* save_mean,
                           const float* save_invstd, float* coef, float* dgamma, float* dbeta, int32_t accumulate,
                           int32_t groups, int32_t blocks, uint32_t affine_groups, ctl_stream stream);
int ctl_bwd_apply(int32_t mode, const float* dy, const float* act_src, const float* bn_src, const float* scale,
                  const float* shift, float slope, const float* coef, int64_t pixels, int32_t c, float* ds,
                  float* dx, int32_t groups, ctl_stream stream);
int ctl_chan_sum_finalize(const float* partial, int32_t c, float* out, int32_t accumulate, ctl_stream stream);
int ctl_sumpool2(const float* dup, float* dx, int32_t n, int32_t h, int32_t w, int32_t c, int32_t accumulate,
                 ctl_stream stream);
int ctl_sigmoid_bwd(const float* dy, const float* y, float* dx, int64_t count, ctl_stream stream);

int ctl_softmax_t_fwd(const float* x, float inv_t, float* p, int64_t pixels, int32_t c, ctl_stream stream);
int ctl_softmax_t_bwd(const float* p, const float* dp, float inv_t, float* dx, int64_t pixels, int32_t c,
                      ctl_stream stream);
int ctl_onehot(const int64_t* label, float* y, int64_t pixels, int32_t c, ctl_stream stream);
int ctl_ce2d_fwd(const float* logit, const int64_t* label, int64_t pixels, int32_t c, double* partial, float* loss,
                 ctl_stream stream);
int ctl_ce2d_bwd(const float* logit, const int64_t* label, const float* gout, int64_t pixels, int32_t c,
                 float* dlogit, ctl_stream stream);
int ctl_mse_fwd(const float* a, const float* b, int64_t count, float scale, double* partial, float* loss,
                ctl_stream stream);
int ctl_mse_bwd(const float* a, const float* b, const float* gout, int64_t count, float scale, float* da,
                ctl_stream stream);
int ctl_argmax_c(const float* logit, uint8_t* out, int64_t pixels, int32_t c, ctl_stream stream);

int ctl_bn_act_dt(const float* x, const float* scale, const float* shift, float slope, float* y, int64_t pixels, int32_t c,
                  int32_t groups, uint32_t bf16_mask, ctl_stream stream);
int ctl_bwd_reduce_dt(int32_t mode, const float* dy, const float* act_src, const float* bn_src, const float* scale,
                      const float* shift, float slope, int64_t pixels, int32_t c, float* partial, int32_t groups,
                      uint32_t bf16_mask, float* ds, ctl_stream stream);
int ctl_bwd_apply_dt(int32_t mode, const float* dy, const float* act_src, const float* bn_src, const float* scale,
                     const float* shift, float slope, const float* coef, int64_t pixels, int32_t c, float* ds, float* dx,
                     int32_t groups, uint32_t bf16_mask, ctl_stream stream);
int ctl_sumpool2_dt(const float* dup, float* dx, int32_t n, int32_t h, int32_t w, int32_t c, int32_t accumulate,
                    uint32_t bf16_mask, ctl_stream stream);

size_t ctl_latent_score_ws_floats(int32_t mode, int32_t n, int32_t hw, int32_t c);
int ctl_latent_score(int32_t mode, const float* grad, float* score, float* scratch, int32_t n, int32_t hw, int32_t c,
                     ctl_stream stream);
size_t ctl_latent_mask_apply_ws_floats(int32_t mode, int32_t n, int32_t hw, int32_t c);
int ctl_latent_mask_apply(int32_t mode, const float* code, const float* score, const float* soft_noise,
                          int32_t k_host, const int32_t* k_dev, float* masked, float* mask_out, float* scratch, int32_t n,
                          int32_t hw, int32_t c, ctl_stream stream);
size_t ctl_latent_mask_fused_ws_floats(int32_t mode, int32_t n, int32_t hw, int32_t c);
int ctl_latent_mask_fused(int32_t mode, const float* grad, const float* code, const float* soft_noise, int32_t k_host,
                          const int32_t* k_dev, float* masked, float* mask_out, float* score_out, float* workspace, int32_t n,
                          int32_t hw, int32_t c, ctl_stream stream);
int ctl_dropout2d(const float* z, const float* keep, uint64_t seed, float p, float* out, float* keep_out, int32_t n,
                  int32_t hw, int32_t c, ctl_stream stream);
int ctl_uniform(float* out, int64_t count, uint64_t seed, ctl_stream stream);
int ctl_step_tick(int64_t* state, ctl_stream stream);
int ctl_spin(int32_t microseconds, ctl_stream stream);
int ctl_dropout2d_ex(const float* z, const float* keep, uint64_t seed_or_salt, const int64_t* state, float p, float* out,
                     float* keep_out, float* mask_full, int32_t n, int32_t hw, int32_t c, ctl_stream stream);
int ctl_uniform_dev(float* out, int64_t count, uint64_t salt, const int64_t* state, ctl_stream stream);
int ctl_dropout2d_dt(const void* z, const float* keep, uint64_t seed_or_salt, const int64_t* state, float p, void* out,
                     float* keep_out, int32_t n, int32_t hw, int32_t c, uint32_t bf16_mask, ctl_stream stream);

int ctl_confusion_hist(const int64_t* label_true, const uint8_t* label_pred, int64_t count, int32_t n_class, int64_t* hist,
                       ctl_stream stream);
size_t ctl_rescale_intensity_ws_floats(int32_t planes);
int ctl_rescale_intensity(const float* x, float* out, float* workspace, int32_t planes, int64_t plane_elems, float new_min,
                          float new_max, float eps, ctl_stream stream);
int ctl_noise_clamp(const float* x, const float* noise, uint64_t seed, float sigma, float lo, float hi, float* out,
                    int64_t count, ctl_stream stream);
int ctl_crop_or_pad(const void* src, void* dst, int32_t elem_bytes, int32_t n, int32_t h, int32_t w, int32_t new_h,
                    int32_t new_w, ctl_stream stream);

int32_t ctl_surface_stats_rows(int32_t d, int32_t n_class, int32_t foreground_only, int32_t mode);
size_t ctl_surface_stats_ws_bytes(int32_t d, int32_t h, int32_t w, int32_t n_class, int32_t foreground_only, int32_t mode);
int ctl_surface_stats(const uint8_t* pred, const int64_t* gt, int32_t d, int32_t h, int32_t w, int32_t n_class,
                      int32_t foreground_only, int32_t mode, int32_t connectivity, const double* sampling, double* table,
                      void* workspace, size_t workspace_bytes, ctl_stream stream);
size_t ctl_surface_map_ws_bytes(int32_t d, int32_t h, int32_t w, int32_t mode);
int ctl_surface_map(const uint8_t* mask, int32_t d, int32_t h, int32_t w, int32_t mode, int32_t connectivity,
                    const double* sampling, double* d2_out, uint8_t* surface_out, void* workspace, size_t workspace_bytes,
                    ctl_stream stream);

size_t ctl_cc_ws_bytes(int32_t d, int32_t h, int32_t w, int32_t n_class, int32_t mode);
int ctl_cc_label(const uint8_t* labelmap, int32_t d, int32_t h, int32_t w, int32_t n_class, int32_t mode, int32_t connectivity,
                 int32_t* labels, ctl_stream stream);
int ctl_cc_keep_largest(const uint8_t* labelmap, int32_t d, int32_t h, int32_t w, int32_t n_class, int32_t mode, int32_t connectivity,
                        uint8_t* out, int64_t* table, void* workspace, size_t workspace_bytes, ctl_stream stream);

size_t ctl_aug_ws_bytes(int32_t n, int32_t hp, int32_t wp);
size_t ctl_aug_warp_ws_bytes(int32_t n, int32_t hp, int32_t wp, int32_t hc, int32_t wc);
int ctl_aug_field(const float* noise, const uint64_t* seeds, const float* alpha, const float* sigma, int32_t n, int32_t hp, int32_t wp,
                  float* field, void* workspace, size_t workspace_bytes, ctl_stream stream);
int ctl_aug_warp(const float* image, const int64_t* label, const float* matrix, const float* intensity, const float* field, int32_t n,
                 int32_t hp, int32_t wp, int32_t hc, int32_t wc, float* image_out, int64_t* label_out, void* workspace,
                 size_t workspace_bytes, ctl_stream stream);
size_t ctl_aug_spline_ws_bytes(int32_t n, int32_t hp, int32_t wp, int32_t n_class);
size_t ctl_aug_warp_cubic_ws_bytes(int32_t n, int32_t hp, int32_t wp, int32_t hc, int32_t wc, int32_t n_class);
int ctl_aug_spline_coeffs(const float* image, const int64_t* label, const float* intensity, int32_t n, int32_t hp, int32_t wp,
                          int32_t n_class, float* coeffs, void* workspace, size_t workspace_bytes, ctl_stream stream);
int ctl_aug_warp_cubic(const float* image, const int64_t* label, const float* matrix, const float* intensity, const float* field, int32_t n,
                       int32_t hp, int32_t wp, int32_t hc, int32_t wc, int32_t n_class, float* image_out, int64_t* label_out,
                       void* workspace, size_t workspace_bytes, ctl_stream stream);
size_t ctl_aug_bias_ws_bytes(int32_t n, int32_t hp, int32_t wp);
int ctl_aug_bias(const float* image, const float* bias, const float* noise, const uint64_t* seeds, int32_t n, int32_t hp, int32_t wp,
                 float* out, void* workspace, size_t workspace_bytes, ctl_stream stream);
int ctl_aug_coarse_field(const float* coarse, int32_t n, int32_t hp, int32_t wp, float* field, ctl_stream stream);

int ctl_adam(float* p, const float* g, float* m, float* v, int64_t count, float lr, float beta1, float beta2,
             float eps, int32_t step, float grad_scale, ctl_stream stream);
int ctl_accumulate(float* dst, const float* const* srcs, int32_t k, int64_t count, ctl_stream stream);
int ctl_adam_dev(float* p, const float* g, float* m, float* v, int64_t count, float lr, float beta1, float beta2,
                 float eps, const int64_t* state, float grad_scale, ctl_stream stream);

enum ctl_op_kind {
    CTL_OP_CONV = 1, CTL_OP_WGRAD = 2, CTL_OP_WGRAD_REDUCE = 3, CTL_OP_PACK = 4, CTL_OP_BN_FINALIZE = 5,
    CTL_OP_BN_EVAL = 6, CTL_OP_BN_ACT = 7, CTL_OP_BWD_REDUCE = 8, CTL_OP_BN_BWD_FINALIZE = 9, CTL_OP_BWD_APPLY = 10,
    CTL_OP_CHAN_SUM_FINALIZE = 11, CTL_OP_SUMPOOL2 = 12, CTL_OP_SIGMOID_BWD = 13, CTL_OP_ZERO = 14, CTL_OP_COPY = 15, CTL_OP_PACK_BATCH = 16,
    CTL_OP_WGRAD_REDUCE_BATCH = 17, CTL_OP_DROPOUT2D = 18, CTL_OP_BN_REPLAY = 19,
    CTL_OP_WGRAD_GROUP = 20
};
#define CTL_OP_MAX_T 14
typedef struct ctl_op {
    int32_t kind;
    int32_t i[27];
    float   f[4];
    int32_t slot[CTL_OP_MAX_T];
    int64_t off[CTL_OP_MAX_T];
    int64_t l[4];
} ctl_op;
int ctl_plan_run(const ctl_op* ops, int32_t n_ops, void* const* bases, int32_t n_bases, ctl_stream stream);

int ctl_prof_start(const char* filter);
int ctl_prof_start_sampled(const char* filter, int32_t every);
int ctl_prof_stop(char* out, size_t cap);
unsigned long long ctl_launch_count(void);
size_t ctl_sizeof_op(void);
size_t ctl_sizeof_conv(void);

#ifdef __cplusplus
}
#endif
#endif
```

Baseline: 1100.

## Add intra-block K-split teams for small-grid X3 3x3 convolutions

Adds a K-split variant of the X3 implicit-GEMM conv kernel where two 256-thread teams in one 512-thread block each process half of the input-channel chunks. The second team's partial accumulators are then reduced through LDS before the lead team runs the epilogue. The variant is picked for stride-1 3x3 plain-input convs with at least 4 chunks when there are few tiles relative to the grid, and the goal is to fill CUs that otherwise sit idle on deep, small-spatial layers. In exchange it doubles LDS staging, lowers occupancy to one block per CU, and adds an extra barrier plus reduction per tile. It is disabled for eval and for convs flagged as part of an X3 chain.

```diff
diff --git a/cooperative_training_and_latent_space_data_augmentation_amd/_ffi.py b/cooperative_training_and_latent_space_data_augmentation_amd/_ffi.py
--- a/cooperative_training_and_latent_space_data_augmentation_amd/_ffi.py
+++ b/cooperative_training_and_latent_space_data_augmentation_amd/_ffi.py
@@ -25,6 +25,7 @@
     ("epi_flags", "<i4"), ("epi_act", "<i4"), ("epi_slope", "<f4"), ("out_h", "<i4"), ("out_w", "<i4"),
     ("out_sy", "<i4"), ("out_sx", "<i4"), ("nsub", "<i4"), ("out_sub", "<i4"), ("groups", "<i4"), ("dt", "<i4")])
 DT_BF16, DT_X16, DT_Y16, DT_RES16, DT_X3 = 1, 2, 4, 8, 16
+DT_X3_CHAIN = 32
 PACK_X3 = 16
 OP_DTYPE = np.dtype([("kind", "<i4"), ("i", "<i4", (27,)), ("f", "<f4", (4,)), ("slot", "<i4", (OP_MAX_T,)),
                      ("off", "<i8", (OP_MAX_T,)), ("l", "<i8", (4,))], align=True)
diff --git a/cooperative_training_and_latent_space_data_augmentation_amd/csrc/ctl_common.h b/cooperative_training_and_latent_space_data_augmentation_amd/csrc/ctl_common.h
--- a/cooperative_training_and_latent_space_data_augmentation_amd/csrc/ctl_common.h
+++ b/cooperative_training_and_latent_space_data_augmentation_amd/csrc/ctl_common.h
@@ -114,6 +114,7 @@
     int g;
     int cot;
     int pc;
+    int ksplit;
 };
 int ctl_conv_pick_cfg(const ctl_conv* d, ctl_conv_cfg* c, int for_wgrad);
 int ctl_conv_grid_x(int ntiles, int other, int occ);
diff --git a/cooperative_training_and_latent_space_data_augmentation_amd/csrc/ctl_conv.hip b/cooperative_training_and_latent_space_data_augmentation_amd/csrc/ctl_conv.hip
--- a/cooperative_training_and_latent_space_data_augmentation_amd/csrc/ctl_conv.hip
+++ b/cooperative_training_and_latent_space_data_augmentation_amd/csrc/ctl_conv.hip
@@ -792,6 +792,7 @@
         }
     }
     c->pc = 0;
+    c->ksplit = 0;
     c->mt = mt; c->tw = tw; c->th = 4 * mt * 16 / tw;
     c->tiles_h = ctl_cdiv(d->hout, c->th);
     c->tiles_w = ctl_cdiv(d->wout, c->tw);
diff --git a/cooperative_training_and_latent_space_data_augmentation_amd/csrc/ctl_conv_igemm.h b/cooperative_training_and_latent_space_data_augmentation_amd/csrc/ctl_conv_igemm.h
--- a/cooperative_training_and_latent_space_data_augmentation_amd/csrc/ctl_conv_igemm.h
+++ b/cooperative_training_and_latent_space_data_augmentation_amd/csrc/ctl_conv_igemm.h
@@ -171,7 +171,7 @@
 #ifndef CTL_PC_SETS_X2
 #define CTL_PC_SETS_X2 2
 #endif
-template <int KS, int S, int MODE, int MT, int TW, int NT, int EPI, bool X2 = false, bool X3 = false, bool PC = false>
+template <int KS, int S, int MODE, int MT, int TW, int NT, int EPI, bool X2 = false, bool X3 = false, bool PC = false, int KSPLIT = 1>
 #ifndef CTL_LB_X2EPI
 #define CTL_LB_X2EPI 2
 #endif
@@ -184,7 +184,7 @@
 #ifndef CTL_LB_X3
 #define CTL_LB_X3(MT, NT, X2) (((NT) == 1 && (MT) >= 2 && !(X2)) ? 3 : 2)
 #endif
-__global__ __launch_bounds__(PC ? 512 : 256, PC ? 2 : X3 ? CTL_LB_X3(MT, NT, X2) : (MT * NT >= 8 || KS == 4) ? 2 : ((MT * NT >= 4) ? (X2 ? (EPI ? CTL_LB_X2EPI : CTL_LB_X2) : CTL_LB_MID)
+__global__ __launch_bounds__(PC ? 512 : 256 * KSPLIT, KSPLIT > 1 ? 1 : PC ? 2 : X3 ? CTL_LB_X3(MT, NT, X2) : (MT * NT >= 8 || KS == 4) ? 2 : ((MT * NT >= 4) ? (X2 ? (EPI ? CTL_LB_X2EPI : CTL_LB_X2) : CTL_LB_MID)
                                                                                     : ((X2 && EPI) ? CTL_LB_SMALL_X2EPI : CTL_LB_SMALL))) void conv_igemm_kernel(const ctl_conv d, const float* __restrict__ x,
                                                           const float* __restrict__ wpack,
                                                           const float* __restrict__ bias,
@@ -203,11 +203,13 @@
     static_assert(!C4 || (KS == 3 && S == 1), "K-packed taps: 3x3 stride-1 only");
     static_assert(!X3 || !C4, "X3: whole 16-channel chunks");
     static_assert(!PC || X3, "the producer / consumer form exists for the X3 launches");
-    constexpr int NIMG = PC ? 2 : 1;
+    static_assert(KSPLIT == 1 || (X3 && !PC), "the K-split form exists for the single-role X3 launches");
+    constexpr int NIMG = PC ? 2 : KSPLIT;
     using XS3 = XStage3<KS, S, C4 ? CTL_IN_PLAIN : MODE, MT, TW, X2>;
     constexpr int NFRAG = X3 ? (TAPS + 1) / 2 : (C4 ? 3 : TAPS);
     constexpr int WSPL = X3 ? 3 : 1;
-    constexpr int RED_FLOATS = 4 * NT * 16 * 2;
+    constexpr int KRED_FLOATS = (KSPLIT - 1) * MT * NT * 1024;
+    constexpr int RED_FLOATS = 4 * NT * 16 * 2 + KRED_FLOATS;
     constexpr int WT_FLOATS = NFRAG * NT * WSPL * 256;
     constexpr int XT_ALLOC = X3 ? XS3::XT_BYTES / 4 : G::XT_FLOATS;
     static_assert((NIMG * (XT_ALLOC + WT_FLOATS) + RED_FLOATS + (X2 ? 3 : 2) * CTL_PRO_MAX) * 4 <= 160 * 1024, "LDS budget of one CU");
@@ -217,12 +219,16 @@
     float* cf_scale = sred + RED_FLOATS;
     float* cf_shift = cf_scale + CTL_PRO_MAX;
     float* cf_c = cf_shift + (X2 ? CTL_PRO_MAX : 0);
+    float* kred = sred + 4 * NT * 16 * 2;
     constexpr int WU = NFRAG * NT * WSPL * 64, NW = (WU + 255) / 256;
 
-    const int tid = threadIdx.x;
+    const int tid = KSPLIT > 1 ? (threadIdx.x & 255) : threadIdx.x;
     const int lane = tid & 63;
-    const int wave_all = __builtin_amdgcn_readfirstlane(tid >> 6);
-    const int wave = PC ? (wave_all & 3) : wave_all;
+    const int wave_all = __builtin_amdgcn_readfirstlane(threadIdx.x >> 6);
+    const int wave = (PC || KSPLIT > 1) ? (wave_all & 3) : wave_all;
+    const int team = KSPLIT > 1 ? (wave_all >> 2) : 0;
+    const bool lead = KSPLIT == 1 || team == 0;
+    float* const xtm = xt + team * XT_ALLOC;
     const bool consumer = PC && wave_all >= 4;
     const int p = lane & 15, q = lane >> 4;
     const int P = gridDim.x < 8 ? (int)gridDim.x : 8;
@@ -234,7 +240,8 @@
     const int cot0 = blockIdx.y * NT;
     const float* wp = wpack + (int64_t)z * wpack_sub_stride;
     const int my_tiles = (bid0 < t_hi) ? (t_hi - bid0 + nb - 1) / nb : 0;
-    const int total_it = my_tiles * G_chunks;
+    const int GL = KSPLIT > 1 ? G_chunks / KSPLIT : G_chunks;
+    const int total_it = my_tiles * GL;
     const int flags = d.epi_flags;
     const int ngroups = d.groups > 1 ? d.groups : 1;
     const int group_n = d.n / ngroups;
@@ -264,6 +271,7 @@
         yrel[m] = (((wrow + m / TWT) * d.out_sy * d.out_w + ((m % TWT) * 16 + p) * d.out_sx) * d.cout + q * 4) * 4;
     const float* xrd = xt + ((wrow * S) * G::IWP + p) * 16 + q * 4;
     const float* wrd = wt + lane * 4;
+    const float* const wtm = wt + team * WT_FLOATS;
     const float* xrd4[3];
 #pragma unroll
     for (int j = 0; j < 3; ++j) {
@@ -281,11 +289,11 @@
             xoff3[f] = (((wrow * S + kh) * G::IWP + p + kcol) * 16) + (q & 1) * XS3::PLANE;
         }
     }
-    const unsigned char* xt8 = reinterpret_cast<const unsigned char*>(xt);
-    const unsigned char* wrd8 = reinterpret_cast<const unsigned char*>(wt) + lane * 16;
+    const unsigned char* xt8 = reinterpret_cast<const unsigned char*>(xtm);
+    const unsigned char* wrd8 = reinterpret_cast<const unsigned char*>(wtm) + lane * 16;
 
     std::conditional_t<X3, XS3, XStage<KS, S, MODE, MT, TW, X2>> xs;
-    xs.init(d);
+    if constexpr (KSPLIT > 1) xs.init(d, tid); else xs.init(d);
     if (KS == 2 && S == 1) {
         xs.pad_h = d.pad == 2 ? 1 - (z >> 1) : 0;
         xs.pad_w = d.pad == 2 ? 1 - (z & 1) : 0;
@@ -318,8 +326,8 @@
     nxt = cur;
     TM_DECL
     if (!PC && total_it > 0) {
-        xs.load(rx, rx2, d, cur.n, cur.th * G::TH, cur.tw * TW, 0);
-        wload(0);
+        xs.load(rx, rx2, d, cur.n, cur.th * G::TH, cur.tw * TW, team);
+        wload(team);
     }
     f32x4 bias4[NT];
     float bv[NT][4];
@@ -336,7 +344,7 @@
     {
         const int ncf = ngroups * d.cin;
         const bool pro_on = X2 || d.pro_affine != 0;
-        const bool con = pro_on && tid < ncf;
+        const bool con = pro_on && lead && tid < ncf;
         const int ci = con ? tid : 0;
         float c0, c1, c2 = 0.f;
         if constexpr (X2) {
@@ -371,13 +379,13 @@
     }
     if constexpr (!PC) {
         if (total_it > 0) {
-            xs.store(xt, d, 0, cf_scale, cf_shift, (cur.n / group_n) * d.cin, cf_c, rxout, xout_on);
-            wstore();
+            xs.store(xtm, d, team, cf_scale, cf_shift, (cur.n / group_n) * d.cin, cf_c, rxout, xout_on);
+            wstore(team);
         }
         __syncthreads();
     }
 
-    constexpr bool WREG3 = X3 && !PC && MT == 1 && (NFRAG * NT * 3 <= 15);
+    constexpr bool WREG3 = X3 && !PC && KSPLIT == 1 && MT == 1 && (NFRAG * NT * 3 <= 15);
     const bool wreg_on = WREG3 && G_chunks == 1;
     x3_bf16x8 wreg[WREG3 ? NFRAG : 1][WREG3 ? 3 : 1][WREG3 ? NT : 1];
     if constexpr (WREG3) {
@@ -416,7 +424,7 @@
                 ssum[t] = ssq[t] = f32x4{0.f, 0.f, 0.f, 0.f};
                 continue;
             }
-            if (p == 0) {
+            if (p == 0 && lead) {
 #pragma unroll
                 for (int r = 0; r < 4; ++r) {
                     sred[((wave * NT + t) * 16 + q * 4 + r) * 2 + 0] = a[r];
@@ -427,7 +435,7 @@
         }
         if constexpr (PC) return;
         __syncthreads();
-        if (tid < NT * 16 * 2) {
+        if (lead && tid < NT * 16 * 2) {
             const int stat = tid / (NT * 16), cl = tid % (NT * 16);
             float v = 0.f;
 #pragma unroll
@@ -452,7 +460,7 @@
                         }
                     }
         }
-    } else if ((flags & CTL_EPI_STATS) && ngroups > 1 && tid < NT * 16 * 2) {
+    } else if ((flags & CTL_EPI_STATS) && ngroups > 1 && lead && tid < NT * 16 * 2) {
         const int stat = tid / (NT * 16), co = cot0 * 16 + tid % (NT * 16);
         if (co < d.cout)
             for (int gi = 0; gi < ngroups; ++gi) stats_partial[(((int64_t)gi * srows + srow) * 2 + stat) * d.cout + co] = 0.f;
@@ -469,7 +477,7 @@
 #ifndef CTL_X3_MS
 #define CTL_X3_MS(MT, NT, X2) ((CTL_LB_X3(MT, NT, X2) == 3 || (MT) < 2) ? 1 : 2)
 #endif
-        constexpr int MS = PC ? (MT >= 2 ? 2 : 1) : CTL_X3_MS(MT, NT, X2);
+        constexpr int MS = PC ? (MT >= 2 ? 2 : 1) : (KSPLIT > 1 && EPI != 0) ? 1 : CTL_X3_MS(MT, NT, X2);
         constexpr int NSTEP = NFRAG * (MT / MS);
         x3_bf16x8 xf[2][MS][3], wf[2][WR ? 1 : 3][WR ? 1 : NT];
         auto xread = [&](int st, int b) {
@@ -758,19 +766,19 @@
         TM_COUNT(6)
         const int n = cur.n, ho0 = cur.th * G::TH, wo0 = cur.tw * TW;
         const bool has_next = it + 1 < total_it;
-        const int g2 = (g + 1 == G_chunks) ? 0 : g + 1;
-        const bool new_w = has_next && G_chunks > 1;
+        const int g2 = (g + 1 == GL) ? 0 : g + 1;
+        const bool new_w = has_next && GL > 1;
         if (g2 == 0) nxt.next();
         if (has_next && !(X3 && (CTL_X3_ABLATE & 2))) {
-            xs.load(rx, rx2, d, nxt.n, nxt.th * G::TH, nxt.tw * TW, g2);
-            if (new_w) wload(g2);
+            xs.load(rx, rx2, d, nxt.n, nxt.th * G::TH, nxt.tw * TW, g2 * KSPLIT + team);
+            if (new_w) wload(g2 * KSPLIT + team);
         }
         TM(0)
         if (g == 0) {
 #pragma unroll
             for (int m = 0; m < MT; ++m)
 #pragma unroll
-                for (int t = 0; t < NT; ++t) acc[m][t] = bias4[t];
+                for (int t = 0; t < NT; ++t) acc[m][t] = lead ? bias4[t] : f32x4{0.f, 0.f, 0.f, 0.f};
         }
         if constexpr (X3 && (CTL_X3_ABLATE & 4)) {
         } else if constexpr (X3) {
@@ -826,21 +834,41 @@
         TM(9)
 #endif
         if (has_next) {
-            xs.store(xt, d, g2, cf_scale, cf_shift, (nxt.n / group_n) * d.cin, cf_c, rxout, xout_on);
-            if (new_w) wstore();
+            xs.store(xtm, d, g2 * KSPLIT + team, cf_scale, cf_shift, (nxt.n / group_n) * d.cin, cf_c, rxout, xout_on);
+            if (new_w) wstore(team);
         }
         TM(3)
         ctl_barrier_lds_writes_done();
         TM(4)
 
-        if (g == G_chunks - 1 && !(X3 && (CTL_X3_ABLATE & 8))) {
+        if (g == GL - 1 && !(X3 && (CTL_X3_ABLATE & 8))) {
+            if constexpr (KSPLIT > 1) {
+                f32x4* kr = reinterpret_cast<f32x4*>(kred);
+                if (!lead) {
+#pragma unroll
+                    for (int m = 0; m < MT; ++m)
+#pragma unroll
+                        for (int t = 0; t < NT; ++t) kr[(((team - 1) * MT + m) * NT + t) * 256 + tid] = acc[m][t];
+                }
+                ctl_barrier_lds_writes_done();
+                if (lead) {
+#pragma unroll
+                    for (int pt = 1; pt < KSPLIT; ++pt)
+#pragma unroll
+                        for (int m = 0; m < MT; ++m)
+#pragma unroll
+                            for (int t = 0; t < NT; ++t) acc[m][t] += kr[(((pt - 1) * MT + m) * NT + t) * 256 + tid];
+                }
+            }
             const int grp = n / group_n;
             if ((flags & CTL_EPI_STATS) && grp != cur_grp) {
                 flush_stats(cur_grp);
                 cur_grp = grp;
             }
-            if (tile_full(ho0, wo0)) { epi_load(std::true_type{}, n, ho0, wo0); epi_finish(std::true_type{}, n, ho0, wo0); }
-            else { epi_load(std::false_type{}, n, ho0, wo0); epi_finish(std::false_type{}, n, ho0, wo0); }
+            if (lead) {
+                if (tile_full(ho0, wo0)) { epi_load(std::true_type{}, n, ho0, wo0); epi_finish(std::true_type{}, n, ho0, wo0); }
+                else { epi_load(std::false_type{}, n, ho0, wo0); epi_finish(std::false_type{}, n, ho0, wo0); }
+            }
         }
         TM(5)
         if (g2 == 0) cur = nxt;
diff --git a/cooperative_training_and_latent_space_data_augmentation_amd/csrc/ctl_conv_x3.hip b/cooperative_training_and_latent_space_data_augmentation_amd/csrc/ctl_conv_x3.hip
--- a/cooperative_training_and_latent_space_data_augmentation_amd/csrc/ctl_conv_x3.hip
+++ b/cooperative_training_and_latent_space_data_augmentation_amd/csrc/ctl_conv_x3.hip
@@ -140,12 +140,32 @@
     }
     return false;
 }
+#define CTL_X3_KSPLIT_TEAMS 2
+template <int KS, int S, int MODE, int MT, int TW, int NT, int EPI, bool X2>
+constexpr bool conv3_ks_ok() { return S == 1 && KS == 3 && MODE == CTL_IN_PLAIN && (EPI == 0 || EPI == 3) && NT == 2 && TW == 16 && (MT == 1 || MT == 2); }
+template <int KS, int S, int MODE, int MT, int TW, int NT, int EPI, bool X2>
+static bool conv3_go_ks(conv3_call& a) {
+    if constexpr (conv3_ks_ok<KS, S, MODE, MT, TW, NT, EPI, X2>()) {
+        if (a.c.ksplit != CTL_X3_KSPLIT_TEAMS) return false;
+        const ctl_conv* d = a.d;
+        const int ntiles = d->n * a.c.tiles_h * a.c.tiles_w;
+        a.grid_x = ctl_conv_grid_x(ntiles, (a.c.cot / NT) * d->nsub, 1);
+        if (a.query) return true;
+        const dim3 grid((unsigned)a.grid_x, (unsigned)(a.c.cot / NT), (unsigned)d->nsub);
+        conv_igemm_kernel<KS, S, MODE, MT, TW, NT, EPI, X2, true, false, CTL_X3_KSPLIT_TEAMS><<<grid, dim3(256 * CTL_X3_KSPLIT_TEAMS), 0, a.stream>>>(
+            *d, a.x, a.wpack, a.bias, a.pro_scale, a.pro_shift, a.res, a.res_scale, a.res_shift, a.y, a.stats_partial, a.c.tiles_h,
+            a.c.tiles_w, a.c.g, (int64_t)ctl_conv_wpack_floats_x3(d->cin, d->cout, d->ks), ntiles, a.res2, a.x2, a.pool, a.xout);
+        return true;
+    }
+    return false;
+}
 template <int KS, int S, int MODE, int MT, int TW, int NT, int EPI, bool X2 = false>
 static void conv3_go(conv3_call& a) {
     if constexpr (!X2 && ((KS == 3 && S == 1 && MODE == CTL_IN_PLAIN) || (KS == 4 && S == 2)) && EPI != 2) {
         if (a.d->pro_affine == 2) { conv3_go<KS, S, MODE, MT, TW, NT, EPI, true>(a); return; }
     }
     a.stat_rows_per_block = 1;
+    if (conv3_go_ks<KS, S, MODE, MT, TW, NT, EPI, X2>(a)) return;
     if (conv3_go_pc<KS, S, MODE, MT, TW, NT, EPI, X2>(a)) return;
     static int occ = 0;
     if (!occ) {
@@ -229,6 +249,13 @@
             }
             break;
         }
+    }
+    static const int ks_teams = ctl_tune_int("CTL_X3_KSPLIT", CTL_X3_KSPLIT_TEAMS), ks_max_tiles = ctl_tune_int("CTL_X3_KSPLIT_MAX_TILES", 1);
+    if (ks_teams == CTL_X3_KSPLIT_TEAMS && !(d->dt & CTL_DT_X3_CHAIN) && conv3_pc_shape_ok(d) && c->nt == 2 && c->g >= 4 &&
+        c->g % CTL_X3_KSPLIT_TEAMS == 0 && c->tw == 16 && (c->mt == 1 || c->mt == 2)) {
+        const int64_t ntiles = (int64_t)d->n * c->tiles_h * c->tiles_w;
+        const int grid_x = ctl_conv_grid_x((int)ntiles, (c->cot / c->nt) * d->nsub, 1);
+        if (ntiles <= (int64_t)ks_max_tiles * grid_x) { c->ksplit = CTL_X3_KSPLIT_TEAMS; c->pc = 0; }
     }
     if (d->stride == 2 && d->ks >= 3) {
         c->nt = 1;
diff --git a/cooperative_training_and_latent_space_data_augmentation_amd/csrc/ctl_plan.cpp b/cooperative_training_and_latent_space_data_augmentation_amd/csrc/ctl_plan.cpp
--- a/cooperative_training_and_latent_space_data_augmentation_amd/csrc/ctl_plan.cpp
+++ b/cooperative_training_and_latent_space_data_augmentation_amd/csrc/ctl_plan.cpp
@@ -34,7 +34,7 @@
 
 int ctl_prof_begin(const char* kind, const ctl_conv* d, const ctl_conv_cfg* c, int nt, hipStream_t stream, bool dy2) {
     if (!g_prof_on) return -1;
-    char id[160], sfx[40];
+    char id[160], sfx[48];
     const int f = d->epi_flags;
     const bool bnb_only = (f & (CTL_EPI_RES | CTL_EPI_ACCUM | CTL_EPI_BNBWD)) == CTL_EPI_BNBWD && d->ks == 3 && d->stride == 1 && d->in_mode == CTL_IN_PLAIN && d->cout % 16 == 0;
     const int e32 = (f & CTL_EPI_TAILBWD) ? 2 : (bnb_only ? 3 : ((f & (CTL_EPI_RES | CTL_EPI_ACCUM | CTL_EPI_BNBWD)) ? 1 : 0));
@@ -43,8 +43,10 @@
     const bool two = d->pro_affine == 2 || dy2;
     char nar[12] = "";
     if (d->cout < 16) snprintf(nar, sizeof(nar), ",co%d", d->cout);
-    if (e) snprintf(sfx, sizeof(sfx), ",e%d%s%s", e, two ? ",x2" : "", nar);
-    else snprintf(sfx, sizeof(sfx), "%s%s", two ? ",x2" : "", nar);
+    char ksp[8] = "";
+    if (c->ksplit > 1) snprintf(ksp, sizeof(ksp), ",k%d", c->ksplit);
+    if (e) snprintf(sfx, sizeof(sfx), ",e%d%s%s%s", e, two ? ",x2" : "", nar, ksp);
+    else snprintf(sfx, sizeof(sfx), "%s%s%s", two ? ",x2" : "", nar, ksp);
     static const bool shapes = ctl_tune_str("CTL_PROF_SHAPES") != nullptr;
     if (shapes)
         snprintf(id, sizeof(id), "%s<ks%d,s%d,in%d,mt%d,tw%d,nt%d%s>[n%d,h%d,ci%d,co%d,e%d]", kind, d->ks, d->stride, d->in_mode, c->mt, c->tw, nt, sfx, d->n,
diff --git a/cooperative_training_and_latent_space_data_augmentation_amd/nets.py b/cooperative_training_and_latent_space_data_augmentation_amd/nets.py
--- a/cooperative_training_and_latent_space_data_augmentation_amd/nets.py
+++ b/cooperative_training_and_latent_space_data_augmentation_amd/nets.py
@@ -195,6 +195,7 @@
         self.pp = tuple(getattr(net, "_cur_pp", (0, 1)))
         self.affine_mask = int(getattr(net, "_cur_affine_mask", 0))
         self.split_tail = bool(getattr(net, "_cur_split", False))
+        self.x3_chain = bool(getattr(net, "_cur_x3_chain", False)) or not bool(getattr(net, "training", True))
         self.act = Arena(S_ACT, self.b16, self.pp)
         self.bscr = Arena(S_BSCR, self.b16)
         self.scr_bytes = 0
@@ -267,6 +268,8 @@
             out = (arena or self.act).tensor(x.n, oh, ow, cout)
         assert (out.n, out.h, out.w, out.c) == (x.n, oh, ow, cout), (out, x.n, oh, ow, cout)
         dt = _ffi.DT_X3 if (wp_ref[0] == S_WP and wp_ref[1] // 4 in self.net._x3_packs) else 0
+        if dt and self.x3_chain:
+            dt |= _ffi.DT_X3_CHAIN
         if self.b16:
             assert bnbwd is None or (x.b16 and out.b16 and bnbwd[0].b16), "CTL_EPI_BNBWD (bf16): x, y and u must be bf16-stored"
             assert tail is None or (out.b16 and tail[0].b16 and tail[1].b16), "CTL_EPI_TAILBWD (bf16): y, out and v must be bf16-stored"
diff --git a/include/ctl_hip.h b/include/ctl_hip.h
--- a/include/ctl_hip.h
+++ b/include/ctl_hip.h
@@ -36,7 +36,7 @@
     int32_t groups;
     int32_t dt;
 } ctl_conv;
-enum { CTL_DT_BF16 = 1, CTL_DT_X16 = 2, CTL_DT_Y16 = 4, CTL_DT_RES16 = 8, CTL_DT_X3 = 16 };
+enum { CTL_DT_BF16 = 1, CTL_DT_X16 = 2, CTL_DT_Y16 = 4, CTL_DT_RES16 = 8, CTL_DT_X3 = 16, CTL_DT_X3_CHAIN = 32 };
 enum { CTL_PACK_X3 = 16 };
 
 size_t ctl_conv_wpack_floats(int32_t cin, int32_t cout, int32_t ks);
```

Result: slower. 1088 (-1.1%).
